# kkrt-labs/stwo-brainfuck

Hardware: AMD Instinct MI355X
Metric: trace cells committed+proved/sec (higher is better)
Workload: dtype u32 (M31 / QM31 modular arithmetic)

## Files before the change

bindings/rust/bfhip_sys.rs:

```rust
#![allow(non_camel_case_types, dead_code)]
use std::ffi::{c_char, c_void};

#[repr(C)] pub struct BfhipCtx { _private: [u8; 0] }
#[repr(C)] pub struct BfhipTrace { _private: [u8; 0] }
#[repr(C)] #[derive(Clone, Copy, Default, Debug, PartialEq, Eq)] pub struct BfhipConventions { pub merkle_node_hash: u32, pub mix_u64: u32, pub logup_mask_order: u32, pub merkle_channel: u32, pub reserved: [u32; 4] }
#[repr(C)] #[derive(Clone, Copy, Debug, PartialEq, Eq)] pub struct BfhipPcsConfig { pub pow_bits: u32, pub log_blowup_factor: u32, pub log_last_layer_degree_bound: u32, pub n_queries: u32, pub reserved: [u32; 4] }
#[repr(C)] #[derive(Clone, Copy, Default, Debug, PartialEq, Eq)] pub struct BfhipCheckReport { pub component: u32, pub log_size: u32, pub n_bad_cells: u64, pub first_bad_cell: u64, pub first_bad_constraint: i32, pub first_bad_value: [u32; 4], pub bad_per_constraint: [u64; 16], pub claimed_sum: [u32; 4], pub reserved: [u32; 3] }
#[repr(C)] #[derive(Clone, Copy, Default, Debug, PartialEq, Eq)] pub struct BfhipRelationEntry { pub relation: u32, pub n_words: u32, pub tuple: [u32; 7], pub net: u32, pub n_yield: u64, pub n_use: u64, pub n_other: u64, pub first_yield_table: i32, pub first_use_table: i32, pub first_yield_row: u64, pub first_use_row: u64, pub reserved: [u32; 2] }
#[repr(C)] #[derive(Clone, Copy, Default, Debug, PartialEq, Eq)] pub struct BfhipRelationReport { pub relation: u32, pub n_words: u32, pub n_entries: u64, pub n_tuples: u64, pub n_unbalanced: u64, pub n_reported: u64, pub reserved: [u32; 2] }
#[repr(C)] #[derive(Clone, Copy, Debug)] pub struct BfhipRelationTable { pub component: i32, pub log_size: u32, pub main_rows_h: *const *const u32 }
#[repr(C)] pub struct BfhipLocalGroup { _private: [u8; 0] }
#[repr(C)] pub struct BfhipPool { _private: [u8; 0] }
#[repr(C)] pub struct BfhipChannel { _private: [u8; 0] }
#[repr(C)] pub struct BfhipPcs { _private: [u8; 0] }
#[repr(C)] pub struct BfhipPcsVerifier { _private: [u8; 0] }
#[repr(C)] pub struct BfhipAir { _private: [u8; 0] }
#[repr(C)] pub struct BfhipAirKernel { _private: [u8; 0] }
#[repr(C)] #[derive(Clone, Copy, Debug, PartialEq, Eq)] pub struct BfhipAirCheckReport { pub log_size: u32, pub n_constraints: u32, pub n_bad_cells: u64, pub first_bad_cell: u64, pub first_bad_constraint: i32, pub reserved0: u32, pub first_bad_value: [u32; 4], pub bad_per_constraint: [u64; 64], pub first_cell_per_constraint: [u64; 64], pub reserved: [u64; 2] }
#[repr(C)] pub struct BfhipLogup { _private: [u8; 0] }
#[repr(C)] pub struct BfhipRelationProgram { _private: [u8; 0] }
#[repr(C)] #[derive(Clone, Copy, Debug)] pub struct BfhipRelationProgramTable { pub program: *const BfhipRelationProgram, pub log_size: u32, pub row_shift: u32, pub cols_h: *const *const u32, pub col_shifts_h: *const u32 }
#[repr(C)] #[derive(Clone, Copy, Default, Debug, PartialEq, Eq)] pub struct BfhipMultiplicityReport { pub relation: u32, pub n_words: u32, pub target_table: u32, pub target_entry: u32, pub n_rows: u64, pub n_row_tuples: u64, pub n_entries: u64, pub n_tuples: u64, pub n_filled: u64, pub n_missing: u64, pub n_reported: u64, pub reserved: [u32; 2] }
#[repr(C)] #[derive(Clone, Copy, Debug)] pub struct BfhipPoolResult { pub ticket: u64, pub user_tag: u64, pub status: i32, pub worker: u32, pub flags: u32, pub log_max_rows: u32, pub proof_json: *mut c_char, pub proof_len: usize, pub error: *mut c_char, pub seconds_queued: f64, pub seconds_proving: f64, pub reserved: [u64; 2] }
#[repr(C)] #[derive(Clone, Copy, Debug)] pub struct BfhipPreflightReport { pub ran: u32, pub rejected: u32, pub n_bad_components: i32, pub n_entries: u32, pub logup_total: [u32; 4], pub components: [BfhipCheckReport; 13], pub relations: [BfhipRelationReport; 3], pub entries: [BfhipRelationEntry; 12], pub seconds: f64, pub reserved: [u64; 3] }
pub const BFHIP_TRACE_REJECTED: i32 = -3;
pub const BFHIP_JOB_CANCELLED: i32 = -2;
pub const BFHIP_POOL_MAX_OUTSTANDING: u32 = 4096;
pub const BFHIP_PCS_MAX_SAMPLES_PER_COLUMN: u32 = 2;
pub const BFHIP_PCS_MAX_POINTS: u32 = 64;
pub const BFHIP_PCS_MAX_COLUMNS: u32 = 4096;
pub const BFHIP_PCS_MAX_TREES: u32 = 64;
pub const BFHIP_AIR_M_COL: u32 = 0; pub const BFHIP_AIR_M_CONST: u32 = 1; pub const BFHIP_AIR_M_ADD: u32 = 2; pub const BFHIP_AIR_M_SUB: u32 = 3;
pub const BFHIP_AIR_M_MUL: u32 = 4; pub const BFHIP_AIR_M_NEG: u32 = 5; pub const BFHIP_AIR_Q_COL: u32 = 6; pub const BFHIP_AIR_Q_PARAM: u32 = 7;
pub const BFHIP_AIR_Q_FROM_M: u32 = 8; pub const BFHIP_AIR_Q_ADD: u32 = 9; pub const BFHIP_AIR_Q_SUB: u32 = 10; pub const BFHIP_AIR_Q_MUL: u32 = 11;
pub const BFHIP_AIR_Q_MULM: u32 = 12; pub const BFHIP_AIR_C_BASE: u32 = 13; pub const BFHIP_AIR_C_EXT: u32 = 14;
pub const BFHIP_AIR_MAX_M_REGS: u32 = 96; pub const BFHIP_AIR_MAX_Q_REGS: u32 = 24; pub const BFHIP_AIR_MAX_INSTRUCTIONS: u32 = 4096;
pub const BFHIP_AIR_MAX_COLUMNS: u32 = 256; pub const BFHIP_AIR_MAX_PARAMS: u32 = 64; pub const BFHIP_AIR_MAX_CONSTRAINTS: u32 = 64;
pub const BFHIP_AIR_MAX_OFFSET: i32 = 16;
pub const BFHIP_LOGUP_FRAC: u32 = 15; pub const BFHIP_LOGUP_END_COL: u32 = 16; pub const BFHIP_LOGUP_MAX_COLUMNS: u32 = 8; pub const BFHIP_LOGUP_MAX_FRACTIONS: u32 = 32;
pub const BFHIP_REL_WORD: u32 = 17; pub const BFHIP_REL_ENTRY: u32 = 18; pub const BFHIP_RELATION_PROGRAM_MAX_RELATIONS: u32 = 16;
pub const BFHIP_RELATION_PROGRAM_MAX_WORDS: u32 = 7; pub const BFHIP_RELATION_PROGRAM_MAX_ENTRIES: u32 = 32;

#[link(name = "bfhip")]
extern "C" {
    pub fn bfhip_last_error() -> *const c_char;
    pub fn bfhip_device_count() -> i32;
    pub fn bfhip_device_memory(device_id: i32, free_bytes: *mut u64, total_bytes: *mut u64) -> i32;
    pub fn bfhip_ctx_create(device_id: i32, max_log_domain: u32, out: *mut *mut BfhipCtx) -> i32;
    pub fn bfhip_ctx_destroy(ctx: *mut BfhipCtx) -> i32;
    pub fn bfhip_ctx_sync(ctx: *mut BfhipCtx) -> i32;
    pub fn bfhip_ctx_set_overlap(ctx: *mut BfhipCtx, mask: u32) -> i32;
    pub fn bfhip_ctx_memory(ctx: *mut BfhipCtx, out: *mut u64) -> i32;
    pub fn bfhip_ctx_set_sync_policy(ctx: *mut BfhipCtx, blocking: i32) -> i32;
    pub fn bfhip_ctx_set_mailbox(ctx: *mut BfhipCtx, mode: i32, timeout_ms: u32, test_delay_ms: i32) -> i32;
    pub fn bfhip_ctx_set_conventions(ctx: *mut BfhipCtx, conv: *const BfhipConventions) -> i32;
    pub fn bfhip_ctx_get_conventions(ctx: *mut BfhipCtx, out: *mut BfhipConventions) -> i32;
    pub fn bfhip_ctx_set_pcs_config(ctx: *mut BfhipCtx, pcs: *const BfhipPcsConfig) -> i32;
    pub fn bfhip_ctx_get_pcs_config(ctx: *mut BfhipCtx, out: *mut BfhipPcsConfig) -> i32;
    pub fn bfhip_malloc(ctx: *mut BfhipCtx, bytes: usize, out_d: *mut *mut c_void) -> i32;
    pub fn bfhip_free(ctx: *mut BfhipCtx, ptr_d: *mut c_void) -> i32;
    pub fn bfhip_upload(ctx: *mut BfhipCtx, dst_d: *mut c_void, src_h: *const c_void, bytes: usize) -> i32;
    pub fn bfhip_download(ctx: *mut BfhipCtx, dst_h: *mut c_void, src_d: *const c_void, bytes: usize) -> i32;
    pub fn bfhip_memset_zero(ctx: *mut BfhipCtx, dst_d: *mut c_void, bytes: usize) -> i32;
    pub fn bfhip_twiddles(ctx: *mut BfhipCtx, tw_d: *mut *const u32, itw_d: *mut *const u32, root_log: *mut u32) -> i32;
    pub fn bfhip_interpolate(ctx: *mut BfhipCtx, src_cols_h: *const *mut u32, dst_cols_h: *const *mut u32, n_cols: u32, log_size: u32, replicated: i32) -> i32;
    pub fn bfhip_evaluate(ctx: *mut BfhipCtx, coeff_cols_h: *const *mut u32, dst_cols_h: *const *mut u32, n_cols: u32, log_size: u32, log_eval: u32, replicated: i32) -> i32;
    pub fn bfhip_is_first_coeffs(ctx: *mut BfhipCtx, log_min: u32, log_max: u32, dst_cols_h: *const *mut u32) -> i32;
    pub fn bfhip_is_first_lde(ctx: *mut BfhipCtx, log_min: u32, log_max: u32, log_blowup: u32, dst_cols_h: *const *mut u32) -> i32;
    pub fn bfhip_is_first_eval_at_point(ctx: *mut BfhipCtx, log_size: u32, point_h: *const u32, out_h: *mut u32) -> i32;
    pub fn bfhip_broadcast16(ctx: *mut BfhipCtx, rows_d: *const u32, dst_d: *mut u32, n_rows: usize) -> i32;
    pub fn bfhip_bit_reverse(ctx: *mut BfhipCtx, src_d: *const u32, dst_d: *mut u32, log_size: u32) -> i32;
    pub fn bfhip_batch_inverse_m31(ctx: *mut BfhipCtx, src_d: *const u32, dst_d: *mut u32, n: usize) -> i32;
    pub fn bfhip_batch_inverse_qm31(ctx: *mut BfhipCtx, src_d: *const *const u32, dst_d: *const *mut u32, n: usize) -> i32;
    pub fn bfhip_accumulate(ctx: *mut BfhipCtx, dst_d: *mut u32, src_d: *const u32, n: usize) -> i32;
    pub fn bfhip_eval_at_point(ctx: *mut BfhipCtx, coeffs_d: *const u32, log_size: u32, replicated: i32, point_h: *const u32, out_h: *mut u32) -> i32;
    pub fn bfhip_merkle_commit_layer(ctx: *mut BfhipCtx, log_size: u32, prev_layer_d: *const c_void, cols_h: *const *const u32, col_shifts_h: *const u32, n_cols: u32, out_hashes_d: *mut c_void) -> i32;
    pub fn bfhip_merkle_commit_layer_poseidon252(ctx: *mut BfhipCtx, log_size: u32, prev_layer_d: *const c_void, cols_h: *const *const u32, col_shifts_h: *const u32, n_cols: u32, out_hashes_d: *mut c_void) -> i32;
    pub fn bfhip_hades_permutation(ctx: *mut BfhipCtx, in_h: *const u32, out_h: *mut u32) -> i32;
    pub fn bfhip_fold_line(ctx: *mut BfhipCtx, src_d: *const *const u32, dst_d: *const *mut u32, log_size: u32, alpha_h: *const u32) -> i32;
    pub fn bfhip_fold_circle_into_line(ctx: *mut BfhipCtx, dst_d: *const *mut u32, src_d: *const *const u32, log_size: u32, alpha_h: *const u32) -> i32;
    pub fn bfhip_fri_fold_leaf(ctx: *mut BfhipCtx, src_d: *const *const u32, quot_d: *const *const u32, dst_d: *const *mut u32, log_size: u32, alpha_h: *const u32, out_hashes_d: *mut c_void) -> i32;
    pub fn bfhip_grind(ctx: *mut BfhipCtx, digest_h: *const u8, pow_bits: u32, nonce: *mut u64) -> i32;
    pub fn bfhip_grind_poseidon252(ctx: *mut BfhipCtx, digest_h: *const u8, pow_bits: u32, start_nonce: u64, nonce: *mut u64, tried: *mut u64) -> i32;
    pub fn bfhip_gather(ctx: *mut BfhipCtx, col_d: *const u32, idx_h: *const u64, n: usize, out_h: *mut u32) -> i32;
    pub fn bfhip_component_shape(component: i32, n_main_cols: *mut u32, n_logup_cols: *mut u32, n_constraints: *mut u32) -> i32;
    pub fn bfhip_logup_generate(ctx: *mut BfhipCtx, component: i32, log_size: u32, main_rows_h: *const *const u32, lookup_h: *const u32, out_cols_h: *const *mut u32, claimed_sum_h: *mut u32) -> i32;
    pub fn bfhip_eval_constraints(ctx: *mut BfhipCtx, component: i32, log_size: u32, is_first_d: *const u32, main_lde_h: *const *const u32, main_shifts_h: *const u32, inter_lde_h: *const *const u32, inter_shifts_h: *const u32, lookup_h: *const u32, claimed_sum_h: *const u32, coeffs_h: *const u32, acc_d: *const *mut u32) -> i32;
    pub fn bfhip_check_constraints(ctx: *mut BfhipCtx, component: i32, log_size: u32, main_rows_h: *const *const u32, logup_cols_h: *const *const u32, lookup_h: *const u32, claimed_sum_h: *const u32, out: *mut BfhipCheckReport) -> i32;
    pub fn bfhip_accumulate_quotients(ctx: *mut BfhipCtx, log_size: u32, cols_h: *const *const u32, col_shifts_h: *const u32, n_cols: u32, n_samples_h: *const u32, sample_points_h: *const u32, sample_values_h: *const u32, random_coeff_h: *const u32, out_d: *const *mut u32) -> i32;
    pub fn bfhip_prove_brainfuck(ctx: *mut BfhipCtx, code: *const c_char, input_h: *const u8, n_input: usize, log_max_rows: u32, proof_json: *mut *mut c_char, proof_len: *mut usize, transcript: *mut *mut c_char, phase_seconds: *mut f64) -> i32;
    pub fn bfhip_free_host(p: *mut c_void);
    pub fn bfhip_ctx_last_proof_flags(ctx: *mut BfhipCtx, flags: *mut u32) -> i32;
    pub fn bfhip_local_group_create(count: u32, out: *mut *mut BfhipLocalGroup) -> i32;
    pub fn bfhip_local_group_destroy(group: *mut BfhipLocalGroup) -> i32;
    pub fn bfhip_ctx_join_local_group(ctx: *mut BfhipCtx, group: *mut BfhipLocalGroup, rank: u32) -> i32;
    pub fn bfhip_rccl_unique_id(id: *mut u8) -> i32;
    pub fn bfhip_ctx_join_rccl_group(ctx: *mut BfhipCtx, id: *const u8, rank: u32, count: u32) -> i32;
    pub fn bfhip_ctx_leave_group(ctx: *mut BfhipCtx) -> i32;
    pub fn bfhip_ctx_set_shard_policy(ctx: *mut BfhipCtx, policy: i32) -> i32;
    pub fn bfhip_ctx_group_stats(ctx: *mut BfhipCtx, out: *mut u64) -> i32;
    pub fn bfhip_ctx_group_times(ctx: *mut BfhipCtx, out_ms: *mut f64) -> i32;
    pub fn bfhip_ctx_group_latency(ctx: *mut BfhipCtx, reset: i32, out_us: *mut f64) -> i32;
    pub fn bfhip_rccl_exchange_raw(id: *const u8, rank: u32, count: u32, n_sends: u32, send_peer: *const u32, send_ptr: *const *mut c_void, send_bytes: *const usize, n_recvs: u32, recv_peer: *const u32, recv_ptr: *const *mut c_void, recv_bytes: *const usize, stats_out: *mut u64) -> i32;
    pub fn bfhip_rccl_selftest(ctx: *mut BfhipCtx) -> i32;
    pub fn bfhip_ctx_group_info(ctx: *mut BfhipCtx, rank: *mut u32, count: *mut u32, transport: *mut *const c_char) -> i32;
    pub fn bfhip_ctx_reuse_preprocessed(ctx: *mut BfhipCtx, on: i32) -> i32;
    pub fn bfhip_trace_create(ctx: *mut BfhipCtx, code: *const c_char, input_h: *const u8, n_input: usize, out: *mut *mut BfhipTrace, log_sizes: *mut u32, n_steps: *mut u64, main_cells: *mut u64, interaction_cells: *mut u64) -> i32;
    pub fn bfhip_trace_create_ram(ctx: *mut BfhipCtx, code: *const c_char, input_h: *const u8, n_input: usize, ram_size: usize, out: *mut *mut BfhipTrace, log_sizes: *mut u32, n_steps: *mut u64, main_cells: *mut u64, interaction_cells: *mut u64) -> i32;
    pub fn bfhip_trace_create_from_registers(ctx: *mut BfhipCtx, trace7_h: *const u32, n_rows: usize, code_words_h: *const u32, n_code: usize, out: *mut *mut BfhipTrace, log_sizes: *mut u32, main_cells: *mut u64, interaction_cells: *mut u64) -> i32;
    pub fn bfhip_trace_destroy(ctx: *mut BfhipCtx, trace: *mut BfhipTrace) -> i32;
    pub fn bfhip_ctx_set_table_builder(ctx: *mut BfhipCtx, on_gpu: i32) -> i32;
    pub fn bfhip_trace_column(ctx: *mut BfhipCtx, trace: *const BfhipTrace, component: u32, column: u32, out_h: *mut u32, cap: usize, n_rows: *mut usize) -> i32;
    pub fn bfhip_prove_trace(ctx: *mut BfhipCtx, trace: *const BfhipTrace, log_max_rows: u32, proof_json: *mut *mut c_char, proof_len: *mut usize, transcript: *mut *mut c_char, phase_seconds: *mut f64) -> i32;
    pub fn bfhip_prove_registers(ctx: *mut BfhipCtx, trace7_h: *const u32, n_rows: usize, code_words_h: *const u32, n_code: usize, log_max_rows: u32, proof_json: *mut *mut c_char, proof_len: *mut usize, transcript: *mut *mut c_char, phase_seconds: *mut f64) -> i32;
    pub fn bfhip_trace_check(ctx: *mut BfhipCtx, trace: *const BfhipTrace, lookup_h: *const u32, out: *mut BfhipCheckReport, logup_total_h: *mut u32, n_bad_components: *mut i32) -> i32;
    pub fn bfhip_relation_summary(ctx: *mut BfhipCtx, tables: *const BfhipRelationTable, n_tables: u32, out: *mut BfhipRelationReport, entries_h: *mut BfhipRelationEntry, cap_per_relation: u32) -> i32;
    pub fn bfhip_trace_relations(ctx: *mut BfhipCtx, trace: *const BfhipTrace, out: *mut BfhipRelationReport, entries_h: *mut BfhipRelationEntry, cap_per_relation: u32) -> i32;
    pub fn bfhip_ctx_set_preflight(ctx: *mut BfhipCtx, on: i32) -> i32;
    pub fn bfhip_ctx_get_preflight(ctx: *mut BfhipCtx, on: *mut i32) -> i32;
    pub fn bfhip_ctx_last_preflight(ctx: *mut BfhipCtx, out: *mut BfhipPreflightReport) -> i32;
    pub fn bfhip_format_preflight(rep: *const BfhipPreflightReport, buf: *mut c_char, cap: usize, need: *mut usize) -> i32;
    pub fn bfhip_pool_create(device_id: i32, n_in_flight: u32, max_log_domain: u32, out: *mut *mut BfhipPool) -> i32;
    pub fn bfhip_pool_destroy(pool: *mut BfhipPool) -> i32;
    pub fn bfhip_pool_size(pool: *mut BfhipPool, n_in_flight: *mut u32) -> i32;
    pub fn bfhip_pool_ctx(pool: *mut BfhipPool, i: u32, out: *mut *mut BfhipCtx) -> i32;
    pub fn bfhip_pool_set_conventions(pool: *mut BfhipPool, conv: *const BfhipConventions) -> i32;
    pub fn bfhip_pool_set_preprocessed(pool: *mut BfhipPool, mode: i32) -> i32;
    pub fn bfhip_pool_set_pcs_config(pool: *mut BfhipPool, pcs: *const BfhipPcsConfig) -> i32;
    pub fn bfhip_pool_set_preflight(pool: *mut BfhipPool, on: i32) -> i32;
    pub fn bfhip_prove_batch(pool: *mut BfhipPool, traces: *const *const BfhipTrace, n: u32, log_max_rows: u32, proofs_json: *mut *mut c_char, proof_lens: *mut usize, statuses: *mut i32, seconds: *mut f64) -> i32;
    pub fn bfhip_prove_batch_brainfuck(pool: *mut BfhipPool, codes: *const *const c_char, inputs_h: *const *const u8, n_inputs: *const usize, n: u32, log_max_rows: u32, proofs_json: *mut *mut c_char, proof_lens: *mut usize, statuses: *mut i32, seconds: *mut f64) -> i32;
    pub fn bfhip_pool_submit_trace(pool: *mut BfhipPool, trace: *const BfhipTrace, log_max_rows: u32, user_tag: u64, ticket: *mut u64) -> i32;
    pub fn bfhip_pool_submit_brainfuck(pool: *mut BfhipPool, code: *const c_char, input_h: *const u8, n_input: usize, log_max_rows: u32, user_tag: u64, ticket: *mut u64) -> i32;
    pub fn bfhip_pool_submit_registers(pool: *mut BfhipPool, trace7_h: *const u32, n_rows: usize, code_words_h: *const u32, n_code: usize, log_max_rows: u32, user_tag: u64, ticket: *mut u64) -> i32;
    pub fn bfhip_pool_wait(pool: *mut BfhipPool, timeout_ms: u32, out: *mut BfhipPoolResult) -> i32;
    pub fn bfhip_pool_outstanding(pool: *mut BfhipPool, queued: *mut u32, running: *mut u32, finished_not_taken: *mut u32) -> i32;
    pub fn bfhip_pool_cancel(pool: *mut BfhipPool, ticket: u64) -> i32;
    pub fn bfhip_verify_brainfuck(proof_json: *const c_char, proof_len: usize, log_max_rows: u32, err: *mut c_char, err_cap: usize) -> i32;
    pub fn bfhip_verify_brainfuck_conv(proof_json: *const c_char, proof_len: usize, log_max_rows: u32, conv: *const BfhipConventions, err: *mut c_char, err_cap: usize) -> i32;
    pub fn bfhip_verify_brainfuck_pcs(proof_json: *const c_char, proof_len: usize, log_max_rows: u32, conv: *const BfhipConventions, pcs: *const BfhipPcsConfig, err: *mut c_char, err_cap: usize) -> i32;
    pub fn bfhip_channel_create(conv: *const BfhipConventions, out: *mut *mut BfhipChannel) -> i32;
    pub fn bfhip_channel_destroy(ch: *mut BfhipChannel) -> i32;
    pub fn bfhip_channel_mix_root(ch: *mut BfhipChannel, hash32: *const u8) -> i32;
    pub fn bfhip_channel_mix_u64(ch: *mut BfhipChannel, v: u64) -> i32;
    pub fn bfhip_channel_mix_felts(ch: *mut BfhipChannel, felts_h: *const u32, n: usize) -> i32;
    pub fn bfhip_channel_draw_felts(ch: *mut BfhipChannel, n: usize, out_h: *mut u32) -> i32;
    pub fn bfhip_channel_draw_point(ch: *mut BfhipChannel, point_out: *mut u32) -> i32;
    pub fn bfhip_channel_state(ch: *mut BfhipChannel, digest: *mut u8, n_sent: *mut u32) -> i32;
    pub fn bfhip_channel_trailing_zeros(ch: *mut BfhipChannel, out: *mut u32) -> i32;
// ... 45 lines not shown
```

include/bfhip.h:

```cpp
#ifndef BFHIP_H
#define BFHIP_H
#include <stdint.h>
#include <stddef.h>

#ifdef __cplusplus
extern "C" {
#endif

typedef struct bfhip_ctx bfhip_ctx;
typedef struct bfhip_trace bfhip_trace;

enum { BFHIP_MERKLE_STWO_COMPRESS = 0, BFHIP_MERKLE_RFC7693 = 1 };
enum { BFHIP_MIX_U64_COMPRESS = 0, BFHIP_MIX_U64_HASH = 1 };
enum { BFHIP_LOGUP_MASK_CUR_PREV = 0, BFHIP_LOGUP_MASK_PREV_CUR = 1 };
enum { BFHIP_CHANNEL_BLAKE2S = 0, BFHIP_CHANNEL_POSEIDON252 = 1 };
typedef struct bfhip_conventions {
    uint32_t merkle_node_hash;
    uint32_t mix_u64;
    uint32_t logup_mask_order;
    uint32_t merkle_channel;
    uint32_t reserved[4];
} bfhip_conventions;

const char* bfhip_last_error(void);
int32_t bfhip_device_count(void);
int32_t bfhip_device_memory(int32_t device_id, uint64_t* free_bytes, uint64_t* total_bytes);

int32_t bfhip_ctx_create(int32_t device_id, uint32_t max_log_domain, bfhip_ctx** out);
int32_t bfhip_ctx_destroy(bfhip_ctx* ctx);
int32_t bfhip_ctx_sync(bfhip_ctx* ctx);
int32_t bfhip_ctx_set_overlap(bfhip_ctx* ctx, uint32_t mask);
int32_t bfhip_ctx_memory(bfhip_ctx* ctx, uint64_t out[4]);
int32_t bfhip_ctx_set_sync_policy(bfhip_ctx* ctx, int32_t blocking);
int32_t bfhip_ctx_set_mailbox(bfhip_ctx* ctx, int32_t mode, uint32_t timeout_ms, int32_t test_delay_ms);

int32_t bfhip_ctx_set_conventions(bfhip_ctx* ctx, const bfhip_conventions* conv);
int32_t bfhip_ctx_get_conventions(bfhip_ctx* ctx, bfhip_conventions* out);

enum { BFHIP_MAX_QUERIES = 256, BFHIP_MAX_LOG_BLOWUP = 16, BFHIP_MAX_POW_BITS = 32 };
typedef struct bfhip_pcs_config {
    uint32_t pow_bits;
    uint32_t log_blowup_factor;
    uint32_t log_last_layer_degree_bound;
    uint32_t n_queries;
    uint32_t reserved[4];
} bfhip_pcs_config;
int32_t bfhip_ctx_set_pcs_config(bfhip_ctx* ctx, const bfhip_pcs_config* pcs);
int32_t bfhip_ctx_get_pcs_config(bfhip_ctx* ctx, bfhip_pcs_config* out);

int32_t bfhip_malloc(bfhip_ctx* ctx, size_t bytes, void** out_d);
int32_t bfhip_free(bfhip_ctx* ctx, void* ptr_d);
int32_t bfhip_upload(bfhip_ctx* ctx, void* dst_d, const void* src_h, size_t bytes);
int32_t bfhip_download(bfhip_ctx* ctx, void* dst_h, const void* src_d, size_t bytes);
int32_t bfhip_memset_zero(bfhip_ctx* ctx, void* dst_d, size_t bytes);

int32_t bfhip_twiddles(bfhip_ctx* ctx, const uint32_t** tw_d, const uint32_t** itw_d, uint32_t* root_log);

int32_t bfhip_interpolate(bfhip_ctx* ctx, uint32_t* const* src_cols_h, uint32_t* const* dst_cols_h, uint32_t n_cols, uint32_t log_size, int32_t replicated);
int32_t bfhip_evaluate(bfhip_ctx* ctx, uint32_t* const* coeff_cols_h, uint32_t* const* dst_cols_h, uint32_t n_cols, uint32_t log_size, uint32_t log_eval, int32_t replicated);

int32_t bfhip_is_first_coeffs(bfhip_ctx* ctx, uint32_t log_min, uint32_t log_max, uint32_t* const* dst_cols_h);
int32_t bfhip_is_first_lde(bfhip_ctx* ctx, uint32_t log_min, uint32_t log_max, uint32_t log_blowup, uint32_t* const* dst_cols_h);
int32_t bfhip_is_first_eval_at_point(bfhip_ctx* ctx, uint32_t log_size, const uint32_t point_h[8], uint32_t out_h[4]);


int32_t bfhip_broadcast16(bfhip_ctx* ctx, const uint32_t* rows_d, uint32_t* dst_d, size_t n_rows);
int32_t bfhip_bit_reverse(bfhip_ctx* ctx, const uint32_t* src_d, uint32_t* dst_d, uint32_t log_size);
int32_t bfhip_batch_inverse_m31(bfhip_ctx* ctx, const uint32_t* src_d, uint32_t* dst_d, size_t n);
int32_t bfhip_batch_inverse_qm31(bfhip_ctx* ctx, const uint32_t* const src_d[4], uint32_t* const dst_d[4], size_t n);
int32_t bfhip_accumulate(bfhip_ctx* ctx, uint32_t* dst_d, const uint32_t* src_d, size_t n);
int32_t bfhip_eval_at_point(bfhip_ctx* ctx, const uint32_t* coeffs_d, uint32_t log_size, int32_t replicated, const uint32_t point_h[8], uint32_t out_h[4]);
int32_t bfhip_merkle_commit_layer(bfhip_ctx* ctx, uint32_t log_size, const void* prev_layer_d, const uint32_t* const* cols_h, const uint32_t* col_shifts_h,
                                  uint32_t n_cols, void* out_hashes_d);
int32_t bfhip_merkle_commit_layer_poseidon252(bfhip_ctx* ctx, uint32_t log_size, const void* prev_layer_d, const uint32_t* const* cols_h,
                                             const uint32_t* col_shifts_h, uint32_t n_cols, void* out_hashes_d);
int32_t bfhip_hades_permutation(bfhip_ctx* ctx, const uint32_t in_h[24], uint32_t out_h[24]);
int32_t bfhip_fold_line(bfhip_ctx* ctx, const uint32_t* const src_d[4], uint32_t* const dst_d[4], uint32_t log_size, const uint32_t alpha_h[4]);
int32_t bfhip_fold_circle_into_line(bfhip_ctx* ctx, uint32_t* const dst_d[4], const uint32_t* const src_d[4], uint32_t log_size, const uint32_t alpha_h[4]);
int32_t bfhip_fri_fold_leaf(bfhip_ctx* ctx, const uint32_t* const src_d[4], const uint32_t* const quot_d[4], uint32_t* const dst_d[4], uint32_t log_size,
                            const uint32_t alpha_h[4], void* out_hashes_d);
int32_t bfhip_grind(bfhip_ctx* ctx, const uint8_t digest_h[32], uint32_t pow_bits, uint64_t* nonce);
int32_t bfhip_grind_poseidon252(bfhip_ctx* ctx, const uint8_t digest_h[32], uint32_t pow_bits, uint64_t start_nonce,
                                uint64_t* nonce, uint64_t* tried);
int32_t bfhip_gather(bfhip_ctx* ctx, const uint32_t* col_d, const uint64_t* idx_h, size_t n, uint32_t* out_h);


int32_t bfhip_component_shape(int32_t component, uint32_t* n_main_cols, uint32_t* n_logup_cols, uint32_t* n_constraints);
int32_t bfhip_logup_generate(bfhip_ctx* ctx, int32_t component, uint32_t log_size, const uint32_t* const* main_rows_h, const uint32_t lookup_h[24],
                             uint32_t* const* out_cols_h, uint32_t claimed_sum_h[4]);
int32_t bfhip_eval_constraints(bfhip_ctx* ctx, int32_t component, uint32_t log_size, const uint32_t* is_first_d, const uint32_t* const* main_lde_h,
                               const uint32_t* main_shifts_h, const uint32_t* const* inter_lde_h, const uint32_t* inter_shifts_h, const uint32_t lookup_h[24],
                               const uint32_t claimed_sum_h[4], const uint32_t* coeffs_h, uint32_t* const acc_d[4]);
typedef struct bfhip_check_report {
    uint32_t component, log_size;
    uint64_t n_bad_cells;
    uint64_t first_bad_cell;
    int32_t  first_bad_constraint;
    uint32_t first_bad_value[4];
    uint64_t bad_per_constraint[16];
    uint32_t claimed_sum[4];
    uint32_t reserved[3];
} bfhip_check_report;
int32_t bfhip_check_constraints(bfhip_ctx* ctx, int32_t component, uint32_t log_size, const uint32_t* const* main_rows_h, const uint32_t* const* logup_cols_h,
                                const uint32_t lookup_h[24], const uint32_t claimed_sum_h[4], bfhip_check_report* out);
int32_t bfhip_accumulate_quotients(bfhip_ctx* ctx, uint32_t log_size, const uint32_t* const* cols_h, const uint32_t* col_shifts_h, uint32_t n_cols,
                                   const uint32_t* n_samples_h, const uint32_t* sample_points_h, const uint32_t* sample_values_h,
                                   const uint32_t random_coeff_h[4], uint32_t* const out_d[4]);

int32_t bfhip_prove_brainfuck(bfhip_ctx* ctx, const char* code, const uint8_t* input_h, size_t n_input, uint32_t log_max_rows,
                              char** proof_json, size_t* proof_len, char** transcript, double* phase_seconds);
void bfhip_free_host(void* p);
int32_t bfhip_ctx_last_proof_flags(bfhip_ctx* ctx, uint32_t* flags);
typedef struct bfhip_local_group bfhip_local_group;
int32_t bfhip_local_group_create(uint32_t count, bfhip_local_group** out);
int32_t bfhip_local_group_destroy(bfhip_local_group* group);
int32_t bfhip_ctx_join_local_group(bfhip_ctx* ctx, bfhip_local_group* group, uint32_t rank);
int32_t bfhip_rccl_unique_id(uint8_t id[128]);
int32_t bfhip_ctx_join_rccl_group(bfhip_ctx* ctx, const uint8_t id[128], uint32_t rank, uint32_t count);
int32_t bfhip_ctx_leave_group(bfhip_ctx* ctx);
int32_t bfhip_ctx_set_shard_policy(bfhip_ctx* ctx, int32_t policy);
int32_t bfhip_ctx_group_stats(bfhip_ctx* ctx, uint64_t out[4]);
int32_t bfhip_ctx_group_times(bfhip_ctx* ctx, double out_ms[3]);
int32_t bfhip_ctx_group_latency(bfhip_ctx* ctx, int32_t reset, double out_us[21]);
int32_t bfhip_rccl_exchange_raw(const uint8_t id[128], uint32_t rank, uint32_t count, uint32_t n_sends, const uint32_t* send_peer, void* const* send_ptr,
                                const size_t* send_bytes, uint32_t n_recvs, const uint32_t* recv_peer, void* const* recv_ptr, const size_t* recv_bytes,
                                uint64_t stats_out[4]);
int32_t bfhip_rccl_selftest(bfhip_ctx* ctx);
int32_t bfhip_ctx_group_info(bfhip_ctx* ctx, uint32_t* rank, uint32_t* count, const char** transport);

int32_t bfhip_ctx_reuse_preprocessed(bfhip_ctx* ctx, int32_t on);

int32_t bfhip_trace_create(bfhip_ctx* ctx, const char* code, const uint8_t* input_h, size_t n_input, bfhip_trace** out,
                           uint32_t log_sizes[13], uint64_t* n_steps, uint64_t* main_cells, uint64_t* interaction_cells);
int32_t bfhip_trace_create_ram(bfhip_ctx* ctx, const char* code, const uint8_t* input_h, size_t n_input, size_t ram_size, bfhip_trace** out,
                               uint32_t log_sizes[13], uint64_t* n_steps, uint64_t* main_cells, uint64_t* interaction_cells);
int32_t bfhip_trace_create_from_registers(bfhip_ctx* ctx, const uint32_t* trace7_h, size_t n_rows, const uint32_t* code_words_h, size_t n_code,
                                          bfhip_trace** out, uint32_t log_sizes[13], uint64_t* main_cells, uint64_t* interaction_cells);
int32_t bfhip_trace_destroy(bfhip_ctx* ctx, bfhip_trace* trace);
int32_t bfhip_ctx_set_table_builder(bfhip_ctx* ctx, int32_t on_gpu);
int32_t bfhip_trace_column(bfhip_ctx* ctx, const bfhip_trace* trace, uint32_t component, uint32_t column, uint32_t* out_h, size_t cap, size_t* n_rows);
int32_t bfhip_prove_trace(bfhip_ctx* ctx, const bfhip_trace* trace, uint32_t log_max_rows, char** proof_json, size_t* proof_len,
                          char** transcript, double* phase_seconds);
// ... 221 lines not shown
```

stwo-brainfuck_amd/__init__.py:

```python
import ctypes
import os
import weakref

import numpy as np

_HERE = os.path.dirname(os.path.abspath(__file__))
_LIB_PATH = os.environ.get("BFHIP_LIBRARY") or os.path.join(_HERE, "libbfhip.so")
TESTHOOKS_LIBRARY = os.path.join(_HERE, "libbfhip_testhooks.so")
_lib = None

P = (1 << 31) - 1


class BfhipError(RuntimeError):
    pass


def lib():
    global _lib
    if _lib is None:
        if not os.path.exists(_LIB_PATH):
            raise BfhipError(f"{_LIB_PATH} is missing: build it with __graft_entry__.build(); there is no CPU fallback")
        _lib = ctypes.CDLL(_LIB_PATH)
        _lib.bfhip_last_error.restype = ctypes.c_char_p
# ... 368 lines not shown
        out = (ctypes.c_double * 6)()
        _check(lib().bfhip_clock_probe_mix(self._h, ctypes.c_double(seconds), int(log_nodes), out))
        d = dict(zip(("ghz", "G_compressions_per_s", "launches", "us_per_launch", "sampler_spanned_the_window", "sampler_seconds"), [float(v) for v in out]))
        d["sampler_spanned_the_window"] = bool(d["sampler_spanned_the_window"])
        return d

    def memory(self):
        out = (ctypes.c_uint64 * 4)()
        _check(lib().bfhip_ctx_memory(self._h, out))
        return dict(zip(("arena_reserved", "arena_peak", "twiddles", "arena_in_use"), [int(v) for v in out]))

    def set_table_builder(self, on_gpu=True):
        _check(lib().bfhip_ctx_set_table_builder(self._h, int(on_gpu)))

    def join_local_group(self, group, rank):
        _check(lib().bfhip_ctx_join_local_group(self._h, group._h, rank))
        self._group = group

    def join_rccl_group(self, unique_id: bytes, rank, count):
        if len(unique_id) != 128:
            raise BfhipError("an RCCL unique id has 128 bytes")
        _check(lib().bfhip_ctx_join_rccl_group(self._h, unique_id, rank, count))

    def set_shard_policy(self, policy=-1):
        _check(lib().bfhip_ctx_set_shard_policy(self._h, int(policy)))

    def leave_group(self):
        _check(lib().bfhip_ctx_leave_group(self._h))
        self._group = None

    def group_stats(self):
        out = (ctypes.c_uint64 * 4)()
        _check(lib().bfhip_ctx_group_stats(self._h, out))
        return dict(zip(("all_gathers", "max_reduces", "exchanges", "bytes_sent"), [int(v) for v in out]))

    def group_times(self):
        out = (ctypes.c_double * 3)()
        _check(lib().bfhip_ctx_group_times(self._h, out))
        return dict(zip(("all_gather_ms", "max_reduce_ms", "exchange_ms"), [float(v) for v in out]))

    def group_latency(self, reset=False):
        out = (ctypes.c_double * 21)()
        _check(lib().bfhip_ctx_group_latency(self._h, 1 if reset else 0, out))
        res = {}
        for k, name in enumerate(("all_gather", "max_reduce", "exchange")):
            v = [float(x) for x in out[7 * k:7 * k + 7]]
            res[name] = {"count": int(v[0]), "gpu_us": {"p50": round(v[1], 1), "p90": round(v[2], 1), "max": round(v[3], 1)},
                         "host_us": {"p50": round(v[4], 1), "p90": round(v[5], 1), "max": round(v[6], 1)}}
        return res

    def group_info(self):
        r, n, t = ctypes.c_uint32(), ctypes.c_uint32(), ctypes.c_char_p()
        _check(lib().bfhip_ctx_group_info(self._h, ctypes.byref(r), ctypes.byref(n), ctypes.byref(t)))
        return r.value, n.value, (t.value or b"").decode()

    def malloc(self, nbytes):
        p = ctypes.c_void_p()
        _check(lib().bfhip_malloc(self._h, ctypes.c_size_t(nbytes), ctypes.byref(p)))
        return p.value

    def free(self, ptr):
        _check(lib().bfhip_free(self._h, ctypes.c_void_p(ptr)))

    def upload(self, arr):
        arr = np.ascontiguousarray(arr)
        ptr = self.malloc(arr.nbytes)
        _check(lib().bfhip_upload(self._h, ctypes.c_void_p(ptr), arr.ctypes.data_as(ctypes.c_void_p), ctypes.c_size_t(arr.nbytes)))
        return ptr

    def download(self, ptr, n, dtype=np.uint32):
        out = np.empty(n, dtype=dtype)
        _check(lib().bfhip_download(self._h, out.ctypes.data_as(ctypes.c_void_p), ctypes.c_void_p(ptr), ctypes.c_size_t(out.nbytes)))
        return out

    @staticmethod
    def _ptr_array(ptrs):
        return (ctypes.c_void_p * len(ptrs))(*ptrs)

    def interpolate(self, src_ptrs, dst_ptrs, log_size, replicated=False):
        _check(lib().bfhip_interpolate(self._h, self._ptr_array(src_ptrs), self._ptr_array(dst_ptrs), len(src_ptrs), log_size, int(replicated)))

    def evaluate(self, coeff_ptrs, dst_ptrs, log_size, log_eval, replicated=False):
        _check(lib().bfhip_evaluate(self._h, self._ptr_array(coeff_ptrs), self._ptr_array(dst_ptrs), len(coeff_ptrs), log_size, log_eval, int(replicated)))

    def is_first_coeffs(self, log_min, log_max, dst_ptrs):
        arr = (ctypes.c_void_p * len(dst_ptrs))(*[p or None for p in dst_ptrs])
        _check(lib().bfhip_is_first_coeffs(self._h, log_min, log_max, arr))

    def is_first_lde(self, log_min, log_max, log_blowup, dst_ptrs):
        arr = (ctypes.c_void_p * len(dst_ptrs))(*[p or None for p in dst_ptrs])
        _check(lib().bfhip_is_first_lde(self._h, log_min, log_max, log_blowup, arr))

    def is_first_eval_at_point(self, log_size, point8):
        pt = (ctypes.c_uint32 * 8)(*[int(v) for v in point8])
        out = (ctypes.c_uint32 * 4)()
        _check(lib().bfhip_is_first_eval_at_point(self._h, log_size, pt, out))
        return list(out)

    def eval_at_point(self, coeff_ptr, log_size, point8, replicated=False):
        pt = (ctypes.c_uint32 * 8)(*[int(v) for v in point8])
        out = (ctypes.c_uint32 * 4)()
        _check(lib().bfhip_eval_at_point(self._h, ctypes.c_void_p(coeff_ptr), log_size, int(replicated), pt, out))
        return list(out)

    def broadcast16(self, rows_ptr, dst_ptr, n_rows):
        _check(lib().bfhip_broadcast16(self._h, ctypes.c_void_p(rows_ptr), ctypes.c_void_p(dst_ptr), ctypes.c_size_t(n_rows)))

    def bit_reverse(self, src_ptr, dst_ptr, log_size):
        _check(lib().bfhip_bit_reverse(self._h, ctypes.c_void_p(src_ptr), ctypes.c_void_p(dst_ptr), log_size))

    def batch_inverse_m31(self, src_ptr, dst_ptr, n):
        _check(lib().bfhip_batch_inverse_m31(self._h, ctypes.c_void_p(src_ptr), ctypes.c_void_p(dst_ptr), ctypes.c_size_t(n)))

    def batch_inverse_qm31(self, src_ptrs, dst_ptrs, n):
        _check(lib().bfhip_batch_inverse_qm31(self._h, self._ptr_array(src_ptrs), self._ptr_array(dst_ptrs), ctypes.c_size_t(n)))

    def accumulate(self, dst_ptr, src_ptr, n):
        _check(lib().bfhip_accumulate(self._h, ctypes.c_void_p(dst_ptr), ctypes.c_void_p(src_ptr), ctypes.c_size_t(n)))

    def merkle_commit_layer(self, log_size, prev_ptr, col_ptrs, out_ptr, col_shifts=None):
        sh = None if col_shifts is None else (ctypes.c_uint32 * len(col_shifts))(*col_shifts)
        _check(lib().bfhip_merkle_commit_layer(self._h, log_size, ctypes.c_void_p(prev_ptr) if prev_ptr else None, self._ptr_array(col_ptrs), sh, len(col_ptrs), ctypes.c_void_p(out_ptr)))

    def merkle_commit_layer_poseidon252(self, log_size, prev_ptr, col_ptrs, out_ptr, col_shifts=None):
        sh = None if col_shifts is None else (ctypes.c_uint32 * len(col_shifts))(*col_shifts)
        _check(lib().bfhip_merkle_commit_layer_poseidon252(self._h, log_size, ctypes.c_void_p(prev_ptr) if prev_ptr else None, self._ptr_array(col_ptrs), sh, len(col_ptrs), ctypes.c_void_p(out_ptr)))

    def hades_permutation(self, state3):
        words = []
        for x in state3:
            words += [(int(x) >> (32 * i)) & 0xFFFFFFFF for i in range(8)]
        out = (ctypes.c_uint32 * 24)()
        _check(lib().bfhip_hades_permutation(self._h, (ctypes.c_uint32 * 24)(*words), out))
        return [sum(int(out[8 * k + i]) << (32 * i) for i in range(8)) for k in range(3)]

    def fold_line(self, src_ptrs, dst_ptrs, log_size, alpha4):
        _check(lib().bfhip_fold_line(self._h, self._ptr_array(src_ptrs), self._ptr_array(dst_ptrs), log_size, (ctypes.c_uint32 * 4)(*[int(v) for v in alpha4])))

    def fri_fold_leaf(self, src_ptrs, quot_ptrs, dst_ptrs, log_size, alpha4, out_ptr):
        _check(lib().bfhip_fri_fold_leaf(self._h, self._ptr_array(src_ptrs) if src_ptrs is not None else None, self._ptr_array(quot_ptrs) if quot_ptrs is not None else None,
                                         self._ptr_array(dst_ptrs), log_size, (ctypes.c_uint32 * 4)(*[int(v) for v in alpha4]), ctypes.c_void_p(out_ptr)))

    def fold_circle_into_line(self, dst_ptrs, src_ptrs, log_size, alpha4):
        _check(lib().bfhip_fold_circle_into_line(self._h, self._ptr_array(dst_ptrs), self._ptr_array(src_ptrs), log_size, (ctypes.c_uint32 * 4)(*[int(v) for v in alpha4])))

    def grind(self, digest32, pow_bits):
        nonce = ctypes.c_uint64()
        _check(lib().bfhip_grind(self._h, bytes(digest32), pow_bits, ctypes.byref(nonce)))
        return nonce.value

    def grind_poseidon252(self, digest32, pow_bits, start_nonce=0, with_tried=False):
        digest32 = bytes(digest32)
        if len(digest32) != 32:
            raise ValueError("grind_poseidon252: the digest is 32 bytes")
        nonce, tried = ctypes.c_uint64(), ctypes.c_uint64()
        _check(lib().bfhip_grind_poseidon252(self._h, digest32, ctypes.c_uint32(pow_bits), ctypes.c_uint64(start_nonce), ctypes.byref(nonce), ctypes.byref(tried)))
        return (nonce.value, tried.value) if with_tried else nonce.value

    def gather(self, col_ptr, indices):
        idx = np.ascontiguousarray(indices, dtype=np.uint64)
        out = np.empty(idx.size, dtype=np.uint32)
        _check(lib().bfhip_gather(self._h, ctypes.c_void_p(col_ptr), idx.ctypes.data_as(ctypes.c_void_p), ctypes.c_size_t(idx.size), out.ctypes.data_as(ctypes.c_void_p)))
        return out

    @staticmethod
    def _u32s(values):
# ... 1162 lines not shown
```

stwo-brainfuck_amd/csrc/api.hip:

```cpp
#include "../../include/bfhip.h"
#include "api_guard.h"
#include "prover.h"
#include <cstdlib>
#include "host/circle.h"
#include "host/quotients.h"
#include "host/hash.h"
#include <cstdio>
#include <vector>
#include <algorithm>
#include <chrono>

using namespace bf;

static thread_local std::string g_err;
void bfhip_set_error(const std::string& s) { g_err = s; }

namespace bf {

void Ctx::ensure_aux() { for (auto& a : aux) if (!a) BF_HIP(hipStreamCreateWithFlags(&a, hipStreamNonBlocking)); }
void Ctx::ensure_side() { if (!stream2) BF_HIP(hipStreamCreateWithFlags(&stream2, hipStreamNonBlocking)); }

void Ctx::init(int dev, u32 max_log_domain, const Ctx* tables_from) {
    int n = 0;
    if (hipGetDeviceCount(&n) != hipSuccess || n == 0) throw HipError("no HIP device: the bfhip backend has no CPU fallback");
// ... 407 lines not shown
    return 0;
    API_CATCH
}
int32_t bfhip_ctx_memory(bfhip_ctx* ctx, uint64_t out[4]) {
    API_CTX(ctx)
    if (!out) throw HipError("null argument");
    uint64_t reserved = 0;
    for (auto& ch : ctx->c.arena.chunks) reserved += ch.size;
    out[0] = reserved; out[1] = ctx->c.arena.peak; out[2] = ctx->c.owns_tables ? (uint64_t)(2 * sizeof(u32)) << ctx->c.tw_root_log : 0;
    out[3] = ctx->c.arena.total_used;
    return 0;
    API_CATCH
}
int32_t bfhip_ctx_get_conventions(bfhip_ctx* ctx, bfhip_conventions* out) {
    API_CTX(ctx)
    if (!out) throw HipError("null argument");
    bfhip_conventions r{};
    r.merkle_node_hash = ctx->c.conv.merkle_node_hash; r.mix_u64 = ctx->c.conv.mix_u64; r.logup_mask_order = ctx->c.conv.logup_mask_order; r.merkle_channel = ctx->c.conv.merkle_channel;
    *out = r;
    return 0;
    API_CATCH
}
int32_t bfhip_ctx_sync(bfhip_ctx* ctx) { API_CTX(ctx) ctx->c.sync(); return 0; API_CATCH }

int32_t bfhip_malloc(bfhip_ctx* ctx, size_t bytes, void** out_d) { API_CTX(ctx) BF_HIP(hipSetDevice(ctx->c.device)); BF_HIP(hipMalloc(out_d, bytes ? bytes : 4)); return 0; API_CATCH }
int32_t bfhip_free(bfhip_ctx* ctx, void* p) { API_CTX(ctx) (void)ctx; BF_HIP(hipFree(p)); return 0; API_CATCH }
int32_t bfhip_upload(bfhip_ctx* ctx, void* dst_d, const void* src_h, size_t bytes) {
    API_CTX(ctx) BF_HIP(hipMemcpyAsync(dst_d, src_h, bytes, hipMemcpyHostToDevice, ctx->c.stream)); ctx->c.sync(); return 0; API_CATCH
}
int32_t bfhip_download(bfhip_ctx* ctx, void* dst_h, const void* src_d, size_t bytes) {
    API_CTX(ctx) BF_HIP(hipMemcpyAsync(dst_h, src_d, bytes, hipMemcpyDeviceToHost, ctx->c.stream)); ctx->c.sync(); return 0; API_CATCH
}
int32_t bfhip_memset_zero(bfhip_ctx* ctx, void* dst_d, size_t bytes) { API_CTX(ctx) BF_HIP(hipMemsetAsync(dst_d, 0, bytes, ctx->c.stream)); return 0; API_CATCH }

int32_t bfhip_twiddles(bfhip_ctx* ctx, const uint32_t** tw_d, const uint32_t** itw_d, uint32_t* root_log) {
    API_CTX(ctx) if (!tw_d || !itw_d || !root_log) throw HipError("null argument"); *tw_d = ctx->c.d_tw; *itw_d = ctx->c.d_itw; *root_log = ctx->c.tw_root_log; return 0; API_CATCH
}

int32_t bfhip_interpolate(bfhip_ctx* ctx, uint32_t* const* src_cols_h, uint32_t* const* dst_cols_h, uint32_t n_cols, uint32_t log_size, int32_t replicated) {
    API_CTX(ctx)
    Ctx& c = ctx->c;
    if (replicated && log_size < 4) throw HipError("replicated columns need log_size >= 4");
    if (!replicated && log_size < 3) throw HipError("circle transforms need log_size >= 3");
    if (log_size > c.tw_root_log + 1) throw HipError("log_size exceeds the context's twiddle tree");
    u32 log = replicated ? log_size - 4 : log_size;
    c.stage_checkpoint();
    StageBatch sb(c);
    auto* s = c.stage(src_cols_h, n_cols);
    auto* d = c.stage(dst_cols_h, n_cols);
    const FftJob job{(const u32* const*)s, (u32* const*)d, n_cols, log, log, !replicated};
    FftPlan plan;
    fft_plan(plan, true, &job, 1, c.d_tw, c.d_itw, c.tw_root_log);
    plan.d_groups = c.stage(plan.groups.data(), plan.groups.size());
    sb.end();
    fft_run(c.stream, plan);
    BF_HIP(hipGetLastError());
    return 0;
    API_CATCH
}

int32_t bfhip_evaluate(bfhip_ctx* ctx, uint32_t* const* coeff_cols_h, uint32_t* const* dst_cols_h, uint32_t n_cols, uint32_t log_size, uint32_t log_eval, int32_t replicated) {
    API_CTX(ctx)
    Ctx& c = ctx->c;
    if (log_eval < log_size) throw HipError("log_eval < log_size");
    if (replicated && log_size < 4) throw HipError("replicated columns need log_size >= 4");
    if (!replicated && log_eval < 3) throw HipError("circle transforms need log_eval >= 3");
    if (log_eval > c.tw_root_log + 1) throw HipError("log_eval exceeds the context's twiddle tree");
    u32 sh = replicated ? 4 : 0;
    c.stage_checkpoint();
    StageBatch sb(c);
    auto* s = c.stage(coeff_cols_h, n_cols);
    auto* d = c.stage(dst_cols_h, n_cols);
    const FftJob job{(const u32* const*)s, (u32* const*)d, n_cols, log_eval - sh, log_size - sh, !replicated};
    FftPlan plan;
    fft_plan(plan, false, &job, 1, c.d_tw, c.d_itw, c.tw_root_log);
    plan.d_groups = c.stage(plan.groups.data(), plan.groups.size());
    sb.end();
    fft_run(c.stream, plan);
    BF_HIP(hipGetLastError());
    return 0;
    API_CATCH
}


int32_t bfhip_is_first_coeffs(bfhip_ctx* ctx, uint32_t log_min, uint32_t log_max, uint32_t* const* dst_cols_h) {
    API_CTX(ctx)
    if (!dst_cols_h) throw HipError("null argument");
    if (log_min < 4 || log_max < log_min || log_max - log_min >= 28) throw HipError("is_first_coeffs: need 4 <= log_min <= log_max < log_min + 28");
    if (log_max > ctx->c.tw_root_log + 1) throw HipError("log_max exceeds the context's twiddle tree");
    IsFirstCols a{}; a.log_min = log_min; a.log_max = log_max;
    for (u32 n = log_min; n <= log_max; n++) a.ptr[n - log_min] = dst_cols_h[n - log_min];
    is_first_coeffs(ctx->c.stream, a, ctx->c.d_itw, ctx->c.tw_root_log);
    BF_HIP(hipGetLastError());
    return 0;
    API_CATCH
}
int32_t bfhip_is_first_lde(bfhip_ctx* ctx, uint32_t log_min, uint32_t log_max, uint32_t log_blowup, uint32_t* const* dst_cols_h) {
    API_CTX(ctx)
    if (!dst_cols_h) throw HipError("null argument");
    if (log_min < 4 || log_max < log_min || log_max - log_min >= 28) throw HipError("is_first_lde: need 4 <= log_min <= log_max < log_min + 28");
    if (log_blowup > 31 || log_max + log_blowup > ctx->c.tw_root_log + 1 || log_max + log_blowup > 31) throw HipError("log_max + log_blowup exceeds the context's twiddle tree");
    IsFirstCols a{}; a.log_min = log_min; a.log_max = log_max;
    for (u32 n = log_min; n <= log_max; n++) a.ptr[n - log_min] = dst_cols_h[n - log_min];
    is_first_lde(ctx->c.stream, a, log_blowup, ctx->c.d_tw, ctx->c.d_itw, ctx->c.tw_root_log);
    BF_HIP(hipGetLastError());
    return 0;
    API_CATCH
}
int32_t bfhip_is_first_eval_at_point(bfhip_ctx* ctx, uint32_t log_size, const uint32_t point_h[8], uint32_t out_h[4]) {
    API_CTX(ctx)
    Ctx& c = ctx->c;
    if (!point_h || !out_h) throw HipError("null argument");
    if (log_size < 4 || log_size > 31 || log_size > c.tw_root_log + 1) throw HipError("is_first_eval_at_point: need 4 <= log_size within the context's twiddle tree");
    c.stage_checkpoint();
    uint4 factors[32];
    Q31 x = q_make(point_h[0], point_h[1], point_h[2], point_h[3]);
    factors[0] = make_uint4(point_h[4], point_h[5], point_h[6], point_h[7]);
    for (u32 b = 1; b < 32; b++) { factors[b] = make_uint4(x.a.a, x.a.b, x.b.a, x.b.b); Q31 s = q_mul(x, x); x = q_subm(q_add(s, s), 1); }
    IsFirstSample job{log_size, 0, 0};
    const IsFirstSample* dj = c.stage(&job, 1);
    const uint4* df = c.stage(factors, 32);
    uint4* dout = nullptr;
    BF_HIP(hipMalloc((void**)&dout, sizeof(uint4)));
    is_first_samples(c.stream, dj, 1, df, dout, c.d_itw, c.tw_root_log);
    uint4 r;
    hipError_t e = hipMemcpyAsync(&r, dout, sizeof(uint4), hipMemcpyDeviceToHost, c.stream);
    if (e == hipSuccess) e = hipStreamSynchronize(c.stream);
    (void)hipFree(dout);
    BF_HIP(e);
    out_h[0] = r.x; out_h[1] = r.y; out_h[2] = r.z; out_h[3] = r.w;
    return 0;
    API_CATCH
}
int32_t bfhip_broadcast16(bfhip_ctx* ctx, const uint32_t* rows_d, uint32_t* dst_d, size_t n_rows) {
    API_CTX(ctx) broadcast16(ctx->c.stream, rows_d, dst_d, (u32)(n_rows * 16)); BF_HIP(hipGetLastError()); return 0; API_CATCH
}
int32_t bfhip_bit_reverse(bfhip_ctx* ctx, const uint32_t* src_d, uint32_t* dst_d, uint32_t log_size) {
    API_CTX(ctx) if (src_d == dst_d) throw HipError("bit_reverse is out of place"); bit_reverse(ctx->c.stream, src_d, dst_d, log_size); BF_HIP(hipGetLastError()); return 0; API_CATCH
}
int32_t bfhip_batch_inverse_m31(bfhip_ctx* ctx, const uint32_t* src_d, uint32_t* dst_d, size_t n) {
    API_CTX(ctx) batch_inverse_m31(ctx->c.stream, src_d, dst_d, (u32)n); BF_HIP(hipGetLastError()); return 0; API_CATCH
}
int32_t bfhip_batch_inverse_qm31(bfhip_ctx* ctx, const uint32_t* const src_d[4], uint32_t* const dst_d[4], size_t n) {
    API_CTX(ctx) batch_inverse_qm31(ctx->c.stream, src_d, dst_d, (u32)n); BF_HIP(hipGetLastError()); return 0; API_CATCH
}
int32_t bfhip_accumulate(bfhip_ctx* ctx, uint32_t* dst_d, const uint32_t* src_d, size_t n) {
    API_CTX(ctx) accumulate(ctx->c.stream, dst_d, src_d, (u32)n); BF_HIP(hipGetLastError()); return 0; API_CATCH
}
int32_t bfhip_eval_at_point(bfhip_ctx* ctx, const uint32_t* coeffs_d, uint32_t log_size, int32_t replicated, const uint32_t point_h[8], uint32_t out_h[4]) {
    API_CTX(ctx)
    Ctx& c = ctx->c;
    if (replicated && log_size < 4) throw HipError("replicated columns need log_size >= 4");
    c.stage_checkpoint();
    uint4 factors[32];
    Q31 x = q_make(point_h[0], point_h[1], point_h[2], point_h[3]);
    factors[0] = make_uint4(point_h[4], point_h[5], point_h[6], point_h[7]);
    for (u32 b = 1; b < 32; b++) { factors[b] = make_uint4(x.a.a, x.a.b, x.b.a, x.b.b); Q31 s = q_mul(x, x); x = q_subm(q_add(s, s), 1); }
    EvalJob job{coeffs_d, replicated ? log_size - 4 : log_size, 0, replicated ? 4u : 0u, 0};
    const EvalJob* dj = c.stage(&job, 1);
    const uint4* df = c.stage(factors, 32);
    u32 nchunks = job.log_n > 12 ? 1u << (job.log_n - 12) : 1u;
    uint4* partials = nullptr; uint4* dout = nullptr;
    BF_HIP(hipMalloc((void**)&partials, sizeof(uint4) * (nchunks + 1)));
    dout = partials + nchunks;
    eval_at_points(c.stream, dj, 1, nchunks, df, partials, dout);
    uint4 r;
// ... 417 lines not shown
```

stwo-brainfuck_amd/csrc/fft.hip:

```cpp
#include "kernels.h"
#include <cstdio>
#include <cstdlib>
#include <stdexcept>
#include <algorithm>
#include <vector>
#include <mutex>
#include <set>
#include <string>

namespace bf {

static constexpr int TILE_LOG = 12;
static constexpr int TILE = 1 << TILE_LOG;
static constexpr int CHUNK_LOG = 5;
static constexpr int STRIDED_K = TILE_LOG - CHUNK_LOG;
static constexpr int FFT_THREADS = 256;
__device__ __forceinline__ u32 scale_shift(u32 scale) { return (u32)__builtin_ctz(scale); }

__device__ __forceinline__ void point_of_index(u32 idx, const uint2* __restrict__ tlo, const uint2* __restrict__ thi, u32& x, u32& y) {
    uint2 a = tlo[idx & 0xffffu], b = thi[(idx >> 16) & 0x7fffu];
    x = m_sub(m_mul(a.x, b.x), m_mul(a.y, b.y));
    y = m_add(m_mul(a.x, b.y), m_mul(a.y, b.x));
}

__global__ void k_gen_twiddles(u32* __restrict__ tw, u32* __restrict__ itw, u32 R, const uint2* __restrict__ tlo, const uint2* __restrict__ thi) {
    u32 g = blockIdx.x * blockDim.x + threadIdx.x;
    u32 total = 1u << R;
    if (g >= total) return;
    if (g == total - 1) { tw[g] = 1; itw[g] = 1; return; }
    u32 j = __clz(~(g << (32 - R)));
    u32 off = total - (1u << (R - j));
    u32 k = g - off;
    u32 bits = R - 1 - j;
    u32 init = (1u << (31 - R - 2)) << j, step = (1u << (31 - R)) << j;
    u32 idx = (init + step * bit_rev(k, bits)) & 0x7fffffffu;
    u32 x, y;
    point_of_index(idx, tlo, thi, x, y);
    tw[g] = x;
    itw[g] = m_inv(x);
}

__global__ void __launch_bounds__(256) k_is_first_coeffs(IsFirstCols a, const u32* __restrict__ itw, u32 tw_total) {
    const u32 u = blockIdx.x * blockDim.x + threadIdx.x + (1u << (a.log_min - 4));
    if (u >= (1u << (a.log_max - 3))) return;
    const u32 n = 35u - __clz(u);
    u32* __restrict__ dst = a.ptr[n - a.log_min];
    if (!dst) return;
    const u32 jhi = u - (1u << (n - 4));
    auto t = [&](u32 i) -> u32 { return i == 0 ? itw[tw_total - (1u << (n - 1)) + 1] : itw[tw_total - (1u << (n - i))]; };
    u32 v[16];
    v[0] = m_inv_pow2(n);
    for (u32 i = 4; i < n; i++) if ((jhi >> (i - 4)) & 1) v[0] = m_mul(v[0], t(i));
#pragma unroll
    for (u32 b = 0; b < 4; b++) {
        const u32 tb = t(b);
#pragma unroll
        for (u32 e = 0; e < (1u << b); e++) v[e + (1u << b)] = m_mul(v[e], tb);
    }
    uint4* o = reinterpret_cast<uint4*>(dst + 16 * (size_t)jhi);
#pragma unroll
    for (int q = 0; q < 4; q++) o[q] = make_uint4(v[4 * q], v[4 * q + 1], v[4 * q + 2], v[4 * q + 3]);
}
void is_first_coeffs(hipStream_t stream, const IsFirstCols& a, const u32* itw, u32 tw_root_log) {
    if (a.log_min < 4 || a.log_max < a.log_min || a.log_max - a.log_min >= 28 || a.log_max > tw_root_log + 1) throw std::runtime_error("is_first_coeffs: unsupported sizes");
    const u32 lanes = (1u << (a.log_max - 3)) - (1u << (a.log_min - 4));
    hipLaunchKernelGGL(k_is_first_coeffs, dim3((lanes + 255) / 256), dim3(256), 0, stream, a, itw, 1u << tw_root_log);
}

__global__ void __launch_bounds__(256) k_is_first_lde(IsFirstCols a, u32 log_blowup, const u32* __restrict__ tw, const u32* __restrict__ itw, u32 tw_total) {
    const u32 u = blockIdx.x * blockDim.x + threadIdx.x;
    if (u < (1u << (a.log_min + log_blowup - 4)) || u >= (1u << (a.log_max + log_blowup - 3))) return;
    const u32 N = 35u - __clz(u), n = N - log_blowup;
    u32* __restrict__ dst = a.ptr[n - a.log_min];
    if (!dst) return;
    const u32 chi = u - (1u << (N - 4));
    auto t = [&](u32 i) -> u32 { return i == 0 ? itw[tw_total - (1u << (n - 1)) + 1] : itw[tw_total - (1u << (n - i))]; };
    u32 pre = m_inv_pow2(n), lane_layers = n;
    if (u >= 64u) {
        const u32 cw = __builtin_amdgcn_readfirstlane(chi >> 6), nw = __builtin_amdgcn_readfirstlane(n), Nw = nw + log_blowup;
        u32 pw = m_inv_pow2(nw);
        for (u32 i = 10; i < nw; i++) {
            const u32 f = m_mul(itw[tw_total - (1u << (nw - i))], tw[tw_total - (1u << (Nw - i)) + (cw >> (i - 9))]);
            pw = m_mul(pw, (cw >> (i - 10)) & 1 ? m_sub(1u, f) : m_add(1u, f));
        }
        pre = pw; lane_layers = min(n, 10u);
    }
    for (u32 i = 4; i < lane_layers; i++) {
        const u32 f = m_mul(t(i), tw[tw_total - (1u << (N - i)) + (chi >> (i - 3))]);
        pre = m_mul(pre, (chi >> (i - 4)) & 1 ? m_sub(1u, f) : m_add(1u, f));
    }
    const uint4 l0 = *reinterpret_cast<const uint4*>(tw + (tw_total - (1u << (N - 1))) + 4 * (size_t)chi);
    const u32 l0w[4] = {l0.x, l0.y, l0.z, l0.w};
    const u32 t0 = t(0), t1 = t(1), t2 = t(2), t3 = t(3);
    const u32 f3 = m_mul(t3, tw[tw_total - (1u << (N - 3)) + chi]);
    u32 w3[2] = {m_mul(pre, m_add(1u, f3)), m_mul(pre, m_sub(1u, f3))};
    u32 v[16];
#pragma unroll
    for (u32 b3 = 0; b3 < 2; b3++) {
        const u32 f2 = m_mul(t2, tw[tw_total - (1u << (N - 2)) + 2 * chi + b3]);
        const u32 w2[2] = {m_mul(w3[b3], m_add(1u, f2)), m_mul(w3[b3], m_sub(1u, f2))};
        const u32 gx = m_mul(t0, l0w[2 * b3]), gy = m_mul(t0, l0w[2 * b3 + 1]);
        const u32 py = m_add(1u, gy), ny = m_sub(1u, gy), px = m_add(1u, gx), nx = m_sub(1u, gx);
        const u32 f0[8] = {py, ny, ny, py, nx, px, px, nx};
#pragma unroll
        for (u32 b2 = 0; b2 < 2; b2++) {
            const u32 f1 = m_mul(t1, l0w[2 * b3 + b2]);
            const u32 w1[2] = {m_mul(w2[b2], m_add(1u, f1)), m_mul(w2[b2], m_sub(1u, f1))};
#pragma unroll
            for (u32 e = 0; e < 4; e++) v[8 * b3 + 4 * b2 + e] = m_mul(w1[e >> 1], f0[4 * b2 + e]);
        }
    }
    g_u32p o = as_global(dst) + 16 * (size_t)chi;
#pragma unroll
    for (int q = 0; q < 4; q++) st16(o + 4 * q, make_uint4(v[4 * q], v[4 * q + 1], v[4 * q + 2], v[4 * q + 3]));
}
__global__ void __launch_bounds__(64) k_is_first_samples(const IsFirstSample* __restrict__ jobs, const uint4* __restrict__ factors, uint4* __restrict__ out,
                                                         const u32* __restrict__ itw, u32 tw_total) {
    const IsFirstSample job = jobs[blockIdx.x];
    const u32 n = job.log_n, b = threadIdx.x;
    Q31 acc = q_one();
    if (b < n) {
        const u32 tb = b == 0 ? itw[tw_total - (1u << (n - 1)) + 1] : itw[tw_total - (1u << (n - b))];
        const uint4 f = factors[(size_t)job.point * 32 + b];
        acc = q_addm(q_mulm(q_make(f.x, f.y, f.z, f.w), tb), 1u);
    }
    for (int s = 1; s < 32; s <<= 1) {
        const Q31 o = q_make((u32)__shfl_xor((int)acc.a.a, s), (u32)__shfl_xor((int)acc.a.b, s), (u32)__shfl_xor((int)acc.b.a, s), (u32)__shfl_xor((int)acc.b.b, s));
        acc = q_mul(acc, o);
    }
    if (b == 0) { acc = q_mulm(acc, m_inv_pow2(n)); out[job.out_idx] = make_uint4(acc.a.a, acc.a.b, acc.b.a, acc.b.b); }
}
void is_first_samples(hipStream_t stream, const IsFirstSample* d_jobs, u32 n_jobs, const void* d_factors, void* d_out, const u32* itw, u32 tw_root_log) {
    if (!n_jobs) return;
    hipLaunchKernelGGL(k_is_first_samples, dim3(n_jobs), dim3(64), 0, stream, d_jobs, (const uint4*)d_factors, (uint4*)d_out, itw, 1u << tw_root_log);
}
void is_first_lde(hipStream_t stream, const IsFirstCols& a, u32 log_blowup, const u32* tw, const u32* itw, u32 tw_root_log) {
    if (a.log_min < 4 || a.log_max < a.log_min || a.log_max - a.log_min >= 28 || a.log_max + log_blowup > tw_root_log + 1 || a.log_max + log_blowup > 31)
        throw std::runtime_error("is_first_lde: unsupported sizes");
    const u32 lanes = 1u << (a.log_max + log_blowup - 3);
    double bytes = 0;
    for (u32 n = a.log_min; n <= a.log_max; n++) if (a.ptr[n - a.log_min]) bytes += 4.0 * (double)(1ull << (n + log_blowup));
    ProfScope ps(stream, "k_is_first_lde", bytes, bytes);
    hipLaunchKernelGGL(k_is_first_lde, dim3((lanes + 255) / 256), dim3(256), 0, stream, a, log_blowup, tw, itw, 1u << tw_root_log);
}

enum { K_TILE12 = 0, K_STRIDED5 = 1, K_STRIDED6 = 2, K_PASS = 3, K_TINY = 4, K_STRIDED_K8 = 5, K_STRIDED_K9 = 6, K_STRIDED_K10 = 7, K_KINDS = 8 };
struct BlockOfGroup { u32 g, tile, by; };
template <bool INV> __device__ __forceinline__ void fft_tiny_body(const PassArgs& a, const BlockOfGroup& bg);
__device__ __forceinline__ BlockOfGroup find_group(const PassArgs* __restrict__ groups, u32 ngroups) {
    u32 g = 0;
    while (g + 1 < ngroups && groups[g + 1].block0 <= blockIdx.x) g++;
    const u32 local = blockIdx.x - groups[g].block0, gx = groups[g].grid_x;
    return {g, local % gx, local / gx};
}
__device__ __forceinline__ const u32* layer_table(const PassArgs& a, u32 layer) {
    u32 eff = a.circle ? layer : layer + 1;
    u32 lg = a.circle ? a.log : a.log + 1;
    u32 len = 1u << (lg - 1 - eff);
    return a.tw + (a.tw_total - 2 * len);
}

template <bool INV>
__device__ __forceinline__ void fft_pass_body(const PassArgs& a, const BlockOfGroup& bg, u32* __restrict__ s_val, u32* __restrict__ s_tw) {
    const u32 t = threadIdx.x;
    const u32 lo = a.lo, k = a.k;
    const u32 c = lo == 0 ? 0 : CHUNK_LOG;
    const u32 tile_log = lo == 0 ? a.tile_log : k + c;
    const u32 tile_n = 1u << tile_log;
    const u32 kt = tile_log - c;
    const u32 tile = bg.tile;
    const u32 n_lhi_log = lo - c;
    const u32 H = lo ? (tile >> n_lhi_log) : 0, Lhi = lo ? (tile & ((1u << n_lhi_log) - 1)) : 0;
    const u32 base = lo ? ((H << (lo + k)) | (Lhi << c)) : (tile << tile_log);

    for (u32 e = t; e < (1u << kt) - (1u << (kt - k)); e += FFT_THREADS) {
        u32 j = __clz(~((e) << (32 - kt)));
        u32 off = (1u << kt) - (1u << (kt - j));
        u32 q = e - off;
        u32 gl = lo + j;
        u32 hbase = lo ? (H << (kt - 1 - j)) : (tile << (kt - 1 - j));
        u32 v;
        if (a.circle && gl == 0) {
            const u32* l0 = layer_table(a, 1);
            u32 h = hbase + q;
            u32 x = l0[(h >> 2) * 2], y = l0[(h >> 2) * 2 + 1];
            u32 sel = h & 3;
            v = sel == 0 ? y : sel == 1 ? m_neg(y) : sel == 2 ? m_neg(x) : x;
        } else {
            v = layer_table(a, gl)[hbase + q];
        }
        s_tw[e] = v;
    }

    const u32 col0 = bg.by * a.cols_per_block;
    const u32 col1 = min(a.ncols, col0 + a.cols_per_block);
    for (u32 col = col0; col < col1; col++) {
        g_cu32p src = as_global(a.src[col]);
        g_u32p dst = as_global(a.dst[col]);
        __syncthreads();
        for (u32 e4 = t * 4; e4 < tile_n; e4 += 4 * FFT_THREADS) {
            u32 gidx = lo ? (base | ((e4 >> c) << lo) | (e4 & ((1u << c) - 1))) : (base + e4);
            uint4 v = a.src_mask < 3u ? make_uint4(src[0], a.src_mask ? src[1] : 0u, 0u, 0u) : ld16(src + (gidx & a.src_mask));
            *reinterpret_cast<uint4*>(&s_val[e4]) = v;
        }
        __syncthreads();
        const u32 nb = tile_n >> 1;
        if (INV) {
            for (u32 j = 0; j < k; j++) {
                u32 dist = 1u << (j + c);
                u32 toff = (1u << kt) - (1u << (kt - j));
                for (u32 b = t; b < nb; b += FFT_THREADS) {
                    u32 i0 = ((b >> (j + c)) << (j + c + 1)) | (b & (dist - 1));
                    u32 tw = s_tw[toff + (b >> (j + c))];
                    u32 v0 = s_val[i0], v1 = s_val[i0 + dist];
                    s_val[i0] = m_add(v0, v1);
                    s_val[i0 + dist] = m_mul(m_sub(v0, v1), tw);
                }
                __syncthreads();
            }
        } else {
            for (int j = (int)k - 1; j >= 0; j--) {
                u32 dist = 1u << (j + c);
                u32 toff = (1u << kt) - (1u << (kt - j));
                for (u32 b = t; b < nb; b += FFT_THREADS) {
                    u32 i0 = ((b >> (j + c)) << (j + c + 1)) | (b & (dist - 1));
                    u32 tw = s_tw[toff + (b >> (j + c))];
                    u32 v0 = s_val[i0], v1 = m_mul(s_val[i0 + dist], tw);
                    s_val[i0] = m_add(v0, v1);
                    s_val[i0 + dist] = m_sub(v0, v1);
                }
                __syncthreads();
            }
        }
        for (u32 e4 = t * 4; e4 < tile_n; e4 += 4 * FFT_THREADS) {
            u32 gidx = lo ? (base | ((e4 >> c) << lo) | (e4 & ((1u << c) - 1))) : (base + e4);
            uint4 v = *reinterpret_cast<uint4*>(&s_val[e4]);
            if (INV && a.scale != 1) { const u32 sk = scale_shift(a.scale); v.x = m_mul_pow2(v.x, sk); v.y = m_mul_pow2(v.y, sk); v.z = m_mul_pow2(v.z, sk); v.w = m_mul_pow2(v.w, sk); }
            st16(dst + gidx, v);
        }
    }
}

template <bool INV>
// ... 80 lines not shown
#pragma unroll
            for (int s = 0; s < 2; s++) {
                const int L = INV ? s : 1 - s;
                if ((u32)L < k) {
#pragma unroll
                    for (int q = 0; q < 4; q++) {
                        u32 i = 1024 * q + 4 * t;
                        if (L == 0) { bfly<INV>(r[q][0], r[q][1], TW(0, i >> 1)); bfly<INV>(r[q][2], r[q][3], TW(0, (i >> 1) + 1)); }
                        else { u32 w = TW(1, i >> 2); bfly<INV>(r[q][0], r[q][2], w); bfly<INV>(r[q][1], r[q][3], w); }
                    }
                }
            }
        };
        auto stage_high = [&]() {
#pragma unroll
            for (int s = 0; s < 2; s++) {
                const int L = INV ? 10 + s : 11 - s;
                if ((u32)L < k) {
                    if (L == 10) { u32 w0 = TW(10, 0), w1 = TW(10, 1);
#pragma unroll
                        for (int j = 0; j < 4; j++) { bfly<INV>(r[0][j], r[1][j], w0); bfly<INV>(r[2][j], r[3][j], w1); } }
                    else { u32 w = TW(11, 0);
#pragma unroll
                        for (int j = 0; j < 4; j++) { bfly<INV>(r[0][j], r[2][j], w); bfly<INV>(r[1][j], r[3][j], w); } }
                }
            }
        };
        auto round_lds = [&](u32 first_layer) {
            u32 lo_bits = first_layer;
            u32 lo = t & ((1u << lo_bits) - 1), hi = t >> lo_bits;
            u32 idx0 = (hi << (lo_bits + 4)) | lo;
            u32 v[16];
#pragma unroll
            for (int e = 0; e < 16; e++) v[e] = s_val[lds_pad(idx0 | ((u32)e << lo_bits))];
            u32 nl = k > first_layer ? k - first_layer : 0;
            radix16<INV>(v, nl, [&](int jl, int pe) -> u32 { return TW(first_layer + jl, ((hi << 4) >> (jl + 1)) + pe); });
#pragma unroll
            for (int e = 0; e < 16; e++) s_val[lds_pad(idx0 | ((u32)e << lo_bits))] = v[e];
        };
        auto put = [&]() {
#pragma unroll
            for (int q = 0; q < 4; q++) *reinterpret_cast<uint4*>(&s_val[lds_pad(1024 * q + 4 * t)]) = make_uint4(r[q][0], r[q][1], r[q][2], r[q][3]);
        };
        auto get = [&]() {
#pragma unroll
            for (int q = 0; q < 4; q++) { uint4 v = *reinterpret_cast<uint4*>(&s_val[lds_pad(1024 * q + 4 * t)]); r[q][0] = v.x; r[q][1] = v.y; r[q][2] = v.z; r[q][3] = v.w; }
        };
        if (INV) {
            stage_low(); put(); __syncthreads();
            round_lds(2); __syncthreads();
            round_lds(6); __syncthreads();
            get(); stage_high();
        } else {
            stage_high(); put(); __syncthreads();
            round_lds(6); __syncthreads();
            round_lds(2); __syncthreads();
            get(); stage_low();
        }
#pragma unroll
        for (int q = 0; q < 4; q++) {
            uint4 v = make_uint4(r[q][0], r[q][1], r[q][2], r[q][3]);
            if (INV && a.scale != 1) { const u32 sk = scale_shift(a.scale); v.x = m_mul_pow2(v.x, sk); v.y = m_mul_pow2(v.y, sk); v.z = m_mul_pow2(v.z, sk); v.w = m_mul_pow2(v.w, sk); }
            st16(dst + base + 1024 * q + 4 * t, v);
        }
    }
}

template <bool INV>
__global__ void __launch_bounds__(256) k_fft_tile12(const PassArgs* __restrict__ groups, u32 ngroups, u32 generic) {
    const BlockOfGroup bg = find_group(groups, ngroups);
    const PassArgs a = groups[bg.g];
    __shared__ __attribute__((aligned(16))) u32 s_val[4096 + 4 * 64];
    __shared__ u32 s_tw[4096];
    if (a.kind == K_PASS) { fft_pass_body<INV>(a, bg, s_val, s_tw); return; }
    if (a.kind == K_TINY) { fft_tiny_body<INV>(a, bg); return; }
    const u32 k = generic ? 0u : a.k;
    if (k == 12) fft_tile12_body<INV, 12>(a, bg, s_val, s_tw);
    else if (k == 11) fft_tile12_body<INV, 11>(a, bg, s_val, s_tw);
    else if (k == 10) fft_tile12_body<INV, 10>(a, bg, s_val, s_tw);
    else if (k == 9) fft_tile12_body<INV, 9>(a, bg, s_val, s_tw);
    else fft_tile12_body<INV, 0>(a, bg, s_val, s_tw);
}

template <bool INV, int CL>
__global__ void __launch_bounds__(4 << CL, 3) k_fft_strided7(const PassArgs* __restrict__ groups, u32 ngroups) {
    const BlockOfGroup bg = find_group(groups, ngroups);
    const PassArgs a = groups[bg.g];
    constexpr u32 C = 1u << CL, NT = 4u << CL;
    __shared__ __attribute__((aligned(16))) u32 s_val[128 * C];
    __shared__ u32 s_tw[128];
    const u32 t = threadIdx.x, lo = a.lo, tile = bg.tile;
    const u32 n_lhi_log = lo - CL;
    const u32 H = tile >> n_lhi_log, Lhi = tile & ((1u << n_lhi_log) - 1);
    const u32 base = (H << (lo + 7)) | (Lhi << CL);
    if (t < 127) {
        u32 j = __clz(~(t << 25));
        u32 q = t - (128u - (128u >> j));
        s_tw[t] = 2u * layer_table(a, lo + j)[(H << (6 - j)) + q];
    }
    auto TW = [&](u32 layer, u32 idx) -> u32 { return s_tw[128u - (128u >> layer) + idx]; };
    const u32 col0 = bg.by * a.cols_per_block, col1 = min(a.ncols, col0 + a.cols_per_block);
    const u32 l4 = 4 * (t & (C / 4 - 1)), r4 = t >> (CL - 2);
    for (u32 col = col0; col < col1; col++) {
        g_cu32p src = as_global(a.src[col]);
        g_u32p dst = as_global(a.dst[col]);
        __syncthreads();
        auto wide_stage = [&](u32 (&r)[8][4]) {
#pragma unroll
            for (int s = 0; s < 3; s++) {
                const int jl = INV ? s : 2 - s;
#pragma unroll
                for (int b = 0; b < 4; b++) {
                    const int q0 = ((b >> jl) << (jl + 1)) | (b & ((1 << jl) - 1));
                    u32 w = TW(jl, (8 * r4 + q0) >> (jl + 1));
#pragma unroll
                    for (int j = 0; j < 4; j++) bfly<INV>(r[q0][j], r[q0 | (1 << jl)][j], w);
                }
            }
        };
        auto narrow_task = [&](u32 id, bool from_global, bool to_global) {
            u32 l = id & (C - 1), mlow = id >> CL;
            u32 v[16];
#pragma unroll
            for (int e = 0; e < 16; e++) {
                u32 m = 8 * e + mlow;
                v[e] = from_global ? __builtin_nontemporal_load(src + ((base | (m << lo) | l) & a.src_mask)) : s_val[C * m + l];
            }
            radix16<INV>(v, 4, [&](int jl, int pe) -> u32 { return TW(3 + jl, pe); });
#pragma unroll
            for (int e = 0; e < 16; e++) {
                u32 m = 8 * e + mlow;
                if (to_global) __builtin_nontemporal_store((INV && a.scale != 1) ? m_mul_pow2(v[e], scale_shift(a.scale)) : v[e], dst + (base | (m << lo) | l));
                else s_val[C * m + l] = v[e];
            }
        };
        if (INV) {
            u32 r[8][4];
#pragma unroll
            for (int q = 0; q < 8; q++) { uint4 v = ld16_stream(src + ((base | ((8 * r4 + q) << lo) | l4) & a.src_mask)); r[q][0] = v.x; r[q][1] = v.y; r[q][2] = v.z; r[q][3] = v.w; }
            wide_stage(r);
#pragma unroll
            for (int q = 0; q < 8; q++) *reinterpret_cast<uint4*>(&s_val[C * (8 * r4 + q) + l4]) = make_uint4(r[q][0], r[q][1], r[q][2], r[q][3]);
            __syncthreads();
            narrow_task(t, false, true);
            narrow_task(t + NT, false, true);
        } else {
            narrow_task(t, true, false);
            __builtin_amdgcn_sched_barrier(0);
            narrow_task(t + NT, true, false);
            __syncthreads();
            u32 r[8][4];
#pragma unroll
            for (int q = 0; q < 8; q++) { uint4 v = *reinterpret_cast<uint4*>(&s_val[C * (8 * r4 + q) + l4]); r[q][0] = v.x; r[q][1] = v.y; r[q][2] = v.z; r[q][3] = v.w; }
            wide_stage(r);
#pragma unroll
            for (int q = 0; q < 8; q++) st16(dst + (base | ((8 * r4 + q) << lo) | l4), make_uint4(r[q][0], r[q][1], r[q][2], r[q][3]));
        }
    }
}

template <bool INV, class TW> __device__ __forceinline__ void radix16_range(u32 (&v)[16], int jl_lo, TW tw) {
#pragma unroll
    for (int s = 0; s < 4; s++) {
        const int jl = INV ? s : 3 - s;
        if (jl >= jl_lo) {
#pragma unroll
            for (int b = 0; b < 8; b++) {
                const int e0 = ((b >> jl) << (jl + 1)) | (b & ((1 << jl) - 1));
                bfly<INV>(v[e0], v[e0 | (1 << jl)], tw(jl, e0 >> (jl + 1)));
            }
        }
    }
}
template <bool INV, int K, int CL>
__global__ void __launch_bounds__((1 << (K + CL)) / 32) k_fft_stridedK(const PassArgs* __restrict__ groups, u32 ngroups) {
    constexpr u32 C = 1u << CL, ROWS = 1u << K, CELLS = ROWS * C, NT = CELLS / 32;
    constexpr int NR = (K + 3) / 4;
    const BlockOfGroup bg = find_group(groups, ngroups);
    const PassArgs a = groups[bg.g];
    __shared__ __attribute__((aligned(16))) u32 s_val[CELLS];
    __shared__ u32 s_tw[ROWS];
    const u32 t = threadIdx.x, lo = a.lo, tile = bg.tile;
    const u32 n_lhi_log = lo - CL;
    const u32 H = tile >> n_lhi_log, Lhi = tile & ((1u << n_lhi_log) - 1);
    const u32 base = (H << (lo + K)) | (Lhi << CL);
    for (u32 e = t; e < ROWS - 1; e += NT) {
        const u32 j = __clz(~(e << (32 - K)));
        const u32 q = e - (ROWS - (ROWS >> j));
        s_tw[e] = 2u * layer_table(a, lo + j)[(H << (K - 1 - j)) + q];
    }
    auto TW = [&](u32 layer, u32 idx) -> u32 { return s_tw[ROWS - (ROWS >> layer) + idx]; };
    const u32 col0 = bg.by * a.cols_per_block, col1 = min(a.ncols, col0 + a.cols_per_block);
    for (u32 col = col0; col < col1; col++) {
        g_cu32p src = as_global(a.src[col]);
        g_u32p dst = as_global(a.dst[col]);
        __syncthreads();
#pragma unroll
        for (u32 i = 0; i < 8; i++) {
            const u32 idx = 4 * (t + NT * i), m = idx >> CL, l = idx & (C - 1);
            const uint4 v = ld16_stream(src + ((base | (m << lo) | l) & a.src_mask));
            *reinterpret_cast<uint4*>(&s_val[idx]) = v;
        }
        __syncthreads();
#pragma unroll
        for (int rr = 0; rr < NR; rr++) {
            const int r = INV ? rr : NR - 1 - rr;
            const int b = (4 * r + 4 <= K) ? 4 * r : K - 4;
            const int jl_lo = 4 * r - b;
#pragma unroll
            for (u32 g2 = 0; g2 < 2; g2++) {
                const u32 id = t + NT * g2, l = id & (C - 1), rest = id >> CL;
                const u32 rest_lo = rest & ((1u << b) - 1), rest_hi = rest >> b;
                const u32 m0 = (rest_hi << (b + 4)) | rest_lo;
                u32 v[16];
#pragma unroll
                for (int e = 0; e < 16; e++) v[e] = s_val[((m0 | ((u32)e << b)) << CL) | l];
                radix16_range<INV>(v, jl_lo, [&](int jl, int pe) -> u32 { return TW(b + jl, (rest_hi << (3 - jl)) + pe); });
#pragma unroll
                for (int e = 0; e < 16; e++) s_val[((m0 | ((u32)e << b)) << CL) | l] = v[e];
            }
            __syncthreads();
        }
#pragma unroll
        for (u32 i = 0; i < 8; i++) {
            const u32 idx = 4 * (t + NT * i), m = idx >> CL, l = idx & (C - 1);
            uint4 v = *reinterpret_cast<uint4*>(&s_val[idx]);
            if (INV && a.scale != 1) { const u32 sk = scale_shift(a.scale); v.x = m_mul_pow2(v.x, sk); v.y = m_mul_pow2(v.y, sk); v.z = m_mul_pow2(v.z, sk); v.w = m_mul_pow2(v.w, sk); }
            st16(dst + (base | (m << lo) | l), v);
        }
    }
}

template <bool INV>
__device__ __forceinline__ void fft_tiny_body(const PassArgs& a, const BlockOfGroup& bg) {
    const u32 n = 1u << a.log, wave = threadIdx.x >> 6, lane = threadIdx.x & 63u, i = lane & (n - 1);
    const u32 col = (bg.tile * (blockDim.x >> 6) + wave) * (64u >> a.log) + (lane >> a.log);
    const bool act = col < a.ncols;
    u32 v = act ? a.src[col][i & a.src_mask] : 0u;
    u32 tw[5];
#pragma unroll
    for (u32 j = 0; j < 5; j++) {
        tw[j] = 1u;
        if (j < a.k) {
            const u32 h = i >> (j + 1);
            if (a.circle && j == 0) {
                const u32* l0 = layer_table(a, 1);
                const u32 x = l0[(h >> 2) * 2], y = l0[(h >> 2) * 2 + 1], sel = h & 3;
                tw[j] = sel == 0 ? y : sel == 1 ? m_neg(y) : sel == 2 ? m_neg(x) : x;
            } else tw[j] = layer_table(a, j)[h];
        }
    }
#pragma unroll
    for (u32 jj = 0; jj < 5; jj++) {
        if (jj >= a.k) break;
        const u32 j = INV ? jj : a.k - 1 - jj;
        const u32 other = (u32)__shfl_xor((int)v, 1 << j);
        const bool hi = (i >> j) & 1u;
        const u32 x = hi ? other : v, y = hi ? v : other;
        u32 t = 0;
#pragma unroll
        for (u32 q = 0; q < 5; q++) if (q == j) t = tw[q];
        if (INV) v = hi ? m_mul(m_sub(x, y), t) : m_add(x, y);
        else { const u32 w = m_mul(y, t); v = hi ? m_sub(x, w) : m_add(x, w); }
    }
    if (act) a.dst[col][i] = INV ? m_mul(v, a.scale) : v;
}
template <bool INV>
__global__ void __launch_bounds__(256) k_fft_tiny(const PassArgs* __restrict__ groups, u32 ngroups) {
    const BlockOfGroup bg = find_group(groups, ngroups);
    const PassArgs a = groups[bg.g];
    fft_tiny_body<INV>(a, bg);
}


void fft_plan(FftPlan& plan, bool inverse, const FftJob* jobs, size_t njobs, const u32* tw, const u32* itw, u32 tw_root_log) {
    plan.inverse = inverse; plan.groups.clear(); plan.launches.clear(); plan.d_groups = nullptr;
    struct Item { int pi, kind; PassArgs a; double bytes, alg; bool single = false; double bfly() const { return 0.5 * a.ncols * (double)(1u << a.log) * a.k; } };
    std::vector<Item> items;
    int max_np = 0;
    for (size_t ji = 0; ji < njobs; ji++) {
        const FftJob& job = jobs[ji];
        const u32 ncols = job.ncols, log = job.log, src_log = job.src_log;
        if (ncols == 0) continue;
        PassArgs a{};
        a.ncols = ncols; a.log = log; a.circle = job.circle ? 1 : 0; a.tw = inverse ? itw : tw; a.tw_total = 1u << tw_root_log; a.scale = 1;
        const u32 nl = inverse ? log : (log > 5 && src_log < 2) ? 2u : src_log;
        if (log <= 5) {
            a.dst = job.d_dst; a.src = job.d_src; a.src_mask = (1u << src_log) - 1; a.lo = 0; a.k = nl;
            a.scale = inverse ? m_inv(1u << log) : 1;
            a.grid_x = (ncols + (256u >> log) - 1) / (256u >> log); a.cols_per_block = 1;
            items.push_back({0, K_TINY, a, 0.0, 0.0, true});
            max_np = std::max(max_np, 1);
            continue;
        }
        if (log >= 12 && nl >= 6) {
            u32 ns = nl > 12 ? (nl - 12 + 6) / 7 : 0;
            u32 k0 = nl - 7 * ns;
            static const bool two_pass = [] { const char* v = getenv("BFHIP_FFT_TWO_PASS"); return !v || v[0] != '0'; }();
            const u32 big_k = (two_pass && nl >= 20 && nl <= 22) ? nl - 12 : 0;
            if (big_k) { ns = 1; k0 = 12; }
            int np = 1 + (int)ns;
            max_np = std::max(max_np, np);
            const double alg = 4.0 * ncols * ((double)(1u << src_log) + (double)(1u << log)) / np;
            for (int pi = 0; pi < np; pi++) {
                int p = inverse ? pi : np - 1 - pi;
                bool first = pi == 0, last = pi == np - 1;
                a.src = first ? job.d_src : (const u32* const*)job.d_dst;
                a.dst = job.d_dst;
                a.src_mask = first ? ((1u << src_log) - 1) : 0xffffffffu;
                a.scale = (inverse && last) ? m_inv(1u << log) : 1;
                u32 ntiles = 1u << (log - 12);
                u32 cpb = ncols;
                while (cpb > 1 && (u64)ntiles * ((ncols + cpb - 1) / cpb) < 2048) cpb = (cpb + 1) / 2;
                a.cols_per_block = cpb;
                const u32 gy = (ncols + cpb - 1) / cpb;
                const double bytes = 8.0 * ncols * (double)(1u << log);
                if (p == 0) {
                    a.lo = 0; a.k = k0; a.tile_log = 12; a.grid_x = ntiles;
                    PassArgs b = a; b.block0 = gy;
                    items.push_back({pi, K_TILE12, b, bytes, alg});
                } else if (big_k) {
                    a.lo = 12; a.k = big_k;
                    const u32 cl = big_k == 10 ? 4 : 5;
                    PassArgs b = a; b.grid_x = 1u << (log - big_k - cl); b.block0 = gy;
                    items.push_back({pi, big_k == 8 ? K_STRIDED_K8 : big_k == 9 ? K_STRIDED_K9 : K_STRIDED_K10, b, bytes, alg});
                } else {
                    a.lo = k0 + 7 * (p - 1); a.k = 7;
#ifndef BF_STRIDED_WIDE_MIN_LOG
#define BF_STRIDED_WIDE_MIN_LOG 20
#endif
                    const bool wide = a.lo >= 6 && log >= BF_STRIDED_WIDE_MIN_LOG;
                    PassArgs b = a; b.grid_x = wide ? ntiles / 2 : ntiles; b.block0 = gy;
                    items.push_back({pi, wide ? K_STRIDED6 : K_STRIDED5, b, bytes, alg});
                }
            }
            continue;
        }
        u32 bounds[8]; int np = 0;
        bounds[0] = 0;
        a.tile_log = log < (u32)TILE_LOG ? log : (u32)TILE_LOG;
        u32 k0 = nl < a.tile_log ? nl : a.tile_log;
        bounds[++np] = k0;
        while (bounds[np] < nl) {
            u32 rem = nl - bounds[np];
            u32 passes_left = (rem + STRIDED_K - 1) / STRIDED_K;
            u32 kk = (rem + passes_left - 1) / passes_left;
            bounds[np + 1] = bounds[np] + kk; np++;
        }
        max_np = std::max(max_np, np);
        const double alg = 4.0 * ncols * ((double)(1u << src_log) + (double)(1u << log)) / np;
        for (int pi = 0; pi < np; pi++) {
            int p = inverse ? pi : np - 1 - pi;
            bool first = pi == 0, last = pi == np - 1;
            a.lo = bounds[p]; a.k = bounds[p + 1] - bounds[p];
            u32 tl = a.lo == 0 ? a.tile_log : a.k + CHUNK_LOG;
            u32 ntiles = 1u << (log - tl);
            a.src = first ? job.d_src : (const u32* const*)job.d_dst;
            a.dst = job.d_dst;
            a.src_mask = first ? ((1u << src_log) - 1) : 0xffffffffu;
            a.scale = (inverse && last) ? m_inv(1u << log) : 1;
            u32 cpb = 1;
            while ((u64)ntiles * ((ncols + cpb - 1) / cpb) > 8192 && cpb < ncols) cpb *= 2;
            a.cols_per_block = cpb;
            PassArgs b = a; b.grid_x = ntiles; b.block0 = (ncols + cpb - 1) / cpb;
            items.push_back({pi, K_PASS, b, 8.0 * ncols * (double)(1u << log), alg, np == 1 && log < (u32)TILE_LOG});
        }
    }
    {
        static const bool fuse = [] { const char* v = getenv("BFHIP_FFT_FUSE_SMALL"); return !v || v[0] != '0'; }();
        int host_pi = -1;
        for (auto& it : items) if (it.kind == K_TILE12 && (host_pi < 0 || it.pi < host_pi)) host_pi = it.pi;
        if (fuse && host_pi >= 0)
            for (auto& it : items)
                if (it.single && (it.kind == K_PASS || it.kind == K_TINY)) { it.a.kind = (u32)it.kind; it.kind = K_TILE12; it.pi = host_pi; }
    }
    for (int pi = 0; pi < max_np; pi++)
        for (int kind = 0; kind < K_KINDS; kind++) {
            FftLaunch L{}; L.kind = kind; L.first_group = (u32)plan.groups.size();
            u32 blocks = 0;
            for (auto& it : items) {
                if (it.pi != pi || it.kind != kind) continue;
                PassArgs a = it.a;
                const u32 gy = (kind == K_TINY || a.kind == K_TINY) ? 1u : a.block0;
                a.block0 = blocks; blocks += a.grid_x * gy;
                plan.groups.push_back(a);
                L.bytes += it.bytes; L.alg += it.alg; L.bfly += it.bfly();
            }
            L.ngroups = (u32)plan.groups.size() - L.first_group; L.total_blocks = blocks;
            if (L.ngroups) plan.launches.push_back(L);
        }
}

static const char* fft_prof_name(const char* base, const FftLaunch& L) {
    static const bool detail = [] { const char* v = getenv("BFHIP_FFT_PROF_DETAIL"); return v && v[0] == '1'; }();
    if (!detail) return base;
    static std::mutex mu; static std::set<std::string> names;
    std::lock_guard<std::mutex> g(mu);
    return names.insert(std::string(base) + "/b" + std::to_string(L.total_blocks) + "/g" + std::to_string(L.ngroups)).first->c_str();
}

void fft_run(hipStream_t stream, const FftPlan& plan) {
    if (plan.launches.empty()) return;
    if (!plan.d_groups) throw std::runtime_error("fft_run: the plan's group table has not been staged");
    const bool inverse = plan.inverse;
    for (const FftLaunch& L : plan.launches) {
        const PassArgs* g = plan.d_groups + L.first_group;
        const dim3 grid(L.total_blocks);
        switch (L.kind) {
            case K_TILE12: {
                ProfScope ps(stream, fft_prof_name(inverse ? "k_fft_tile12<true>" : "k_fft_tile12<false>", L), L.bytes, L.alg, false, L.bfly);
                static const u32 generic = [] { const char* v = getenv("BFHIP_FFT_TILE12_GENERIC"); return (v && v[0] == '1') ? 1u : 0u; }();
                if (inverse) hipLaunchKernelGGL(k_fft_tile12<true>, grid, dim3(256), 0, stream, g, L.ngroups, generic);
                else hipLaunchKernelGGL(k_fft_tile12<false>, grid, dim3(256), 0, stream, g, L.ngroups, generic);
                break; }
            case K_STRIDED5: {
                ProfScope ps(stream, fft_prof_name(inverse ? "k_fft_strided7<true>" : "k_fft_strided7<false>", L), L.bytes, L.alg, false, L.bfly);
                if (inverse) hipLaunchKernelGGL((k_fft_strided7<true, 5>), grid, dim3(128), 0, stream, g, L.ngroups);
                else hipLaunchKernelGGL((k_fft_strided7<false, 5>), grid, dim3(128), 0, stream, g, L.ngroups);
                break; }
            case K_STRIDED6: {
                ProfScope ps(stream, fft_prof_name(inverse ? "k_fft_strided7<true>" : "k_fft_strided7<false>", L), L.bytes, L.alg, false, L.bfly);
                if (inverse) hipLaunchKernelGGL((k_fft_strided7<true, 6>), grid, dim3(256), 0, stream, g, L.ngroups);
                else hipLaunchKernelGGL((k_fft_strided7<false, 6>), grid, dim3(256), 0, stream, g, L.ngroups);
                break; }
            case K_STRIDED_K8: {
                ProfScope ps(stream, fft_prof_name(inverse ? "k_fft_stridedK<true>" : "k_fft_stridedK<false>", L), L.bytes, L.alg, false, L.bfly);
                if (inverse) hipLaunchKernelGGL((k_fft_stridedK<true, 8, 5>), grid, dim3(256), 0, stream, g, L.ngroups);
                else hipLaunchKernelGGL((k_fft_stridedK<false, 8, 5>), grid, dim3(256), 0, stream, g, L.ngroups);
                break; }
            case K_STRIDED_K9: {
                ProfScope ps(stream, fft_prof_name(inverse ? "k_fft_stridedK<true>" : "k_fft_stridedK<false>", L), L.bytes, L.alg, false, L.bfly);
                if (inverse) hipLaunchKernelGGL((k_fft_stridedK<true, 9, 5>), grid, dim3(512), 0, stream, g, L.ngroups);
                else hipLaunchKernelGGL((k_fft_stridedK<false, 9, 5>), grid, dim3(512), 0, stream, g, L.ngroups);
                break; }
            case K_STRIDED_K10: {
                ProfScope ps(stream, fft_prof_name(inverse ? "k_fft_stridedK<true>" : "k_fft_stridedK<false>", L), L.bytes, L.alg, false, L.bfly);
                if (inverse) hipLaunchKernelGGL((k_fft_stridedK<true, 10, 4>), grid, dim3(512), 0, stream, g, L.ngroups);
                else hipLaunchKernelGGL((k_fft_stridedK<false, 10, 4>), grid, dim3(512), 0, stream, g, L.ngroups);
                break; }
            case K_PASS: {
                ProfScope ps(stream, fft_prof_name(inverse ? "k_fft_pass<true>" : "k_fft_pass<false>", L), L.bytes, L.alg, false, L.bfly);
                if (inverse) hipLaunchKernelGGL(k_fft_pass<true>, grid, dim3(FFT_THREADS), 0, stream, g, L.ngroups);
                else hipLaunchKernelGGL(k_fft_pass<false>, grid, dim3(FFT_THREADS), 0, stream, g, L.ngroups);
                break; }
            default:
                if (inverse) hipLaunchKernelGGL(k_fft_tiny<true>, grid, dim3(256), 0, stream, g, L.ngroups);
                else hipLaunchKernelGGL(k_fft_tiny<false>, grid, dim3(256), 0, stream, g, L.ngroups);
        }
    }
}

void gen_twiddles(hipStream_t stream, u32* d_tw, u32* d_itw, u32 R, const uint2* d_tlo, const uint2* d_thi) {
    u32 total = 1u << R;
    hipLaunchKernelGGL(k_gen_twiddles, dim3((total + 255) / 256), dim3(256), 0, stream, d_tw, d_itw, R, d_tlo, d_thi);
}

}
```

stwo-brainfuck_amd/csrc/kernels.h:

```cpp
#pragma once
#include <hip/hip_runtime.h>
#include "m31.h"
#include "air.h"
#include <string>
#include <vector>

struct bfhip_trace;

namespace bf {

struct ColDesc { const u32* ptr; u32 shift; u32 pad_; };

int prof_mode(hipStream_t s);
void prof_enable(hipStream_t s, int mode);
void prof_run_begin(hipStream_t s, const char* name);
void prof_run_end(hipStream_t s);
void prof_begin(hipStream_t s, const char* name, double bytes, double units, double aux = 0.0);
void prof_end(hipStream_t s);
void prof_reset(hipStream_t s);
std::string prof_report_json(const hipStream_t* streams, int n);
void prof_forget(hipStream_t s);
struct ProfScope {
    hipStream_t s; bool on;
    ProfScope(hipStream_t s_, const char* name, double bytes, double units = 0.0, bool dominant = false, double aux = 0.0) : s(s_) {
        int m = prof_mode(s);
        on = m == 1 || (m == 2 && dominant);
        if (on) prof_begin(s, name, bytes, units, aux);
    }
    ~ProfScope() { if (on) prof_end(s); }
};

#if defined(__HIPCC__)
#define BF_GLOBAL __attribute__((address_space(1)))
typedef u32 bf_u32x4 __attribute__((ext_vector_type(4)));
typedef BF_GLOBAL u32* g_u32p;
typedef const BF_GLOBAL u32* g_cu32p;
__device__ __forceinline__ g_cu32p as_global(const u32* p) { return (g_cu32p)(unsigned long long)p; }
__device__ __forceinline__ g_u32p as_global(u32* p) { return (g_u32p)(unsigned long long)p; }
__device__ __forceinline__ uint4 ld16(g_cu32p p) { bf_u32x4 v = *(const BF_GLOBAL bf_u32x4*)p; return make_uint4(v.x, v.y, v.z, v.w); }
__device__ __forceinline__ uint4 ld16_stream(g_cu32p p) { bf_u32x4 v = __builtin_nontemporal_load((const BF_GLOBAL bf_u32x4*)p); return make_uint4(v.x, v.y, v.z, v.w); }
__device__ __forceinline__ void st16(g_u32p p, uint4 v) { bf_u32x4 w = {v.x, v.y, v.z, v.w}; __builtin_nontemporal_store(w, (BF_GLOBAL bf_u32x4*)p); }
#define BF_CONSTANT __attribute__((address_space(4)))
template <class T> __device__ __forceinline__ T ld_constant(const T* p) {
    static_assert(sizeof(T) % 4 == 0 && alignof(T) >= 4, "word-sized parameter blocks only");
    T out;
    const BF_CONSTANT u32* s = (const BF_CONSTANT u32*)(unsigned long long)p;
#pragma unroll
    for (u32 i = 0; i < sizeof(T) / 4; i++) reinterpret_cast<u32*>(&out)[i] = s[i];
    return out;
}
__device__ __forceinline__ u32 ld_col(const ColDesc& d, u32 i) {
    const u32 byte_off = (i >> d.shift) << 2;
    return *(g_cu32p)((const BF_GLOBAL char*)(unsigned long long)d.ptr + byte_off);
}
#endif

void gen_twiddles(hipStream_t stream, u32* d_tw, u32* d_itw, u32 R, const uint2* d_tlo, const uint2* d_thi);
struct FftJob { const u32* const* d_src; u32* const* d_dst; u32 ncols, log, src_log; bool circle; };
struct PassArgs {
    u32* const* dst;
    const u32* const* src;
    u32 ncols, cols_per_block;
    u32 log;
    u32 lo, k;
    u32 tile_log;
    u32 src_mask;
    u32 circle;
    u32 scale;
    u32 tw_total;
    const u32* tw;
    u32 block0, grid_x;
    u32 kind;
};
struct FftLaunch { int kind; u32 first_group, ngroups, total_blocks; double bytes, alg, bfly; };
struct FftPlan { bool inverse = false; std::vector<PassArgs> groups; std::vector<FftLaunch> launches; const PassArgs* d_groups = nullptr; };
void fft_plan(FftPlan& plan, bool inverse, const FftJob* jobs, size_t njobs, const u32* tw, const u32* itw, u32 tw_root_log);
void fft_run(hipStream_t stream, const FftPlan& plan);

struct IsFirstCols { u32* ptr[28]; u32 log_min, log_max; };
void is_first_coeffs(hipStream_t stream, const IsFirstCols& a, const u32* itw, u32 tw_root_log);
void is_first_lde(hipStream_t stream, const IsFirstCols& a, u32 log_blowup, const u32* tw, const u32* itw, u32 tw_root_log);
struct IsFirstSample { u32 log_n, point, out_idx; };
void is_first_samples(hipStream_t stream, const IsFirstSample* d_jobs, u32 n_jobs, const void* d_factors, void* d_out, const u32* itw, u32 tw_root_log);

void merkle_layer(hipStream_t stream, void* out, const void* prev, const ColDesc* d_cols, u32 ncols, u32 log, double col_bytes, u32 out_shift, u32 prev_shift,
                  u32 node_conv, u32 first = 0, u32 count = 0);
struct MerkleTreeDesc { uint4* layers[32]; u32 shifts[32]; u32 col_off[32]; const ColDesc* cols; u32 n_cols, max_log; };
static constexpr u32 MERKLE_SUBTREE_ROOT_LEVEL = 9;
void merkle_subtree(hipStream_t stream, const MerkleTreeDesc& tree, u32 hi, u32 node_conv, double bytes, double compressions);
void merkle_subtree_share(hipStream_t stream, const MerkleTreeDesc& tree, u32 hi, u32 stop, u32 lo, u32 wg0, u32 n_wg, u32 node_conv, double bytes, double compressions);
void merkle_top(hipStream_t stream, const MerkleTreeDesc& tree, u32 top_hi, u32 node_conv, u32* d_chan, u32* d_alpha8, u32* d_root_copy, double bytes, double compressions,
                u32* d_stamp = nullptr, u32 stamp_value = 0);
struct FriTailLayer {
    u32* ev[4];
    const u32* quot[4];
    uint4* tree[11];
};
struct FriTailArgs {
    u32 n_layers, top_log;
    u32 alpha_idx, root_idx;
    u32* ev_last[4];
    u32* chan; u32* alpha; u32* roots;
    const u32* itw; u32 tw_total, rfc;
    FriTailLayer layer[10];
};
void fri_tail(hipStream_t stream, const FriTailArgs* d_args, double bytes, double compressions);
struct FriLayerArgs {
    const u32* src[4]; const u32* quot[4]; u32* dst[4]; uint4* tree[18];
    const u32* alpha8; const u32* itw; u32 tw_total, log, rfc, pad_;
    u32* counter; u32* chan; u32* alpha_out; u32* root_out;
};
void fri_layer(hipStream_t stream, const FriLayerArgs& a);
enum FriFoldMode : int { FF_LINE = 0, FF_LINE_CIRCLE = 1, FF_CIRCLE = 2 };
struct FriFoldLeafArgs { const u32* src[4]; const u32* quot[4]; u32* dst[4]; const u32* alpha8; const u32* itw; u32 tw_total, log; };
void fri_fold_leaf(hipStream_t stream, void* out, const FriFoldLeafArgs& a, int mode, u32 node_conv);
void grind_span(hipStream_t stream, const u32* d_digest, u64 base, u32 span, u32 pow_bits, unsigned long long* d_best, u32 mix_u64_conv);
void clock_probe_launch(hipStream_t stream, uint4* d_stamps, u32* d_sink, u32 blocks, u32 iters);
void clock_sampler_launch(hipStream_t stream, uint4* d_out, const u32* d_stop_alias, unsigned long long max_ticks);
void fill_mix(hipStream_t stream, u32* p, size_t n);
void channel_mix_root_draw(hipStream_t stream, u32* d_chan, const u32* d_root, u32* d_alpha8, u32* d_root_copy);

void merkle_layer_poseidon(hipStream_t stream, void* out, const void* prev, const ColDesc* d_cols, u32 ncols, u32 log, u32 out_shift = 0, u32 prev_shift = 0,
                           u32 first = 0, u32 count = 0);
void hades_once(hipStream_t stream, const u32* d_in24, u32* d_out24);
void grind_poseidon_span(hipStream_t stream, const u32* d_digest, u64 base, u32 span, u32 pow_bits, unsigned long long* d_best);

struct ConstraintLaunch {
    const u32* is_first; ColDesc trace[13]; ColDesc inter[12]; u32* acc[4]; Q31 coeff[12]; Lookups el; Q31 total_sum; u32 denom_inv[2]; u32 log_size;
    u32 overwrite;
    u32 row0, n_rows;
    const u32* inter_prev[4];
};
void eval_constraints(hipStream_t stream, int comp, const ConstraintLaunch* d_args, u32 log_size, u32 n_rows = 0, u32 group_rows = 0);
u32 constraint_group_rows(const ConstraintLaunch& L, int comp);
struct ConstraintClass { u32 n_comps, block0, group_rows, pad_; u32 comp[13]; u32 pad2_[3]; };
struct ConstraintBatch { u32 n_classes, total_blocks, pad_[2]; ConstraintClass cls[13]; };
void constraint_batch_init(ConstraintBatch& b, const ConstraintLaunch* launches, u32 n);
void eval_constraints_batch(hipStream_t stream, const ConstraintBatch* d_batch, const ConstraintBatch& h_batch, const ConstraintLaunch* d_args);
struct LogupLaunch {
    const u32* cols[13];
    u32* out_rep[8];
    u32* out_last[4];
    void* vrow; void* wloc; void* totals; void* claimed;
    Lookups el; u32 log_rows; int comp;
};
struct LogupItem { const u32* cols[13]; u32* out_rep[8]; u32* out_last[4]; uint4* vrow; uint4* wloc; uint4* totals; uint4* claimed; u32 log_rows; int comp; u32 nb; u32 pad_; };
struct LogupBatch { Lookups el; u32 n; u32 rows_blk0[14], scan_blk0[14], last_blk0[14]; u32 pad_; LogupItem item[13]; };
void logup_batch_init(LogupBatch& b, const Lookups& el, const LogupLaunch* L, u32 n);
void logup_batch_run(hipStream_t stream, const LogupBatch* d_batch, const LogupBatch& h_batch);
void broadcast16(hipStream_t stream, const u32* d_rows, u32* d_out, u32 n_cells);

struct CheckReportDev { u64 n_bad_cells, first_bad_cell; u64 bad_per_constraint[16]; u32 first_bad_constraint; u32 first_bad_value[4]; u32 pad_[3]; };
struct CheckLaunch { ColDesc trace[13]; ColDesc inter[12]; Lookups el; Q31 total_sum; u32 log_size; u32 pad_; CheckReportDev* report; };
void check_constraints_launch(hipStream_t stream, int comp, const CheckLaunch* d_args, u32 log_size);
struct CheckReadback { CheckReportDev report[N_COMPONENTS]; uint4 claimed[N_COMPONENTS]; uint4 total; };
struct CheckBatch { u32 blk0[N_COMPONENTS + 1]; u32 pad_[2]; CheckReadback* out; };
void check_batch_init(CheckBatch& b, const u32 log_sizes[N_COMPONENTS], CheckReadback* d_out);
void check_batch_run(hipStream_t stream, const CheckBatch* d_batch, const CheckBatch& h_batch, const CheckLaunch* d_launches);

// ... 34 lines not shown
```

stwo-brainfuck_amd/csrc/prover.h:

```cpp
#pragma once
#include "../../include/bfhip.h"
#include "ctx.h"
#include "host/circle.h"
#include "host/quotients.h"
#include "host/proof.h"
#include <chrono>
#include <functional>
#include <map>
#include <string>
#include <vector>

namespace bf {

void build_tables_device(Ctx& c, const std::vector<u32> trace7_soa[7], u32 n, const std::vector<u32>& code, const std::function<u32*(size_t)>& alloc,
                         std::vector<std::vector<u32*>>& cols_out, u32 log_sizes_out[13]);
void build_tables_device(Ctx& c, const TraceSoA& t, const std::vector<u32>& code, const std::function<u32*(size_t)>& alloc,
                         std::vector<std::vector<u32*>>& cols_out, u32 log_sizes_out[13]);

static constexpr u32 OWNER_ALL = 0xFFFFFFFFu;

struct DCol {
    u32* ptr = nullptr; u32 log_size = 0; u32 shift = 0;
    u32 lc = 0;
    bool sliced() const { return lc != 0; }
    size_t stored() const { return size_t(1) << (log_size - shift - lc); }
    ColDesc desc() const { return ColDesc{ptr, shift, 0}; }
    bool mine(u64 cell, u32 rank) const { return lc == 0 || (cell >> (log_size - lc)) == rank; }
};
struct DevMerkle { std::vector<u32*> layers; std::vector<u32> shifts; u32 max_log = 0; Hash32 root; int band_lo = 0, band_hi = -1; std::vector<DCol> cols; };
struct DTree { std::vector<DCol> polys, evals, prev; std::vector<u32> owner; DevMerkle mk; bool is_first_closed = false; };
struct DSecure {
    u32* c[4]; u32 log_size; u32 lc = 0;
    bool mine(u64 cell, u32 rank) const { return lc == 0 || (cell >> (log_size - lc)) == rank; }
};

struct Gather {
    std::vector<GatherReq> reqs;
    u32 n_words = 0;
    size_t add(const u32* base, u64 idx, bool mine = true) { reqs.push_back({mine ? base : nullptr, idx, n_words, 1u}); n_words += 1; return n_words - 1; }
    size_t add_hash(const u32* layer, u64 node_slot, bool mine) { reqs.push_back({mine ? layer : nullptr, node_slot * 8, n_words, 8u}); n_words += 8; return n_words - 8; }
    size_t add_col(const DCol& col, u64 cell, u32 rank) { return add(col.ptr, cell >> col.shift, col.mine(cell, rank)); }
    std::vector<u32> run(Ctx& c, int stamp_slot = -1);
};

struct TraceInput {
    std::vector<std::vector<DCol>> rows;
    u32 log_sizes[N_COMPONENTS];
    u64 n_steps = 0, main_cells = 0, interaction_cells = 0;
    std::vector<u32*> owned;
    void release() { for (u32* p : owned) (void)hipFree(p); owned.clear(); rows.clear(); }
};

struct PreprocessedCache {
    bool enabled = false, valid = false, replicate = false; u32 lmr = 0, node_conv = 0, channel = 0, log_blowup = 0, shard_rank = 0, shard_count = 1; DTree tree; Arena keep;
    bool matches(const Ctx& c, u32 log_max_rows) const {
        return enabled && valid && lmr == log_max_rows && node_conv == c.conv.merkle_node_hash && channel == c.conv.merkle_channel && log_blowup == c.pcs.log_blowup &&
               shard_rank == c.shard.rank && shard_count == c.shard.count && replicate == (c.shard.count > 1 && c.shard_replicate);
    }
};

struct SharedPreprocessed {
    bool valid = false; u32 lmr = 0, node_conv = 0, channel = 0, log_blowup = 0;
    DTree tree;
    hipEvent_t ready = nullptr;
    const Hash32* pinned_root = nullptr;
    u32 root_slot = 0;
    bool matches(const Ctx& c, u32 log_max_rows) const {
        return valid && lmr == log_max_rows && node_conv == c.conv.merkle_node_hash && channel == c.conv.merkle_channel && log_blowup == c.pcs.log_blowup &&
               c.shard.count == 1;
    }
};

inline CheckReportDev check_report_init() { CheckReportDev r{}; r.first_bad_cell = ~u64(0); r.first_bad_constraint = 0xffffffffu; return r; }
inline void check_report_fill(bfhip_check_report& out, const CheckReportDev& r, int component, u32 log_size, Q31 claimed) {
    out = bfhip_check_report{};
    out.component = (u32)component; out.log_size = log_size;
    out.n_bad_cells = r.n_bad_cells; out.first_bad_cell = r.first_bad_cell; out.first_bad_constraint = (int32_t)r.first_bad_constraint;
    for (int w = 0; w < 4; w++) out.first_bad_value[w] = r.first_bad_value[w];
    for (int j = 0; j < 16; j++) out.bad_per_constraint[j] = r.bad_per_constraint[j];
    out.claimed_sum[0] = claimed.a.a; out.claimed_sum[1] = claimed.a.b; out.claimed_sum[2] = claimed.b.a; out.claimed_sum[3] = claimed.b.b;
}
inline CheckLaunch check_launch_of(int component, u32 log_size, const u32* const* main_rows, const u32* const* logup_cols, const Lookups& el, Q31 total_sum,
                                   CheckReportDev* d_report) {
    CheckLaunch L{};
    const u32 n_inter = 4 * n_logup_cols(component);
    for (u32 j = 0; j < n_main_cols(component); j++) L.trace[j] = ColDesc{main_rows[j], LOG_N_LANES, 0};
    for (u32 j = 0; j < n_inter; j++) L.inter[j] = ColDesc{logup_cols[j], j + 4 < n_inter ? LOG_N_LANES : 0u, 0};
    L.el = el; L.total_sum = total_sum; L.log_size = log_size; L.report = d_report;
    return L;
}
inline Lookups default_check_lookups() {
    Lookups el;
    Channel ch;
    { Q31 z, a; ch.draw_two_felts(z, a); el.memory = make_lookup(z, a); }
    { Q31 z, a; ch.draw_two_felts(z, a); el.instruction = make_lookup(z, a); }
    { Q31 z, a; ch.draw_two_felts(z, a); el.processor = make_lookup(z, a); }
    return el;
}

inline void sync_both(Ctx& c) { c.sync(); if (c.stream2) BF_HIP(hipStreamSynchronize(c.stream2)); for (auto a : c.aux) if (a) BF_HIP(hipStreamSynchronize(a)); }

struct PhaseTimes { double preprocessed = 0, main_trace = 0, interaction = 0, composition = 0, oods = 0, quotients = 0, fri = 0, decommit = 0, tables = 0, total = 0; };

struct HipProver {
    Ctx& c;
    PcsConfig cfg;
    u32 log_max_rows;
    Channel ch;
    PhaseTimes tm;
    std::string transcript;
    bool want_transcript = false;

    HipProver(Ctx& ctx, u32 lmr) : c(ctx), cfg(ctx.pcs), log_max_rows(lmr) {}

    void tap(const char* name);
    static double now() { return std::chrono::duration<double>(std::chrono::steady_clock::now().time_since_epoch()).count(); }
    std::vector<std::pair<const char*, double>> host_marks;
    bool trace_host = [] { const char* v = getenv("BFHIP_TRACE_HOST"); return v && (v[0] == '1' || v[0] == '2'); }();
    bool trace_host_mean = [] { const char* v = getenv("BFHIP_TRACE_HOST"); return v && v[0] == '2'; }();
    double mark_t0 = 0;
    void mark(const char* label) { if (trace_host) host_marks.push_back({label, (now() - mark_t0) * 1e6}); }
    void print_marks();
    void check_config() const;
    BrainfuckProof prove(const TraceInput& in) { return prove([&]() -> const TraceInput& { return in; }); }
    BrainfuckProof prove(const std::function<const TraceInput&()>& get_input);
    void preflight(const TraceInput& in);

    FftPlan fft_prepare(bool inverse, const std::vector<DCol>& src, const std::vector<DCol>& dst);
    void fft_launch(const FftPlan& plan);
    void fft_cols(bool inverse, const std::vector<DCol>& src, const std::vector<DCol>& dst);
    template <class F> void stage_blocks(Mailbox* mbx, F&& f) {
        if (mbx) { mbx->begin(); f(); mbx->arm(); }
        else { StageBatch sb(c); f(); sb.end(); }
    }

    struct ChannelStep { u32* chan; u32* alpha8; u32* root_copy; };
    struct MerklePlan {
        DevMerkle mk; std::vector<DCol> cols; std::vector<size_t> off; std::vector<double> bytes; size_t n_all = 0;
        const ColDesc* d_all = nullptr; MerkleTreeDesc tree{}; bool poseidon = false;
        u32 fused_top = 0, sub_hi = 0;
        double top_bytes = 0, top_comp = 0, sub_bytes = 0, sub_comp = 0;
        int band_fuse_hi = -1; u32 band_fuse_r = 0; double band_bytes = 0, band_comp = 0;
        bool folded_leaves = false; FriFoldLeafArgs fold{}; int fold_mode = -1;
    };
    MerklePlan merkle_plan(const std::vector<DCol>& cols_in, bool folded_leaves = false);
    struct LevelWait { int level; hipEvent_t ev; };
    DevMerkle merkle_run(MerklePlan& p, Hash32* pinned_root = nullptr, bool no_readback = false, const ChannelStep* step = nullptr, const std::vector<LevelWait>* waits = nullptr,
                         int stamp_slot = -1, bool* stamped = nullptr);
    DevMerkle merkle_commit(const std::vector<DCol>& cols_in, Hash32* pinned_root = nullptr, bool no_readback = false, const ChannelStep* step = nullptr);

    static constexpr u32 SLICE_MIN_LOG_PER_RANK = 14;
    static constexpr u32 SHARE_MIN_LOG_PER_RANK = 14;
    bool sharded() const { return c.shard.count > 1; }
    u32 lc() const { return c.shard.log_count; }
    bool slice_log(u32 log) const { return sharded() && log >= lc() + SLICE_MIN_LOG_PER_RANK; }
    bool replicate() const { return sharded() && c.shard_replicate; }
    bool transforms_here(u32 owner) const { return owner == OWNER_ALL || owner == c.shard.rank || replicate(); }
    bool slice_col(u32 log, u32 shift) const { return sharded() && log >= shift + lc() + SLICE_MIN_LOG_PER_RANK; }
    size_t slice_cells(u32 log) const { return size_t(1) << (log - lc()); }
    size_t slice_first(u32 log) const { return (size_t)c.shard.rank << (log - lc()); }
    u32* alloc_slice(u32 log, u32 shift = 0);
    std::vector<u32> assign_owners(const std::vector<DCol>& polys, u32 log_blowup) const;
    void commit_tree(DTree& t, Hash32* pinned_root = nullptr, bool with_prev = false);
    void commit_tree_overlapped(DTree& t, Hash32* pinned_root, const std::vector<DCol>* interp_src = nullptr, int stamp_slot = -1, bool evals_ready = false);
    static void upload_trace(Ctx& c, const std::vector<Registers>& vm_trace, const std::vector<u32>& code, TraceInput& in, bool use_arena = false, bool on_gpu = true);
    static void upload_registers(Ctx& c, const u32* trace7_h, size_t n_rows, const u32* code_words_h, size_t n_code, TraceInput& in, bool use_arena, bool with_place);
    void build_preprocessed(DTree& tree, Hash32* pinned_root);
    void build_shared_preprocessed(SharedPreprocessed& sp);

    struct CompositionPlan {
        std::vector<ConstraintLaunch> launches; std::vector<DSecure> acc; std::vector<bool> have; u32 total = 0, max_log = 0;
        ConstraintLaunch* h_staged = nullptr;
    };
    CompositionPlan composition_prepare(std::vector<DTree>& trees, const BrainfuckProof& bp, const size_t* main_off, const size_t* inter_off, const Lookups& el);
    static void composition_challenge_fields(const BrainfuckProof& bp, u32 total, Q31 random_coeff, ConstraintLaunch* launches);
    void composition_fill(const BrainfuckProof& bp, CompositionPlan& cp, Q31 random_coeff);
    void compute_composition(std::vector<DTree>& trees, const BrainfuckProof& bp, CompositionPlan& cp, Q31 random_coeff, Mailbox* mbx = nullptr);
    struct SamplePlan { std::vector<EvalJob> jobs; std::vector<IsFirstSample> isf; u32 partial_off = 0, n_all = 0; };
    SamplePlan sample_prepare(const std::vector<DTree>& trees, const std::vector<std::vector<std::vector<u32>>>& mask);
    static void sample_factors(const std::vector<PtQ>& points, uint4* factors);
    struct SampleRun { uint4* h_factors = nullptr; uint4* d_out = nullptr; };
    SampleRun sample_launch(const SamplePlan& sp, const std::vector<PtQ>& points, Mailbox* mbx);
    const uint4* sample_results() const { return reinterpret_cast<const uint4*>(c.h_small + 4096); }
    void sample_unpack(const std::vector<DTree>& trees, const std::vector<std::vector<std::vector<u32>>>& mask, const uint4* out, u32 n_all, StarkProof& pf);
    void sample(const std::vector<DTree>& trees, const std::vector<std::vector<std::vector<u32>>>& mask, const std::vector<PtQ>& points, StarkProof& pf, const SamplePlan& sp);
    struct QuotientGroup {
        u32 log = 0; std::vector<ColDesc> descs; std::vector<ColSamples> cols; std::vector<std::pair<size_t, size_t>> src;
        QuotientBatch* h_batches = nullptr; QuotientEntry* h_entries = nullptr; size_t n_batches = 0, n_entries = 0;
    };
    struct QuotientRun { std::vector<QuotientGroup> groups; std::vector<DSecure> out; };
    std::vector<QuotientGroup> quotient_groups(const std::vector<DTree>& trees, const std::vector<std::vector<std::vector<u32>>>& mask);
    static void quotient_constants(QuotientGroup& g, const std::vector<PtQ>& points, const StarkProof* pf, Q31 random_coeff,
                                   std::vector<QuotientBatch>& batches, std::vector<QuotientEntry>& entries);
    QuotientRun compute_quotients(const std::vector<DTree>& trees, const std::vector<std::vector<std::vector<u32>>>& mask, const std::vector<PtQ>& points,
                                  const StarkProof* pf, Q31 random_coeff, std::vector<LevelWait>* q_waits, Mailbox* mb0 = nullptr, Mailbox* mb1 = nullptr);
    void quotients_fill(QuotientRun& qr, const std::vector<PtQ>& points, const StarkProof& pf, Q31 random_coeff, Mailbox* mb0, Mailbox* mb1);

    typedef std::function<void(const std::vector<u32>&)> Finisher;
    Finisher decommit(Gather& g, const DevMerkle& mk, const std::vector<DCol>& cols_in, const std::map<u32, std::vector<size_t>>& queries_per_log,
                      std::vector<u32>* queried_values, MerkleDecommitment* dec);
    static std::vector<size_t> fold_queries(const std::vector<size_t>& q, u32 n);
    static void positions_and_witness(const std::vector<size_t>& queries, std::vector<size_t>& positions, std::vector<size_t>& witness_pos);
    Finisher gather_secure_deferred(Gather& g, const DSecure& s, const std::vector<size_t>& pos, std::vector<Q31>* out);
    static std::vector<DCol> secure_cols(const DSecure& s);
    enum : u32 { FRI_BY_LAUNCHES = 0, FRI_BY_FOLD_LEAF = 1, FRI_BY_LAYER_KERNEL = 2, FRI_BY_TAIL = 3, FRI_QUOTIENT = 4, FRI_NO_TREE = 15 };
    static constexpr size_t FRI_MAX_LAYERS = 40;
    struct FriCommitted {
        struct Inner { DSecure ev; DevMerkle tree; }; DevMerkle first_tree; std::vector<DCol> first_cols; std::vector<Inner> inner;
        std::vector<DSecure> layers; std::vector<u32> path; u32* d_alpha = nullptr; u32* d_chan = nullptr;
    };
    FriCommitted fri_commit(std::vector<DSecure>& quotients, StarkProof& pf, const std::vector<LevelWait>& q_waits, const std::function<void()>& while_the_commit_phase_runs,
// ... 9 lines not shown
```

stwo-brainfuck_amd/csrc/prover.hip:

```cpp
#include <atomic>
#include "prover.h"
#include "host/verifier.h"
#include <algorithm>
#include <cstdio>
#include <mutex>
#include <thread>

namespace bf {

void HipProver::tap(const char* name) {
    if (!want_transcript) return;
    char buf[3]; transcript += name; transcript += ':';
    for (int i = 0; i < 32; i++) { snprintf(buf, sizeof buf, "%02x", ch.digest.b[i]); transcript += buf; }
    transcript += '\n';
}
void HipProver::print_marks() {
    if (!trace_host) return;
    if (trace_host_mean) {
        static std::mutex mu; static std::vector<std::pair<const char*, double>> sum; static int n = 0;
        std::lock_guard<std::mutex> g(mu);
        if (sum.size() != host_marks.size()) { sum.assign(host_marks.size(), {nullptr, 0.0}); n = 0; }
        double prev = 0;
        for (size_t i = 0; i < host_marks.size(); i++) { sum[i].first = host_marks[i].first; sum[i].second += host_marks[i].second - prev; prev = host_marks[i].second; }
        if (++n == 20) {
// ... 164 lines not shown
                    trees[1].polys[i].ptr = c.alloc_u32(trees[1].polys[i].stored());
                    s_mine.push_back(src[i]); p_mine.push_back(trees[1].polys[i]);
                }
                fft_cols(true, s_mine, p_mine);
                commit_tree(trees[1], pinned_root1);
            } else {
                for (auto& p : trees[1].polys) p.ptr = c.alloc_u32(p.stored());
                commit_tree_overlapped(trees[1], pinned_root1, &src, mb ? 1 : -1);
            }
        }
        BF_HIP(hipEventRecord(c.ev[2], c.stream));
        mark("main tree enqueued");
        prepare_logup();
        if (mb) {
            h_lb = enqueue_interaction(Lookups{}, &mb_logup);
            mark("interaction phase enqueued behind its mailbox");
            c.wait_stamp(1);
        } else c.sync();
        mark("main root arrived");
    } catch (...) { join_side(); throw; }
    join_side();
    mark("side stream joined");
    if (shared) {
        const auto w0 = std::chrono::steady_clock::now();
        for (u32 polls = 0;; polls++) {
            hipError_t e = hipEventQuery(shared->ready);
            if (e == hipSuccess) break;
            if (e != hipErrorNotReady) BF_HIP(e);
            if (polls > 64) std::this_thread::yield();
            if ((polls & 1023u) == 1023u && std::chrono::duration<double>(std::chrono::steady_clock::now() - w0).count() > 120.0)
                throw HipError("pool: the batch's shared preprocessed commitment did not complete");
        }
        trees[0].mk.root = *shared->pinned_root;
        mark("shared preprocessed tree ready");
    }
    if (!reuse) {
        trees[0].mk.root = *pinned_root0;
        if (cache.enabled) {
            cache.tree = trees[0]; cache.lmr = log_max_rows; cache.node_conv = c.conv.merkle_node_hash; cache.channel = c.conv.merkle_channel; cache.log_blowup = cfg.log_blowup;
            cache.shard_rank = c.shard.rank; cache.shard_count = c.shard.count; cache.replicate = replicate(); cache.valid = true;
        }
    }
    trees[1].mk.root = *pinned_root1;
    ch.mix_root(trees[0].mk.root);
    tap("root0");
    for (int k = 0; k < N_COMPONENTS; k++) ch.mix_u64(bp.log_sizes[k]);
    ch.mix_root(trees[1].mk.root);
    tap("root1");
    const double wall_phase01 = now() - t0;

    t0 = now();
    Lookups el;
    { Q31 z, a; ch.draw_two_felts(z, a); el.memory = make_lookup(z, a); }
    { Q31 z, a; ch.draw_two_felts(z, a); el.instruction = make_lookup(z, a); }
    { Q31 z, a; ch.draw_two_felts(z, a); el.processor = make_lookup(z, a); }
    mark("lookup elements drawn");
    auto take_claimed = [&](const uint4* h_claimed) {
        for (int k = 0; k < N_COMPONENTS; k++) bp.claimed_sums[k] = q_make(h_claimed[k].x, h_claimed[k].y, h_claimed[k].z, h_claimed[k].w);
        for (int k = 0; k < N_COMPONENTS; k++) ch.mix_felts(&bp.claimed_sums[k], 1);
    };
    std::vector<std::vector<std::vector<u32>>> mask(4);
    auto build_mask = [&]() {
        mask[0].assign(trees[0].polys.size(), {});
        for (int k = 0; k < N_COMPONENTS; k++) mask[0][log_max_rows - bp.log_sizes[k]] = {0};
        for (int k = 0; k < N_COMPONENTS; k++) {
            for (u32 j = 0; j < n_main_cols(k); j++) mask[1].push_back({0});
            u32 ni = 4 * n_logup_cols(k);
            for (u32 j = 0; j < ni; j++) {
                if (j + 4 >= ni) { if (c.conv.logup_mask_order == 1) mask[2].push_back({(u32)(1 + k), 0}); else mask[2].push_back({0, (u32)(1 + k)}); }
                else mask[2].push_back({0});
            }
        }
        mask[3].assign(4, {0});
    };
    Hash32* pinned_root3 = reinterpret_cast<Hash32*>(c.h_small + 2368);
    Q31 random_coeff;
    if (mb) {
        h_lb->el = el;
        mb_logup.post();
        mark("lookup elements posted");
        composition_plan = composition_prepare(trees, bp, main_off, inter_off, el);
        compute_composition(trees, bp, composition_plan, q_zero(), &mb_constraints);
        build_mask();
        commit_tree_overlapped(trees[3], pinned_root3, nullptr, 3);
        sample_plan = sample_prepare(trees, mask);
        mark("composition phase enqueued behind its mailbox");
        c.wait_stamp(2);
        mark("interaction root arrived");
        take_claimed(pinned_claimed);
        trees[2].mk.root = *pinned_root2;
        ch.mix_root(trees[2].mk.root);
        tap("root2");
        tm.interaction = now() - t0;
        t0 = now();
        random_coeff = ch.draw_felt();
        composition_fill(bp, composition_plan, random_coeff);
        mb_constraints.post();
        mark("random coefficient posted");
    } else {
        enqueue_interaction(el, nullptr);
        if (sharded()) {
            uint4 h_claimed[N_COMPONENTS];
            c.read_back(h_claimed, d_claimed, sizeof(h_claimed));
            take_claimed(h_claimed);
            std::vector<DCol> mine_cols;
            for (size_t i = 0; i < inter_vals.size(); i++) if (kept(i)) mine_cols.push_back(inter_vals[i]);
            fft_cols(true, mine_cols, mine_cols);
            commit_tree(trees[2], nullptr, true);
        } else {
            composition_plan = composition_prepare(trees, bp, main_off, inter_off, el);
            mark("interaction tree enqueued + composition prepared");
            c.sync();
            mark("interaction root arrived");
            take_claimed(pinned_claimed);
            trees[2].mk.root = *pinned_root2;
            ch.mix_root(trees[2].mk.root);
        }
        tap("root2");
        tm.interaction = now() - t0;

        t0 = now();
        random_coeff = ch.draw_felt();
        if (sharded()) composition_plan = composition_prepare(trees, bp, main_off, inter_off, el);
        compute_composition(trees, bp, composition_plan, random_coeff);
        mark("constraints + composition transforms launched");
        build_mask();
        if (sharded()) commit_tree(trees[3]);
        else {
            commit_tree_overlapped(trees[3], pinned_root3);
            sample_plan = sample_prepare(trees, mask);
            mark("composition tree enqueued + samples prepared");
        }
    }

    std::vector<PtQ> points(1 + N_COMPONENTS);
    PtQ oods;
    auto draw_oods = [&]() {
        Q31 t = ch.draw_felt();
        Q31 t2 = q_mul(t, t);
        Q31 d = q_inv(q_addm(t2, 1));
        oods.x = q_mul(q_sub(q_one(), t2), d);
        oods.y = q_mul(q_add(t, t), d);
        points[0] = oods;
        for (int k = 0; k < N_COMPONENTS; k++) points[1 + k] = pq_add(oods, pq_neg(to_q(index_to_point(subgroup_gen(bp.log_sizes[k])))));
    };
    auto mix_samples = [&]() {
        std::vector<Q31> flat;
        for (auto& t : bp.proof.sampled_values) for (auto& col : t) for (auto& v : col) flat.push_back(v);
        ch.mix_felts(flat.data(), flat.size());
    };
    std::vector<LevelWait> q_waits;
    std::vector<DSecure> quotients;
    if (mb) {
        const SampleRun sr = sample_launch(sample_plan, points, &mb_samples);
        c.post_stamp(4);
        mark("sampling enqueued behind its mailbox");
        c.wait_stamp(3);
        mark("composition root arrived");
        trees[3].mk.root = *pinned_root3;
        ch.mix_root(trees[3].mk.root);
        tap("root3");
        tm.composition = now() - t0;
        t0 = now();
        draw_oods();
        sample_factors(points, sr.h_factors);
        mb_samples.post();
        mark("out-of-domain point posted");
        QuotientRun qr = compute_quotients(trees, mask, points, nullptr, q_one(), nullptr, &mb_quot0, &mb_quot1);
        BF_HIP(hipEventRecord(c.ev[5], c.stream));
        quotients = qr.out;
        mark("quotients enqueued behind their mailboxes");
        c.wait_stamp(4);
        sample_unpack(trees, mask, sample_results(), sample_plan.n_all, bp.proof);
        mark("sampled values arrived");
        mix_samples();
        tap("sampled");
        tm.oods = now() - t0;
        t0 = now();
        Q31 q_coeff = ch.draw_felt();
        mark("sampled values mixed, quotient coefficient drawn");
        quotients_fill(qr, points, bp.proof, q_coeff, &mb_quot0, &mb_quot1);
        mark("quotient constants posted");
    } else {
        if (!sharded()) {
            c.sync();
            mark("composition root arrived");
            trees[3].mk.root = *pinned_root3;
            ch.mix_root(trees[3].mk.root);
        }
        tap("root3");
        tm.composition = now() - t0;
        t0 = now();
        draw_oods();
        if (sharded()) sample_plan = sample_prepare(trees, mask);
        sample(trees, mask, points, bp.proof, sample_plan);
        mark("sampled values arrived");
        mix_samples();
        tap("sampled");
        tm.oods = now() - t0;

        t0 = now();
        Q31 q_coeff = ch.draw_felt();
        mark("sampled values mixed, quotient coefficient drawn");
        BF_HIP(hipEventRecord(c.ev[4], c.stream));
        quotients = compute_quotients(trees, mask, points, &bp.proof, q_coeff, &q_waits).out;
        BF_HIP(hipEventRecord(c.ev[5], c.stream));
        mark("quotients launched");
    }


    auto mailbox_gave_up = [&]() { for (int k = 1; k <= 5; k++) if (c.mailbox_err_host()[2 * k]) return true; return false; };
    const char* mailbox_msg = "a mailbox kernel gave up waiting for the host (BFHIP_MAILBOX_TIMEOUT_MS): the proof was computed from stale challenge words";
// ... 47 lines not shown
```

stwo-brainfuck_amd/csrc/prover_commit.hip:

```cpp
#include "prover.h"
#include <algorithm>

namespace bf {

#ifdef BFHIP_TEST_HOOKS
struct PolyCapture {
    struct Poly { u32 log_size, shift; std::vector<u32> stored; };
    bool on = false; int saved_mailbox_mode = -1;
    std::vector<std::vector<Poly>> trees;
};
static void capture_tree(Ctx& c, const DTree& t) {
    if (!c.capture || !c.capture->on) return;
    c.capture->trees.emplace_back();
    auto& out = c.capture->trees.back();
    out.resize(t.polys.size());
    for (size_t i = 0; i < t.polys.size(); i++) {
        const DCol& p = t.polys[i];
        if (!p.ptr || p.sliced()) throw HipError("bfhip_test_capture_polys: a polynomial this rank does not hold whole");
        out[i].log_size = p.log_size; out[i].shift = p.shift; out[i].stored.resize(p.stored());
        BF_HIP(hipMemcpyAsync(out[i].stored.data(), p.ptr, p.stored() * sizeof(u32), hipMemcpyDeviceToHost, c.stream));
    }
}
#endif

FftPlan HipProver::fft_prepare(bool inverse, const std::vector<DCol>& src, const std::vector<DCol>& dst) {
    std::map<std::pair<u32, u32>, std::vector<size_t>> groups;
    for (size_t i = 0; i < dst.size(); i++) groups[{dst[i].log_size, dst[i].shift}].push_back(i);
    struct Job { size_t off, n; u32 log, src_log, sh; };
    std::vector<Job> jobs; std::vector<const u32*> ptrs;
    for (auto it = groups.rbegin(); it != groups.rend(); ++it) {
        const auto& idx = it->second;
        u32 log = it->first.first, sh = it->first.second;
        std::map<u32, std::vector<size_t>> by_src;
        for (size_t i : idx) by_src[src[i].log_size].push_back(i);
        for (auto& kv : by_src) {
            jobs.push_back({ptrs.size(), kv.second.size(), log, kv.first, sh});
            for (size_t i : kv.second) ptrs.push_back(src[i].ptr);
            for (size_t i : kv.second) ptrs.push_back(dst[i].ptr);
        }
    }
    FftPlan plan;
    if (jobs.empty()) return plan;
    StageBatch sb(c);
    const u32* const* d_ptrs = c.stage(ptrs.data(), ptrs.size());
    std::vector<FftJob> fj;
    for (auto& j : jobs) fj.push_back({d_ptrs + j.off, (u32* const*)(d_ptrs + j.off + j.n), (u32)j.n, j.log - j.sh, j.src_log - j.sh, j.sh == 0});
    fft_plan(plan, inverse, fj.data(), fj.size(), c.d_tw, c.d_itw, c.tw_root_log);
    plan.d_groups = c.stage(plan.groups.data(), plan.groups.size());
    sb.end();
    return plan;
}
void HipProver::fft_launch(const FftPlan& plan) { fft_run(c.stream, plan); BF_HIP(hipGetLastError()); }
void HipProver::fft_cols(bool inverse, const std::vector<DCol>& src, const std::vector<DCol>& dst) {
    c.stage_checkpoint();
    fft_launch(fft_prepare(inverse, src, dst));
}

HipProver::MerklePlan HipProver::merkle_plan(const std::vector<DCol>& cols_in, bool folded_leaves) {
    if (cols_in.empty()) throw HipError("merkle_commit: no columns");
    MerklePlan p;
    p.cols = cols_in;
    std::vector<DCol>& cols = p.cols;
    std::stable_sort(cols.begin(), cols.end(), [](const DCol& a, const DCol& b) { return a.log_size > b.log_size; });
    DevMerkle& mk = p.mk;
    mk.cols = cols;
    mk.max_log = cols[0].log_size;
    mk.layers.resize(mk.max_log + 1);
    mk.shifts.assign(mk.max_log + 1, 0);
    u32 min_col_log = cols.back().log_size;
    std::vector<ColDesc> all; p.off.assign(mk.max_log + 2, 0); p.bytes.assign(mk.max_log + 1, 0.0);
    {
        size_t ci = 0;
        for (int log = (int)mk.max_log; log >= 0; log--) {
            p.off[log] = all.size();
            u32 sh = log < (int)mk.max_log ? (mk.shifts[log + 1] ? mk.shifts[log + 1] - 1 : 0) : 32;
            while (ci < cols.size() && cols[ci].log_size == (u32)log) { sh = std::min(sh, cols[ci].shift); p.bytes[log] += 4.0 * cols[ci].stored(); all.push_back(cols[ci++].desc()); }
            mk.shifts[log] = std::min<u32>(sh == 32 ? 0 : sh, (u32)log);
        }
    }
    p.n_all = all.size();
    p.poseidon = c.conv.merkle_channel == 1;
    (void)min_col_log;
    u32 fused_top = std::min<u32>(mk.max_log + 1, 10);
    while (fused_top > 0 && mk.shifts[std::min(fused_top, mk.max_log)] != 0) fused_top--;
    if (p.poseidon) fused_top = 0;
    p.fused_top = fused_top;
    const ShardGroup& sg = c.shard;
    if (sg.count > 1) {
        const int share_min = p.poseidon ? 8 : (int)SHARE_MIN_LOG_PER_RANK;
        int lo = std::max<int>((int)sg.log_count + share_min, (int)fused_top);
        while (lo <= (int)mk.max_log && (int)lo - (int)mk.shifts[lo] < (int)sg.log_count + share_min) lo++;
        const bool worth = (int)mk.max_log - (int)mk.shifts[mk.max_log] >= (int)sg.log_count + (int)SLICE_MIN_LOG_PER_RANK;
        if (worth && lo <= (int)mk.max_log) { mk.band_hi = (int)mk.max_log; mk.band_lo = lo; }
        for (auto& col : cols) if (col.sliced() && ((int)col.log_size < mk.band_lo || (int)col.log_size > mk.band_hi)) throw HipError("shard group: a row-sharded column lies outside the share-wise Merkle band");
    }
    const bool banded = mk.band_hi >= mk.band_lo;
    for (int log = (int)mk.max_log; log >= 0; log--) {
        const size_t stored = (size_t(1) << log) >> mk.shifts[log];
        if (banded && log > mk.band_lo && log <= mk.band_hi) {
            const size_t per_rank = stored >> sg.log_count;
            mk.layers[log] = reinterpret_cast<u32*>(reinterpret_cast<uintptr_t>(c.arena.alloc(32 * per_rank)) - 32 * per_rank * sg.rank);
        } else mk.layers[log] = (u32*)c.arena.alloc(32 * stored);
    }
    if (fused_top == 10 && mk.max_log >= 11) {
        u32 hi = std::min<u32>(banded ? (u32)mk.band_lo - 1 : mk.max_log, 17);
        if (folded_leaves && hi == mk.max_log) hi--;
        while (hi > 10 && mk.shifts[hi] != 0) hi--;
        if (hi > 10) { p.sub_hi = hi; p.fused_top = fused_top = MERKLE_SUBTREE_ROOT_LEVEL; }
    }
    auto level_cols = [&](int log) { return (log > 0 ? p.off[log - 1] : all.size()) - p.off[log]; };
    auto level_cost = [&](int log, double& bytes, double& comp) {
        const double nodes = (double)(1u << log), nc = (double)level_cols(log);
        const bool has = log < (int)mk.max_log;
        bytes += nodes * ((has ? 64.0 : 0.0) + 32.0) + p.bytes[log];
        comp += nodes * ((has ? 1.0 : 0.0) + (double)(((u32)nc + 15) / 16) + ((!has && nc == 0) ? 1.0 : 0.0));
    };
    if (banded && !p.poseidon && fused_top > 0 && mk.band_hi > mk.band_lo && c.shard.band_fusion) {
        const int hi = std::min(mk.band_hi, mk.band_lo + 3);
        bool plain = true;
        for (int lg = mk.band_lo; lg <= std::min(hi + 1, (int)mk.max_log); lg++) plain = plain && mk.shifts[lg] == 0;
        const u32 r = 8 - (u32)(hi - mk.band_lo);
        if (plain && (u32)mk.band_lo >= sg.log_count + r) {
            p.band_fuse_hi = hi; p.band_fuse_r = r;
            for (int lg = hi; lg >= mk.band_lo; lg--) level_cost(lg, p.band_bytes, p.band_comp);
            p.band_bytes /= sg.count; p.band_comp /= sg.count;
        }
    }
    for (int log = (int)fused_top - 1; log >= 0; log--) level_cost(log, p.top_bytes, p.top_comp);
    if (p.sub_hi) for (int log = (int)p.sub_hi; log >= (int)MERKLE_SUBTREE_ROOT_LEVEL; log--) level_cost(log, p.sub_bytes, p.sub_comp);
    p.d_all = all.empty() ? nullptr : c.stage(all.data(), all.size());
// ... 135 lines not shown
        }
        if (recvs.empty()) return;
        if (comm_stream != c.stream) { BF_HIP(hipEventRecord(after_copies, c.stream)); BF_HIP(hipStreamWaitEvent(comm_stream, after_copies, 0)); }
        c.shard.comm->exchange(comm_stream, sends, recvs);
    };
    std::vector<size_t> owned;
    u32 big = 0;
    for (size_t i = 0; i < n; i++) if (t.owner[i] != OWNER_ALL && !replicate()) { owned.push_back(i); big = std::max(big, t.evals[i].log_size); }
    std::vector<size_t> first_wave, second_wave;
    for (size_t i : owned) (t.evals[i].log_size == big ? first_wave : second_wave).push_back(i);
    if (sharded() && c.exchange_overlapped() && !second_wave.empty() && c.aux[0]) {
        std::vector<DCol> sa, da, sb2, db2;
        {
            size_t k = 0;
            for (size_t i = 0; i < n; i++) {
                const bool mine = t.owner[i] == OWNER_ALL || t.owner[i] == c.shard.rank;
                if (!mine) continue;
                const bool wave_a = t.owner[i] != OWNER_ALL && t.evals[i].log_size == big;
                (wave_a ? sa : sb2).push_back(fsrc[k]); (wave_a ? da : db2).push_back(fdst[k]);
                k++;
            }
        }
        c.stage_checkpoint();
        FftPlan pa = fft_prepare(false, sa, da), pb = fft_prepare(false, sb2, db2);
        try {
            fft_launch(pa);
            exchange_columns(c.aux[0], first_wave, c.next_event());
            fft_launch(pb);
            exchange_columns(c.aux[0], second_wave, c.next_event());
            hipEvent_t done = c.next_event();
            BF_HIP(hipEventRecord(done, c.aux[0]));
            BF_HIP(hipStreamWaitEvent(c.stream, done, 0));
        } catch (...) {
            (void)hipStreamSynchronize(c.aux[0]);
            throw;
        }
    } else {
        fft_cols(false, fsrc, fdst);
        if (sharded() && !replicate()) exchange_columns(c.stream, owned, nullptr);
    }
    BF_HIP(hipGetLastError());
    t.mk = merkle_commit(t.evals, pinned_root);
    if (!pinned_root) ch.mix_root(t.mk.root);
#ifdef BFHIP_TEST_HOOKS
    capture_tree(c, t);
#endif
}

void HipProver::commit_tree_overlapped(DTree& t, Hash32* pinned_root, const std::vector<DCol>* interp_src, int stamp_slot, bool evals_ready) {
    const size_t n = t.polys.size();
    t.owner.assign(n, OWNER_ALL);
    if (evals_ready) {
        if (interp_src || t.evals.size() != n) throw HipError("commit_tree_overlapped: ready evaluations do not match the tree");
        t.prev.assign(n, DCol());
        c.stage_checkpoint();
        StageBatch sb(c);
        MerklePlan mp = merkle_plan(t.evals);
        sb.end();
        bool stamped = false;
        t.mk = merkle_run(mp, pinned_root, false, nullptr, nullptr, stamp_slot, &stamped);
        if (stamp_slot >= 0 && !stamped) c.post_stamp(stamp_slot);
        if (!pinned_root) ch.mix_root(t.mk.root);
#ifdef BFHIP_TEST_HOOKS
        capture_tree(c, t);
#endif
        return;
    }
    t.evals.resize(n); t.prev.assign(n, DCol());
    u32 max_log = 0;
    for (size_t i = 0; i < n; i++) {
        DCol e; e.log_size = t.polys[i].log_size + cfg.log_blowup; e.shift = t.polys[i].shift; e.ptr = c.alloc_u32(e.stored());
        t.evals[i] = e; max_log = std::max(max_log, e.log_size);
    }
    std::vector<DCol> src[2], pol[2], ev[2];
    u32 next_log = 0;
    for (size_t i = 0; i < n; i++) {
        const int w = t.evals[i].log_size == max_log ? 0 : 1;
        if (interp_src) src[w].push_back((*interp_src)[i]);
        pol[w].push_back(t.polys[i]); ev[w].push_back(t.evals[i]);
        if (w) next_log = std::max(next_log, t.evals[i].log_size);
    }
    const bool overlap = (c.overlap & 1u) && !ev[1].empty() && max_log >= 19;
    c.stage_checkpoint();
    FftPlan fi[2], fe[2];
    MerklePlan mp;
    {
        StageBatch sb(c);
        for (int w = 0; w < 2; w++) {
            if (interp_src) fi[w] = fft_prepare(true, src[w], pol[w]);
            fe[w] = fft_prepare(false, pol[w], ev[w]);
        }
        mp = merkle_plan(t.evals);
        sb.end();
    }
    hipStream_t main = c.stream, aux = c.aux_of(main);
    if (interp_src) fft_launch(fi[0]);
    fft_launch(fe[0]);
    if (!overlap) {
        if (interp_src) fft_launch(fi[1]);
        fft_launch(fe[1]);
        bool stamped = false;
        t.mk = merkle_run(mp, pinned_root, false, nullptr, nullptr, stamp_slot, &stamped);
        if (stamp_slot >= 0 && !stamped) c.post_stamp(stamp_slot);
    } else {
        hipEvent_t e1 = c.next_event(), e2 = c.next_event(), e3 = c.next_event();
        BF_HIP(hipEventRecord(e1, main));
        if (interp_src) fft_launch(fi[1]);
        fft_launch(fe[1]);
        BF_HIP(hipEventRecord(e2, main));
        BF_HIP(hipStreamWaitEvent(aux, e1, 0));
        std::vector<LevelWait> waits = {{(int)next_log, e2}};
        c.stream = aux;
        try { t.mk = merkle_run(mp, nullptr, true, nullptr, &waits); } catch (...) { c.stream = main; (void)hipStreamSynchronize(aux); throw; }
        c.stream = main;
        BF_HIP(hipEventRecord(e3, aux));
        BF_HIP(hipStreamWaitEvent(main, e3, 0));
        if (pinned_root) BF_HIP(hipMemcpyAsync(pinned_root->b, t.mk.layers[0], 32, hipMemcpyDeviceToHost, main));
        else c.read_back(t.mk.root.b, t.mk.layers[0], 32);
        if (stamp_slot >= 0) c.post_stamp(stamp_slot);
    }
    if (!pinned_root) ch.mix_root(t.mk.root);
#ifdef BFHIP_TEST_HOOKS
    capture_tree(c, t);
#endif
}

void HipProver::upload_trace(Ctx& c, const std::vector<Registers>& vm_trace, const std::vector<u32>& code, TraceInput& in, bool use_arena, bool on_gpu) {
    c.refuse_in_session("trace upload");
    in.rows.assign(N_COMPONENTS, {});
    in.n_steps = vm_trace.size();
    in.main_cells = in.interaction_cells = 0;
    auto alloc = [&](size_t words) -> u32* {
        if (use_arena) return c.alloc_u32(words);
        u32* p = nullptr; BF_HIP(hipMalloc((void**)&p, (words ? words : 1) * sizeof(u32))); in.owned.push_back(p); return p;
    };
    if (on_gpu) {
        std::vector<u32> soa[7];
        size_t n = vm_trace.size();
        for (auto& v : soa) v.resize(n);
        for (size_t i = 0; i < n; i++) { const Registers& r = vm_trace[i]; soa[0][i] = r.clk; soa[1][i] = r.ip; soa[2][i] = r.ci; soa[3][i] = r.ni; soa[4][i] = r.mp; soa[5][i] = r.mv; soa[6][i] = r.mvi; }
        std::vector<std::vector<u32*>> cols;
        build_tables_device(c, soa, (u32)n, code, alloc, cols, in.log_sizes);
        for (int k = 0; k < N_COMPONENTS; k++)
            for (u32 j = 0; j < n_main_cols(k); j++) { DCol r; r.log_size = in.log_sizes[k]; r.shift = LOG_N_LANES; r.ptr = cols[k][j]; in.rows[k].push_back(r); }
    } else {
        std::vector<Table> tables = build_tables(vm_trace, code);
        for (int k = 0; k < N_COMPONENTS; k++) {
            in.log_sizes[k] = tables[k].log_size();
            for (u32 j = 0; j < n_main_cols(k); j++) {
                DCol r; r.log_size = in.log_sizes[k]; r.shift = LOG_N_LANES;
                r.ptr = alloc(r.stored());
                BF_HIP(hipMemcpyAsync(r.ptr, tables[k].cols[j].data(), r.stored() * sizeof(u32), hipMemcpyHostToDevice, c.stream));
                in.rows[k].push_back(r);
            }
        }
    }
    for (int k = 0; k < N_COMPONENTS; k++) {
        in.main_cells += (u64)n_main_cols(k) << in.log_sizes[k];
        in.interaction_cells += (u64)(4 * n_logup_cols(k)) << in.log_sizes[k];
    }
    c.sync();
}

void HipProver::upload_registers(Ctx& c, const u32* trace7_h, size_t n_rows, const u32* code_words_h, size_t n_code, TraceInput& in, bool use_arena, bool with_place) {
    auto bad_register = [&](size_t row, int reg) {
        std::string m = "register value is not a canonical M31";
        if (with_place) m += " (row " + std::to_string(row) + ", register " + std::to_string(reg) + ")";
        return HipError(m);
    };
    c.refuse_in_session("trace upload");
    auto check_code = [&]() {
        std::vector<u32> ins(code_words_h, code_words_h + n_code);
        for (u32 w : ins) if (w >= P31) throw HipError("program word is not a canonical M31");
        return ins;
    };
    if (!c.tables_on_gpu) {
        std::vector<Registers> tr(n_rows);
        for (size_t i = 0; i < n_rows; i++) {
            const u32* v = trace7_h + 7 * i;
            for (int k = 0; k < 7; k++) if (v[k] >= P31) throw bad_register(i, k);
            tr[i] = Registers{v[0], v[1], v[2], v[3], v[4], v[5], v[6]};
        }
        upload_trace(c, tr, check_code(), in, use_arena, false);
        return;
    }
    c.stage_checkpoint();
    u64 first_bad = ~u64(0);
    TraceSoA t = ingest_registers(c, trace7_h, n_rows, &first_bad);
    if (first_bad != ~u64(0)) throw bad_register(size_t(first_bad >> 3), int(first_bad & 7));
    std::vector<u32> ins = check_code();
// ... 133 lines not shown
```

stwo-brainfuck_amd/csrc/prover_oods.hip:

```cpp
#include "prover.h"
#include <algorithm>

namespace bf {

HipProver::CompositionPlan HipProver::composition_prepare(std::vector<DTree>& trees, const BrainfuckProof& bp, const size_t* main_off, const size_t* inter_off, const Lookups& el) {
    CompositionPlan cp;
    for (int k = 0; k < N_COMPONENTS; k++) { cp.total += n_constraints(k); cp.max_log = std::max(cp.max_log, bp.log_sizes[k] + 1); }
    const bool own_domain = cfg.log_blowup != 1;
    std::vector<DCol> cd_src, cd_dst;
    IsFirstCols cd_is_first{}; cd_is_first.log_min = LOG_N_LANES; cd_is_first.log_max = log_max_rows;
    auto on_constraint_domain = [&](const DCol& poly) {
        if (poly.sliced()) throw HipError("composition: a row-sharded polynomial on the constraint domain");
        DCol e; e.log_size = poly.log_size + 1; e.shift = poly.shift; e.ptr = c.alloc_u32(e.stored());
        cd_src.push_back(poly); cd_dst.push_back(e);
        return e;
    };
    cp.acc.resize(cp.max_log + 1); cp.have.assign(cp.max_log + 1, false); cp.launches.resize(N_COMPONENTS);
    for (int k = 0; k < N_COMPONENTS; k++) {
        u32 log = bp.log_sizes[k], eval_log = log + 1;
        const bool sl = slice_log(eval_log) && !replicate();
        if (!cp.have[eval_log]) {
            cp.acc[eval_log].log_size = eval_log; cp.acc[eval_log].lc = sl ? lc() : 0;
            for (int w = 0; w < 4; w++) cp.acc[eval_log].c[w] = sl ? alloc_slice(eval_log) : c.alloc_u32(size_t(1) << eval_log);
        }
        ConstraintLaunch L{};
        L.overwrite = cp.have[eval_log] ? 0u : 1u;
        cp.have[eval_log] = true;
        const u32 ni = 4 * n_logup_cols(k);
        if (!own_domain) {
            L.is_first = trees[0].evals[log_max_rows - log].ptr;
            for (u32 j = 0; j < n_main_cols(k); j++) L.trace[j] = trees[1].evals[main_off[k] + j].desc();
            for (u32 j = 0; j < ni; j++) L.inter[j] = trees[2].evals[inter_off[k] + j].desc();
        } else {
            const DCol& isf = trees[0].polys[log_max_rows - log];
            if (isf.shift != 0 || isf.log_size != log) throw HipError("composition: unexpected IsFirst polynomial layout");
            if (trees[0].is_first_closed) {
                u32*& e = cd_is_first.ptr[log - LOG_N_LANES];
                if (!e) e = c.alloc_u32(size_t(1) << eval_log);
                L.is_first = e;
            } else L.is_first = on_constraint_domain(isf).ptr;
            for (u32 j = 0; j < n_main_cols(k); j++) L.trace[j] = on_constraint_domain(trees[1].polys[main_off[k] + j]).desc();
            for (u32 j = 0; j < ni; j++) L.inter[j] = on_constraint_domain(trees[2].polys[inter_off[k] + j]).desc();
        }
        for (int w = 0; w < 4; w++) { const DCol& pv = trees[2].prev[inter_off[k] + ni - 4 + w]; L.inter_prev[w] = pv.ptr; }
        if (sl) { L.row0 = (u32)slice_first(eval_log); L.n_rows = (u32)slice_cells(eval_log); }
        for (int w = 0; w < 4; w++) L.acc[w] = cp.acc[eval_log].c[w];
        L.el = el; L.log_size = log;
        for (u32 i = 0; i < 2; i++) L.denom_inv[i] = m_inv(coset_vanishing_m(log, canonic_domain_at(eval_log, i)));
        cp.launches[k] = L;
    }
    if (own_domain) fft_cols(false, cd_src, cd_dst);
    if (own_domain && trees[0].is_first_closed) is_first_lde(c.stream, cd_is_first, 1, c.d_tw, c.d_itw, c.tw_root_log);
    return cp;
}
void HipProver::composition_challenge_fields(const BrainfuckProof& bp, u32 total, Q31 random_coeff, ConstraintLaunch* launches) {
    std::vector<Q31> powers(total);
    { Q31 cur = q_one(); for (u32 i = 0; i < total; i++) { powers[i] = cur; cur = q_mul(cur, random_coeff); } }
    u32 remaining = total;
    for (int k = 0; k < N_COMPONENTS; k++) {
        const u32 nc = n_constraints(k);
        for (u32 j = 0; j < nc; j++) launches[k].coeff[j] = powers[remaining - 1 - j];
        remaining -= nc;
        launches[k].total_sum = bp.claimed_sums[k];
    }
}
void HipProver::composition_fill(const BrainfuckProof& bp, CompositionPlan& cp, Q31 random_coeff) {
    if (!cp.h_staged) throw HipError("composition_fill without a staged launch table");
    composition_challenge_fields(bp, cp.total, random_coeff, cp.h_staged);
}
void HipProver::compute_composition(std::vector<DTree>& trees, const BrainfuckProof& bp, CompositionPlan& cp, Q31 random_coeff, Mailbox* mbx) {
    const u32 max_log = cp.max_log;
    std::vector<DSecure>& acc = cp.acc;
    std::vector<bool>& have = cp.have;
    std::vector<ConstraintLaunch>& launches = cp.launches;
    if (!mbx) composition_challenge_fields(bp, cp.total, random_coeff, launches.data());
    c.stage_checkpoint();
    {
        ConstraintBatch cb;
        constraint_batch_init(cb, launches.data(), N_COMPONENTS);
        const ConstraintLaunch* d_launches = nullptr; const ConstraintBatch* d_cb = nullptr;
        stage_blocks(mbx, [&] {
            d_launches = c.stage(launches.data(), launches.size());
            d_cb = c.stage(&cb, 1);
        });
        if (mbx) cp.h_staged = mbx->host(d_launches);
        eval_constraints_batch(c.stream, d_cb, cb, d_launches);
    }
    BF_HIP(hipGetLastError());
    if (!sharded() || replicate()) {
        std::vector<DCol> all_vals;
        std::vector<u32> logs;
        for (u32 log = max_log; log >= 1; log--) {
            if (!have[log]) continue;
            logs.push_back(log);
            for (int w = 0; w < 4; w++) { DCol v; v.ptr = acc[log].c[w]; v.log_size = log; v.shift = 0; all_vals.push_back(v); }
        }
        if (logs.size() > 13) throw HipError("composition: too many distinct sizes");
        fft_cols(true, all_vals, all_vals);
        AccumulateSizes as{};
        for (int w = 0; w < 4; w++) as.dst[w] = acc[logs[0]].c[w];
        for (size_t k = 1; k < logs.size(); k++) { for (int w = 0; w < 4; w++) as.src[k - 1][w] = acc[logs[k]].c[w]; as.log[k - 1] = logs[k]; }
        as.n = (u32)logs.size() - 1;
        accumulate_sizes(c.stream, as);
        BF_HIP(hipGetLastError());
        trees[3].polys.assign(all_vals.begin(), all_vals.begin() + 4);
        trees[3].owner.assign(4, OWNER_ALL);
        if (replicate() && slice_log(all_vals[0].log_size + cfg.log_blowup)) for (int w = 0; w < 4; w++) trees[3].owner[w] = (u32)w % c.shard.count;
        return;
    }
    bool cur_have = false; std::vector<DCol> cur(4);
    bool cur_owned = false;
    auto owner_of = [&](int w) { return (u32)w % c.shard.count; };
    for (u32 log = 1; log <= max_log; log++) {
        if (!have[log]) continue;
        std::vector<DCol> vals(4), mine_vals;
        const bool sl = acc[log].lc != 0;
        if (sl) {
            const size_t cells = slice_cells(log), bytes = cells * sizeof(u32), first = slice_first(log);
            std::vector<Xfer> sends, recvs;
            for (int w = 0; w < 4; w++) {
                vals[w].log_size = log; vals[w].shift = 0;
                sends.push_back({owner_of(w), acc[log].c[w] + first, bytes});
                if (owner_of(w) == c.shard.rank) {
                    vals[w].ptr = c.alloc_u32(size_t(1) << log);
                    for (u32 r = 0; r < c.shard.count; r++) recvs.push_back({r, vals[w].ptr + r * cells, bytes});
                    mine_vals.push_back(vals[w]);
                }
            }
            std::stable_sort(recvs.begin(), recvs.end(), [](const Xfer& a, const Xfer& b) { return a.peer < b.peer; });
            c.shard.comm->exchange(c.stream, sends, recvs);
        } else {
            if (cur_owned) throw HipError("composition: a replicated accumulator above a row-sharded one");
            for (int w = 0; w < 4; w++) { vals[w].ptr = acc[log].c[w]; vals[w].log_size = log; vals[w].shift = 0; mine_vals.push_back(vals[w]); }
        }
        fft_cols(true, mine_vals, mine_vals);
        if (cur_have)
            for (int w = 0; w < 4; w++) if (!sl || owner_of(w) == c.shard.rank) accumulate(c.stream, vals[w].ptr, cur[w].ptr, 1u << cur[w].log_size);
        cur = vals; cur_have = true; cur_owned = sl;
    }
    trees[3].polys = cur;
    trees[3].owner.assign(4, OWNER_ALL);
    if (cur_owned || (sharded() && slice_log(cur[0].log_size + cfg.log_blowup))) for (int w = 0; w < 4; w++) trees[3].owner[w] = owner_of(w);
}

HipProver::SamplePlan HipProver::sample_prepare(const std::vector<DTree>& trees, const std::vector<std::vector<std::vector<u32>>>& mask) {
    SamplePlan sp;
    for (size_t t = 0; t < trees.size(); t++)
        for (size_t col = 0; col < trees[t].polys.size(); col++)
            for (u32 pt : mask[t][col]) {
                const u32 ji = sp.n_all++;
                const u32 owner = trees[t].owner.empty() ? OWNER_ALL : trees[t].owner[col];
                if (sharded() && ((owner == OWNER_ALL || replicate()) ? ji % c.shard.count : owner) != c.shard.rank) continue;
                const DCol& p = trees[t].polys[col];
                if (trees[t].is_first_closed) { sp.isf.push_back({p.log_size, pt, ji}); continue; }
                EvalJob j{}; j.coeffs = p.ptr; j.log_n = p.log_size - p.shift; j.point = pt; j.factor_shift = p.shift; j.partial_off = sp.partial_off; j.out_idx = ji;
                sp.partial_off += j.log_n > 12 ? 1u << (j.log_n - 12) : 1u;
                sp.jobs.push_back(j);
            }
    return sp;
}
void HipProver::sample_factors(const std::vector<PtQ>& points, uint4* factors) {
    for (size_t p = 0; p < points.size(); p++) {
        Q31 x = points[p].x;
        auto pk = [](Q31 q) { return make_uint4(q.a.a, q.a.b, q.b.a, q.b.b); };
        factors[p * 32 + 0] = pk(points[p].y);
        for (u32 b = 1; b < 32; b++) { factors[p * 32 + b] = pk(x); x = q_double_x(x); }
    }
}
HipProver::SampleRun HipProver::sample_launch(const SamplePlan& sp, const std::vector<PtQ>& points, Mailbox* mbx) {
    SampleRun sr;
    const bool pinned = !sharded() && sp.n_all * sizeof(uint4) <= c.h_small_bytes - 4096;
    if (mbx && !pinned) throw HipError("sampling: too many samples for the pinned result buffer");
    std::vector<uint4> factors(points.size() * 32, make_uint4(0, 0, 0, 0));
    if (!mbx) sample_factors(points, factors.data());
    c.stage_checkpoint();
    const uint4* d_factors = nullptr; const EvalJob* d_jobs = nullptr; const IsFirstSample* d_isf = nullptr;
    stage_blocks(mbx, [&] {
        d_factors = c.stage(factors.data(), factors.size());
        d_jobs = sp.jobs.empty() ? nullptr : c.stage(sp.jobs.data(), sp.jobs.size());
        d_isf = sp.isf.empty() ? nullptr : c.stage(sp.isf.data(), sp.isf.size());
    });
    if (mbx) sr.h_factors = mbx->host(d_factors);
    void* d_partials = c.arena.alloc(size_t(sp.partial_off ? sp.partial_off : 1) * sizeof(uint4));
    if (!pinned) {
        sr.d_out = (uint4*)c.arena.alloc(sp.n_all * sizeof(uint4));
        if (sharded()) BF_HIP(hipMemsetAsync(sr.d_out, 0, sp.n_all * sizeof(uint4), c.stream));
// ... 132 lines not shown
```

Measured before the change: 14.07 billion.

## Fuse interpolation and low-degree extension into a single seam FFT pass

```diff
diff --git a/bindings/rust/bfhip_sys.rs b/bindings/rust/bfhip_sys.rs
--- a/bindings/rust/bfhip_sys.rs
+++ b/bindings/rust/bfhip_sys.rs
@@ -65,6 +65,7 @@
     pub fn bfhip_twiddles(ctx: *mut BfhipCtx, tw_d: *mut *const u32, itw_d: *mut *const u32, root_log: *mut u32) -> i32;
     pub fn bfhip_interpolate(ctx: *mut BfhipCtx, src_cols_h: *const *mut u32, dst_cols_h: *const *mut u32, n_cols: u32, log_size: u32, replicated: i32) -> i32;
     pub fn bfhip_evaluate(ctx: *mut BfhipCtx, coeff_cols_h: *const *mut u32, dst_cols_h: *const *mut u32, n_cols: u32, log_size: u32, log_eval: u32, replicated: i32) -> i32;
+    pub fn bfhip_interpolate_extend(ctx: *mut BfhipCtx, src_cols_h: *const *mut u32, coeff_cols_h: *const *mut u32, ext_cols_h: *const *mut u32, n_cols: u32, log_size: u32, log_blowup: u32, replicated: i32, col_log_sizes_h: *const u32, addend_cols_h: *const *const u32, addend_log_sizes_h: *const u32, n_addends: u32) -> i32;
     pub fn bfhip_is_first_coeffs(ctx: *mut BfhipCtx, log_min: u32, log_max: u32, dst_cols_h: *const *mut u32) -> i32;
     pub fn bfhip_is_first_lde(ctx: *mut BfhipCtx, log_min: u32, log_max: u32, log_blowup: u32, dst_cols_h: *const *mut u32) -> i32;
     pub fn bfhip_is_first_eval_at_point(ctx: *mut BfhipCtx, log_size: u32, point_h: *const u32, out_h: *mut u32) -> i32;
diff --git a/include/bfhip.h b/include/bfhip.h
--- a/include/bfhip.h
+++ b/include/bfhip.h
@@ -58,6 +58,9 @@
 
 int32_t bfhip_interpolate(bfhip_ctx* ctx, uint32_t* const* src_cols_h, uint32_t* const* dst_cols_h, uint32_t n_cols, uint32_t log_size, int32_t replicated);
 int32_t bfhip_evaluate(bfhip_ctx* ctx, uint32_t* const* coeff_cols_h, uint32_t* const* dst_cols_h, uint32_t n_cols, uint32_t log_size, uint32_t log_eval, int32_t replicated);
+int32_t bfhip_interpolate_extend(bfhip_ctx* ctx, uint32_t* const* src_cols_h, uint32_t* const* coeff_cols_h, uint32_t* const* ext_cols_h, uint32_t n_cols, uint32_t log_size,
+                                 uint32_t log_blowup, int32_t replicated, const uint32_t* col_log_sizes_h, const uint32_t* const* addend_cols_h, const uint32_t* addend_log_sizes_h,
+                                 uint32_t n_addends);
 
 int32_t bfhip_is_first_coeffs(bfhip_ctx* ctx, uint32_t log_min, uint32_t log_max, uint32_t* const* dst_cols_h);
 int32_t bfhip_is_first_lde(bfhip_ctx* ctx, uint32_t log_min, uint32_t log_max, uint32_t log_blowup, uint32_t* const* dst_cols_h);
diff --git a/stwo-brainfuck_amd/__init__.py b/stwo-brainfuck_amd/__init__.py
--- a/stwo-brainfuck_amd/__init__.py
+++ b/stwo-brainfuck_amd/__init__.py
@@ -474,6 +474,15 @@
 
     def evaluate(self, coeff_ptrs, dst_ptrs, log_size, log_eval, replicated=False):
         _check(lib().bfhip_evaluate(self._h, self._ptr_array(coeff_ptrs), self._ptr_array(dst_ptrs), len(coeff_ptrs), log_size, log_eval, int(replicated)))
+
+    def interpolate_extend(self, src_ptrs, coeff_ptrs, ext_ptrs, log_size, log_blowup, replicated=False, col_log_sizes=None, addends=None, addend_log_sizes=()):
+        n = len(src_ptrs)
+        logs = (ctypes.c_uint32 * n)(*col_log_sizes) if col_log_sizes is not None else None
+        na = len(addend_log_sizes)
+        add = (ctypes.c_void_p * (n * na))(*[p or None for col in addends for p in col]) if na else None
+        add_logs = (ctypes.c_uint32 * na)(*addend_log_sizes) if na else None
+        _check(lib().bfhip_interpolate_extend(self._h, self._ptr_array(src_ptrs), self._ptr_array(coeff_ptrs), self._ptr_array(ext_ptrs), n, log_size, log_blowup,
+                                              int(replicated), logs, add, add_logs, na))
 
     def is_first_coeffs(self, log_min, log_max, dst_ptrs):
         arr = (ctypes.c_void_p * len(dst_ptrs))(*[p or None for p in dst_ptrs])
diff --git a/stwo-brainfuck_amd/csrc/api.hip b/stwo-brainfuck_amd/csrc/api.hip
--- a/stwo-brainfuck_amd/csrc/api.hip
+++ b/stwo-brainfuck_amd/csrc/api.hip
@@ -513,6 +513,47 @@
     API_CATCH
 }
 
+int32_t bfhip_interpolate_extend(bfhip_ctx* ctx, uint32_t* const* src_cols_h, uint32_t* const* coeff_cols_h, uint32_t* const* ext_cols_h, uint32_t n_cols, uint32_t log_size,
+                                 uint32_t log_blowup, int32_t replicated, const uint32_t* col_log_sizes_h, const uint32_t* const* addend_cols_h, const uint32_t* addend_log_sizes_h,
+                                 uint32_t n_addends) {
+    API_CTX(ctx)
+    Ctx& c = ctx->c;
+    if (!src_cols_h || !coeff_cols_h || !ext_cols_h || (n_addends && (!addend_cols_h || !addend_log_sizes_h))) throw HipError("null argument");
+    const u32 sh = replicated ? 4 : 0;
+    std::vector<DCol> src(n_cols), pol(n_cols), ev(n_cols);
+    std::vector<std::vector<HipProver::SeamAdd>> adds(n_cols);
+    bool seam_for_addends = true;
+    for (u32 i = 0; i < n_cols; i++) {
+        const u32 log = col_log_sizes_h ? col_log_sizes_h[i] : log_size;
+        if (replicated && log < 4) throw HipError("replicated columns need log_size >= 4");
+        if (!replicated && log < 3) throw HipError("circle transforms need log_size >= 3");
+        if (log + log_blowup > c.tw_root_log + 1) throw HipError("log_size + log_blowup exceeds the context's twiddle tree");
+        src[i].ptr = src_cols_h[i]; pol[i].ptr = coeff_cols_h[i]; ev[i].ptr = ext_cols_h[i];
+        if (!src[i].ptr || !pol[i].ptr || !ev[i].ptr) throw HipError("null column");
+        src[i].log_size = pol[i].log_size = log; ev[i].log_size = log + log_blowup;
+        src[i].shift = pol[i].shift = ev[i].shift = sh;
+        for (u32 k = 0; k < n_addends; k++) {
+            const u32* p = addend_cols_h[(size_t)i * n_addends + k];
+            if (!p) continue;
+            if (addend_log_sizes_h[k] > log || addend_log_sizes_h[k] < sh) throw HipError("an addend larger than its column");
+            adds[i].push_back({p, addend_log_sizes_h[k]});
+        }
+        if (adds[i].size() > 1 || (!adds[i].empty() && !fft_seam_eligible(log - sh, log + log_blowup - sh))) seam_for_addends = false;
+    }
+    HipProver pv(c, 0);
+    c.stage_checkpoint();
+    if (seam_for_addends) pv.fft_launch(pv.fft_prepare_seam(src, pol, ev, n_addends ? &adds : nullptr));
+    else {
+        pv.fft_launch(pv.fft_prepare(true, src, pol));
+        for (u32 i = 0; i < n_cols; i++) for (auto& ad : adds[i]) accumulate(c.stream, pol[i].ptr, ad.ptr, 1u << (ad.log - sh));
+        c.stage_checkpoint();
+        pv.fft_launch(pv.fft_prepare(false, pol, ev));
+    }
+    BF_HIP(hipGetLastError());
+    return 0;
+    API_CATCH
+}
+
 
 int32_t bfhip_is_first_coeffs(bfhip_ctx* ctx, uint32_t log_min, uint32_t log_max, uint32_t* const* dst_cols_h) {
     API_CTX(ctx)
diff --git a/stwo-brainfuck_amd/csrc/fft.hip b/stwo-brainfuck_amd/csrc/fft.hip
--- a/stwo-brainfuck_amd/csrc/fft.hip
+++ b/stwo-brainfuck_amd/csrc/fft.hip
@@ -7,6 +7,7 @@
 #include <mutex>
 #include <set>
 #include <string>
+#include <type_traits>
 
 namespace bf {
 
@@ -15,6 +16,7 @@
 static constexpr int CHUNK_LOG = 5;
 static constexpr int STRIDED_K = TILE_LOG - CHUNK_LOG;
 static constexpr int FFT_THREADS = 256;
+static constexpr u32 FFT_MAX_COSETS = 4;
 __device__ __forceinline__ u32 scale_shift(u32 scale) { return (u32)__builtin_ctz(scale); }
 
 __device__ __forceinline__ void point_of_index(u32 idx, const uint2* __restrict__ tlo, const uint2* __restrict__ thi, u32& x, u32& y) {
@@ -144,7 +146,8 @@
     hipLaunchKernelGGL(k_is_first_lde, dim3((lanes + 255) / 256), dim3(256), 0, stream, a, log_blowup, tw, itw, 1u << tw_root_log);
 }
 
-enum { K_TILE12 = 0, K_STRIDED5 = 1, K_STRIDED6 = 2, K_PASS = 3, K_TINY = 4, K_STRIDED_K8 = 5, K_STRIDED_K9 = 6, K_STRIDED_K10 = 7, K_KINDS = 8 };
+enum { K_TILE12 = 0, K_STRIDED5 = 1, K_STRIDED6 = 2, K_PASS = 3, K_TINY = 4, K_STRIDED_K8 = 5, K_STRIDED_K9 = 6, K_STRIDED_K10 = 7, K_STRIDED5_COSETS = 8, K_STRIDED6_COSETS = 9, K_KINDS = 10,
+       K_SEAM5 = 10, K_SEAM6 = 11, K_SEAM5_ADD = 12, K_SEAM6_ADD = 13 };
 struct BlockOfGroup { u32 g, tile, by; };
 template <bool INV> __device__ __forceinline__ void fft_tiny_body(const PassArgs& a, const BlockOfGroup& bg);
 __device__ __forceinline__ BlockOfGroup find_group(const PassArgs* __restrict__ groups, u32 ngroups) {
@@ -153,12 +156,13 @@
     const u32 local = blockIdx.x - groups[g].block0, gx = groups[g].grid_x;
     return {g, local % gx, local / gx};
 }
-__device__ __forceinline__ const u32* layer_table(const PassArgs& a, u32 layer) {
-    u32 eff = a.circle ? layer : layer + 1;
-    u32 lg = a.circle ? a.log : a.log + 1;
+__device__ __forceinline__ const u32* layer_table_of(const u32* tw, u32 tw_total, u32 circle, u32 log, u32 layer) {
+    u32 eff = circle ? layer : layer + 1;
+    u32 lg = circle ? log : log + 1;
     u32 len = 1u << (lg - 1 - eff);
-    return a.tw + (a.tw_total - 2 * len);
-}
+    return tw + (tw_total - 2 * len);
+}
+__device__ __forceinline__ const u32* layer_table(const PassArgs& a, u32 layer) { return layer_table_of(a.tw, a.tw_total, a.circle, a.log, layer); }
 
 template <bool INV>
 __device__ __forceinline__ void fft_pass_body(const PassArgs& a, const BlockOfGroup& bg, u32* __restrict__ s_val, u32* __restrict__ s_tw) {
@@ -405,42 +409,86 @@
     else fft_tile12_body<INV, 0>(a, bg, s_val, s_tw);
 }
 
-template <bool INV, int CL>
+template <bool INV, int CL, bool COSETS = false>
 __global__ void __launch_bounds__(4 << CL, 3) k_fft_strided7(const PassArgs* __restrict__ groups, u32 ngroups) {
     const BlockOfGroup bg = find_group(groups, ngroups);
     const PassArgs a = groups[bg.g];
     constexpr u32 C = 1u << CL, NT = 4u << CL;
     __shared__ __attribute__((aligned(16))) u32 s_val[128 * C];
-    __shared__ u32 s_tw[128];
+    static_assert(!(INV && COSETS), "the zero-extending pass is a forward pass");
+    __shared__ u32 s_tw[COSETS ? 128 * FFT_MAX_COSETS : 128];
     const u32 t = threadIdx.x, lo = a.lo, tile = bg.tile;
     const u32 n_lhi_log = lo - CL;
     const u32 H = tile >> n_lhi_log, Lhi = tile & ((1u << n_lhi_log) - 1);
     const u32 base = (H << (lo + 7)) | (Lhi << CL);
-    if (t < 127) {
-        u32 j = __clz(~(t << 25));
-        u32 q = t - (128u - (128u >> j));
-        s_tw[t] = 2u * layer_table(a, lo + j)[(H << (6 - j)) + q];
-    }
-    auto TW = [&](u32 layer, u32 idx) -> u32 { return s_tw[128u - (128u >> layer) + idx]; };
+    const u32 ncosets = COSETS ? a.ncosets : 1u;
+    for (u32 e = t; e < 128u * ncosets; e += NT) {
+        const u32 tt = e & 127u, hh = COSETS ? e >> 7 : H;
+        if (tt == 127u) continue;
+        u32 j = __clz(~(tt << 25));
+        u32 q = tt - (128u - (128u >> j));
+        s_tw[e] = 2u * layer_table(a, lo + j)[(hh << (6 - j)) + q];
+    }
+    u32 tw0 = 0;
+    auto TW = [&](u32 layer, u32 idx) -> u32 { return s_tw[tw0 + 128u - (128u >> layer) + idx]; };
     const u32 col0 = bg.by * a.cols_per_block, col1 = min(a.ncols, col0 + a.cols_per_block);
     const u32 l4 = 4 * (t & (C / 4 - 1)), r4 = t >> (CL - 2);
+    auto wide_stage = [&](u32 (&r)[8][4]) {
+#pragma unroll
+        for (int s = 0; s < 3; s++) {
+            const int jl = INV ? s : 2 - s;
+#pragma unroll
+            for (int b = 0; b < 4; b++) {
+                const int q0 = ((b >> jl) << (jl + 1)) | (b & ((1 << jl) - 1));
+                u32 w = TW(jl, (8 * r4 + q0) >> (jl + 1));
+#pragma unroll
+                for (int j = 0; j < 4; j++) bfly<INV>(r[q0][j], r[q0 | (1 << jl)][j], w);
+            }
+        }
+    };
+    if constexpr (COSETS) {
+        const u32 src_base = Lhi << CL;
+        for (u32 col = col0 + H; col < col1; col += ncosets) {
+            const BF_GLOBAL char* src = (const BF_GLOBAL char*)as_global(a.src[col]);
+            g_u32p dst = as_global(a.dst[col]);
+            u32 v[2][16];
+#pragma unroll
+            for (u32 g2 = 0; g2 < 2; g2++) {
+                const u32 id = t + NT * g2, l = id & (C - 1), mlow = id >> CL;
+#pragma unroll
+                for (u32 e = 0; e < 16; e++) v[g2][e] = __builtin_nontemporal_load((g_cu32p)(src + ((src_base | ((8 * e + mlow) << lo) | l) << 2)));
+                __builtin_amdgcn_sched_barrier(0);
+            }
+#pragma unroll 1
+            for (u32 h = 0; h < ncosets; h++) {
+                __syncthreads();
+                tw0 = 128u * h;
+#pragma unroll
+                for (u32 g2 = 0; g2 < 2; g2++) {
+                    const u32 id = t + NT * g2, l = id & (C - 1), mlow = id >> CL;
+                    u32 w[16];
+#pragma unroll
+                    for (u32 e = 0; e < 16; e++) w[e] = v[g2][e];
+                    radix16<false>(w, 4, [&](int jl, int pe) -> u32 { return TW(3 + jl, pe); });
+#pragma unroll
+                    for (u32 e = 0; e < 16; e++) s_val[C * (8 * e + mlow) + l] = w[e];
+                }
+                __syncthreads();
+                u32 r[8][4];
+#pragma unroll
+                for (int q = 0; q < 8; q++) { uint4 x = *reinterpret_cast<uint4*>(&s_val[C * (8 * r4 + q) + l4]); r[q][0] = x.x; r[q][1] = x.y; r[q][2] = x.z; r[q][3] = x.w; }
+                wide_stage(r);
+                const u32 out_base = (h << (lo + 7)) | src_base;
+#pragma unroll
+                for (int q = 0; q < 8; q++) st16(dst + (out_base | ((8 * r4 + q) << lo) | l4), make_uint4(r[q][0], r[q][1], r[q][2], r[q][3]));
+            }
+        }
+        return;
+    }
     for (u32 col = col0; col < col1; col++) {
         g_cu32p src = as_global(a.src[col]);
         g_u32p dst = as_global(a.dst[col]);
         __syncthreads();
-        auto wide_stage = [&](u32 (&r)[8][4]) {
-#pragma unroll
-            for (int s = 0; s < 3; s++) {
-                const int jl = INV ? s : 2 - s;
-#pragma unroll
-                for (int b = 0; b < 4; b++) {
-                    const int q0 = ((b >> jl) << (jl + 1)) | (b & ((1 << jl) - 1));
-                    u32 w = TW(jl, (8 * r4 + q0) >> (jl + 1));
-#pragma unroll
-                    for (int j = 0; j < 4; j++) bfly<INV>(r[q0][j], r[q0 | (1 << jl)][j], w);
-                }
-            }
-        };
         auto narrow_task = [&](u32 id, bool from_global, bool to_global) {
             u32 l = id & (C - 1), mlow = id >> CL;
             u32 v[16];
@@ -478,6 +526,131 @@
             wide_stage(r);
 #pragma unroll
             for (int q = 0; q < 8; q++) st16(dst + (base | ((8 * r4 + q) << lo) | l4), make_uint4(r[q][0], r[q][1], r[q][2], r[q][3]));
+        }
+    }
+}
+
+template <int CL, bool ADD>
+__global__ void __launch_bounds__(4 << CL, ADD ? 3 : 4) k_fft_seam(const PassArgs* __restrict__ groups, u32 ngroups) {
+    const BlockOfGroup bg = find_group(groups, ngroups);
+    const PassArgs a = groups[bg.g];
+    constexpr u32 C = 1u << CL, NT = 4u << CL;
+    __shared__ __attribute__((aligned(16))) u32 s_val[128 * C];
+    __shared__ u32 s_tw[128 * (1 + FFT_MAX_COSETS)];
+    const u32 t = threadIdx.x, lo = a.lo, ncosets = a.ncosets;
+    const u32 src_base = bg.tile << CL;
+    for (u32 e = t; e < 128u * (1 + ncosets); e += NT) {
+        const u32 tt = e & 127u, seg = e >> 7;
+        if (tt == 127u) continue;
+        const u32 j = __clz(~(tt << 25)), q = tt - (128u - (128u >> j));
+        s_tw[e] = 2u * (seg == 0 ? layer_table(a, lo + j)[q] : layer_table_of(a.tw2, a.tw_total, a.circle, a.log2, lo + j)[((seg - 1) << (6 - j)) + q]);
+    }
+    u32 tw0 = 0;
+    auto TW = [&](u32 layer, u32 idx) -> u32 { return s_tw[tw0 + 128u - (128u >> layer) + idx]; };
+    const u32 col0 = bg.by * a.cols_per_block, col1 = min(a.ncols, col0 + a.cols_per_block);
+    const u32 sk = scale_shift(a.scale);
+    constexpr bool has_add = ADD;
+    for (u32 col = col0; col < col1; col++) {
+        g_cu32p src = as_global(a.src[col]);
+        BF_GLOBAL char* coef = (BF_GLOBAL char*)as_global(a.dst[col]);
+        g_u32p ext = as_global(a.dst2[col]);
+        __syncthreads();
+        u32 tl = t;
+        asm volatile("" : "+v"(tl));
+        const u32 l4 = 4 * (tl & (C / 4 - 1)), r4 = tl >> (CL - 2);
+        tw0 = 0;
+        u32 asum[2][16];
+        bool add_here = false;
+        u32 add_log = 0;
+        auto add_rows = [&](u32 l) -> u32 { return add_log > lo ? 1u << (add_log - lo) : ((src_base | l) < (1u << add_log) ? 1u : 0u); };
+        if (has_add) {
+            const SeamAddend ad = ld_constant(a.addends + col);
+            add_here = ad.ptr != nullptr; add_log = ad.log;
+            if (add_here) {
+                const BF_GLOBAL char* ap = (const BF_GLOBAL char*)as_global(ad.ptr);
+#pragma unroll
+                for (u32 g2 = 0; g2 < 2; g2++) {
+                    const u32 id = tl + NT * g2, l = id & (C - 1), mlow = id >> CL;
+                    const u32 mlim = add_rows(l);
+                    auto take = [&](u32 m) -> u32 { return *(g_cu32p)(ap + (m < mlim ? ((m << lo) | src_base | l) << 2 : 0u)); };
+                    const u32 ne = ad.log > lo + 3 ? 1u << (ad.log - lo - 3) : 1u;
+                    auto fetch = [&](auto NE) {
+#pragma unroll
+                        for (u32 e = 0; e < 16; e++) asum[g2][e] = e < decltype(NE)::value ? take(8 * e + mlow) : 0u;
+                    };
+                    if (ne == 1) fetch(std::integral_constant<u32, 1>{});
+                    else if (ne == 2) fetch(std::integral_constant<u32, 2>{});
+                    else if (ne == 4) fetch(std::integral_constant<u32, 4>{});
+                    else if (ne == 8) fetch(std::integral_constant<u32, 8>{});
+                    else fetch(std::integral_constant<u32, 16>{});
+                }
+            }
+        }
+        {
+            u32 r[8][4];
+#pragma unroll
+            for (int q = 0; q < 8; q++) { uint4 x = ld16_stream(src + (src_base | ((8 * r4 + q) << lo) | l4)); r[q][0] = x.x; r[q][1] = x.y; r[q][2] = x.z; r[q][3] = x.w; }
+#pragma unroll
+            for (int jl = 0; jl < 3; jl++)
+#pragma unroll
+                for (int b = 0; b < 4; b++) {
+                    const int q0 = ((b >> jl) << (jl + 1)) | (b & ((1 << jl) - 1));
+                    const u32 w = TW(jl, (8 * r4 + q0) >> (jl + 1));
+#pragma unroll
+                    for (int j = 0; j < 4; j++) bfly<true>(r[q0][j], r[q0 | (1 << jl)][j], w);
+                }
+#pragma unroll
+            for (int q = 0; q < 8; q++) *reinterpret_cast<uint4*>(&s_val[C * (8 * r4 + q) + l4]) = make_uint4(r[q][0], r[q][1], r[q][2], r[q][3]);
+        }
+        __syncthreads();
+        u32 v[2][16];
+#pragma unroll
+        for (u32 g2 = 0; g2 < 2; g2++) {
+            const u32 id = tl + NT * g2, l = id & (C - 1), mlow = id >> CL;
+#pragma unroll
+            for (u32 e = 0; e < 16; e++) v[g2][e] = s_val[C * (8 * e + mlow) + l];
+            radix16<true>(v[g2], 4, [&](int jl, int pe) -> u32 { return TW(3 + jl, pe); });
+#pragma unroll
+            for (u32 e = 0; e < 16; e++) v[g2][e] = m_mul_pow2(v[g2][e], sk);
+            if (add_here) {
+                const u32 mlim = add_rows(l);
+#pragma unroll
+                for (u32 e = 0; e < 16; e++) v[g2][e] = m_add(v[g2][e], 8 * e + mlow < mlim ? asum[g2][e] : 0u);
+            }
+#pragma unroll
+            for (u32 e = 0; e < 16; e++) __builtin_nontemporal_store(v[g2][e], (g_u32p)(coef + ((src_base | ((8 * e + mlow) << lo) | l) << 2)));
+            __builtin_amdgcn_sched_barrier(0);
+        }
+#pragma unroll 1
+        for (u32 h = 0; h < ncosets; h++) {
+            if (h) __syncthreads();
+            tw0 = 128u * (1 + h);
+#pragma unroll
+            for (u32 g2 = 0; g2 < 2; g2++) {
+                const u32 id = tl + NT * g2, l = id & (C - 1), mlow = id >> CL;
+                u32 w[16];
+#pragma unroll
+                for (u32 e = 0; e < 16; e++) w[e] = v[g2][e];
+                radix16<false>(w, 4, [&](int jl, int pe) -> u32 { return TW(3 + jl, pe); });
+#pragma unroll
+                for (u32 e = 0; e < 16; e++) s_val[C * (8 * e + mlow) + l] = w[e];
+            }
+            __syncthreads();
+            u32 r[8][4];
+#pragma unroll
+            for (int q = 0; q < 8; q++) { uint4 x = *reinterpret_cast<uint4*>(&s_val[C * (8 * r4 + q) + l4]); r[q][0] = x.x; r[q][1] = x.y; r[q][2] = x.z; r[q][3] = x.w; }
+#pragma unroll
+            for (int jl = 2; jl >= 0; jl--)
+#pragma unroll
+                for (int b = 0; b < 4; b++) {
+                    const int q0 = ((b >> jl) << (jl + 1)) | (b & ((1 << jl) - 1));
+                    const u32 w = TW(jl, (8 * r4 + q0) >> (jl + 1));
+#pragma unroll
+                    for (int j = 0; j < 4; j++) bfly<false>(r[q0][j], r[q0 | (1 << jl)][j], w);
+                }
+            const u32 out_base = (h << (lo + 7)) | src_base;
+#pragma unroll
+            for (int q = 0; q < 8; q++) st16(ext + (out_base | ((8 * r4 + q) << lo) | l4), make_uint4(r[q][0], r[q][1], r[q][2], r[q][3]));
         }
     }
 }
@@ -596,12 +769,18 @@
 }
 
 
-void fft_plan(FftPlan& plan, bool inverse, const FftJob* jobs, size_t njobs, const u32* tw, const u32* itw, u32 tw_root_log) {
-    plan.inverse = inverse; plan.groups.clear(); plan.launches.clear(); plan.d_groups = nullptr;
-    struct Item { int pi, kind; PassArgs a; double bytes, alg; bool single = false; double bfly() const { return 0.5 * a.ncols * (double)(1u << a.log) * a.k; } };
-    std::vector<Item> items;
-    int max_np = 0;
+static int fft_seam_mode() {
+    static const int mode = [] { const char* v = getenv("BFHIP_FFT_SEAM"); return (v && v[0] == '0') ? 0 : (v && v[0] == '1') ? 1 : 2; }();
+    return mode;
+}
+
+namespace {
+struct Item { int pi, kind; PassArgs a; double bytes, alg; bool single = false; int job = -1; double bfly() const { return 0.5 * a.ncols * (double)(1u << a.log) * a.k; } };
+}
+static void plan_collect(std::vector<Item>& items, int& max_np, bool inverse, const FftJob* jobs, size_t njobs, const u32* tw, const u32* itw, u32 tw_root_log) {
+    auto tag = [&](int ji) { for (auto& it : items) if (it.job < 0) it.job = ji; };
     for (size_t ji = 0; ji < njobs; ji++) {
+        tag((int)ji - 1);
         const FftJob& job = jobs[ji];
         const u32 ncols = job.ncols, log = job.log, src_log = job.src_log;
         if (ncols == 0) continue;
@@ -654,7 +833,10 @@
 #endif
                     const bool wide = a.lo >= 6 && log >= BF_STRIDED_WIDE_MIN_LOG;
                     PassArgs b = a; b.grid_x = wide ? ntiles / 2 : ntiles; b.block0 = gy;
-                    items.push_back({pi, wide ? K_STRIDED6 : K_STRIDED5, b, bytes, alg});
+                    const bool cosets = !inverse && first && fft_seam_mode() >= 1 && a.lo + 7 == src_log && log > src_log && (1u << (log - src_log)) <= FFT_MAX_COSETS;
+                    if (cosets) b.ncosets = 1u << (log - src_log);
+                    if (cosets) items.push_back({pi, wide ? K_STRIDED6_COSETS : K_STRIDED5_COSETS, b, 4.0 * ncols * ((double)(1u << src_log) + (double)(1u << log)), alg});
+                    else items.push_back({pi, wide ? K_STRIDED6 : K_STRIDED5, b, bytes, alg});
                 }
             }
             continue;
@@ -689,6 +871,9 @@
             items.push_back({pi, K_PASS, b, 8.0 * ncols * (double)(1u << log), alg, np == 1 && log < (u32)TILE_LOG});
         }
     }
+    tag((int)njobs - 1);
+}
+static void plan_emit(FftPlan& plan, std::vector<Item>& items, int max_np, bool inverse) {
     {
         static const bool fuse = [] { const char* v = getenv("BFHIP_FFT_FUSE_SMALL"); return !v || v[0] != '0'; }();
         int host_pi = -1;
@@ -699,7 +884,7 @@
     }
     for (int pi = 0; pi < max_np; pi++)
         for (int kind = 0; kind < K_KINDS; kind++) {
-            FftLaunch L{}; L.kind = kind; L.first_group = (u32)plan.groups.size();
+            FftLaunch L{}; L.kind = kind; L.inverse = inverse; L.first_group = (u32)plan.groups.size();
             u32 blocks = 0;
             for (auto& it : items) {
                 if (it.pi != pi || it.kind != kind) continue;
@@ -714,6 +899,75 @@
         }
 }
 
+void fft_plan(FftPlan& plan, bool inverse, const FftJob* jobs, size_t njobs, const u32* tw, const u32* itw, u32 tw_root_log) {
+    plan.inverse = inverse; plan.groups.clear(); plan.launches.clear(); plan.d_groups = nullptr;
+    std::vector<Item> items;
+    int max_np = 0;
+    plan_collect(items, max_np, inverse, jobs, njobs, tw, itw, tw_root_log);
+    plan_emit(plan, items, max_np, inverse);
+}
+
+bool fft_seam_eligible(u32 log, u32 log_ext) {
+    const bool two_pass = [] { const char* v = getenv("BFHIP_FFT_TWO_PASS"); return !v || v[0] != '0'; }();
+    return fft_seam_mode() >= 2 && log >= 13 && !(two_pass && log >= 20 && log <= 22) && log_ext > log && (1u << (log_ext - log)) <= FFT_MAX_COSETS;
+}
+
+void fft_plan_seam(FftPlan& plan, const FftSeamJob* jobs, size_t njobs, const u32* tw, const u32* itw, u32 tw_root_log) {
+    plan.inverse = true; plan.groups.clear(); plan.launches.clear(); plan.d_groups = nullptr;
+    std::vector<FftJob> ji, jf;
+    std::vector<size_t> jf_of;
+    for (size_t j = 0; j < njobs; j++) {
+        const FftSeamJob& s = jobs[j];
+        ji.push_back({s.d_src, s.d_dst, s.ncols, s.log, s.log, s.circle});
+        if (s.d_ext) { jf.push_back({(const u32* const*)s.d_dst, s.d_ext, s.ncols, s.log_ext, s.log, s.circle}); jf_of.push_back(j); }
+    }
+    std::vector<Item> inv, fwd, seam;
+    int np_inv = 0, np_fwd = 0;
+    plan_collect(inv, np_inv, true, ji.data(), ji.size(), tw, itw, tw_root_log);
+    plan_collect(fwd, np_fwd, false, jf.data(), jf.size(), tw, itw, tw_root_log);
+    std::vector<bool> taken(njobs, false);
+    if (fft_seam_mode() >= 2)
+        for (size_t f = 0; f < fwd.size(); f++) {
+            if (fwd[f].pi != 0 || (fwd[f].kind != K_STRIDED5_COSETS && fwd[f].kind != K_STRIDED6_COSETS)) continue;
+            const size_t j = jf_of[(size_t)fwd[f].job];
+            for (size_t i = 0; i < inv.size(); i++) {
+                if (inv[i].job != (int)j || (inv[i].kind != K_STRIDED5 && inv[i].kind != K_STRIDED6) || inv[i].a.scale == 1 || inv[i].a.lo != fwd[f].a.lo) continue;
+                const u32 cl = fwd[f].kind == K_STRIDED6_COSETS ? 6 : 5;
+                Item s = inv[i];
+                s.a.dst2 = fwd[f].a.dst; s.a.tw2 = fwd[f].a.tw; s.a.log2 = fwd[f].a.log; s.a.ncosets = fwd[f].a.ncosets;
+                s.a.addends = jobs[j].d_addends; s.a.n_addends = jobs[j].d_addends ? 1 : 0;
+                s.pi = 0; s.kind = jobs[j].d_addends ? (cl == 6 ? K_SEAM6_ADD : K_SEAM5_ADD) : (cl == 6 ? K_SEAM6 : K_SEAM5);
+                s.a.grid_x = 1u << (s.a.lo - cl);
+                const double n = (double)(1u << s.a.log), n_ext = (double)(1u << s.a.log2);
+                s.bytes = 4.0 * s.a.ncols * (n + n + n_ext); s.alg = inv[i].alg + fwd[f].alg;
+                seam.push_back(s);
+                seam.back().a.k = 7;
+                inv.erase(inv.begin() + (long)i); fwd[f].pi = -1;
+                taken[j] = true;
+                break;
+            }
+        }
+    for (size_t j = 0; j < njobs; j++) if (jobs[j].d_addends && !taken[j]) throw std::runtime_error("fft_plan_seam: addends on a job that does not take the seam launch");
+    fwd.erase(std::remove_if(fwd.begin(), fwd.end(), [](const Item& it) { return it.pi < 0; }), fwd.end());
+    plan_emit(plan, inv, np_inv, true);
+    for (int kind : {K_SEAM5, K_SEAM6, K_SEAM5_ADD, K_SEAM6_ADD}) {
+        FftLaunch L{}; L.kind = kind; L.inverse = true; L.first_group = (u32)plan.groups.size();
+        u32 blocks = 0;
+        for (auto& it : seam) {
+            if (it.kind != kind) continue;
+            PassArgs a = it.a;
+            const u32 gy = a.block0;
+            a.block0 = blocks; blocks += a.grid_x * gy;
+            plan.groups.push_back(a);
+            L.bytes += it.bytes; L.alg += it.alg;
+            L.bfly += 0.5 * a.ncols * 7.0 * ((double)(1u << a.log) + (double)(1u << a.log2));
+        }
+        L.ngroups = (u32)plan.groups.size() - L.first_group; L.total_blocks = blocks;
+        if (L.ngroups) plan.launches.push_back(L);
+    }
+    plan_emit(plan, fwd, np_fwd, false);
+}
+
 static const char* fft_prof_name(const char* base, const FftLaunch& L) {
     static const bool detail = [] { const char* v = getenv("BFHIP_FFT_PROF_DETAIL"); return v && v[0] == '1'; }();
     if (!detail) return base;
@@ -725,8 +979,8 @@
 void fft_run(hipStream_t stream, const FftPlan& plan) {
     if (plan.launches.empty()) return;
     if (!plan.d_groups) throw std::runtime_error("fft_run: the plan's group table has not been staged");
-    const bool inverse = plan.inverse;
     for (const FftLaunch& L : plan.launches) {
+        const bool inverse = L.inverse;
         const PassArgs* g = plan.d_groups + L.first_group;
         const dim3 grid(L.total_blocks);
         switch (L.kind) {
@@ -745,6 +999,18 @@
                 ProfScope ps(stream, fft_prof_name(inverse ? "k_fft_strided7<true>" : "k_fft_strided7<false>", L), L.bytes, L.alg, false, L.bfly);
                 if (inverse) hipLaunchKernelGGL((k_fft_strided7<true, 6>), grid, dim3(256), 0, stream, g, L.ngroups);
                 else hipLaunchKernelGGL((k_fft_strided7<false, 6>), grid, dim3(256), 0, stream, g, L.ngroups);
+                break; }
+            case K_STRIDED5_COSETS: case K_STRIDED6_COSETS: {
+                ProfScope ps(stream, fft_prof_name("k_fft_strided7<false>", L), L.bytes, L.alg, false, L.bfly);
+                if (L.kind == K_STRIDED5_COSETS) hipLaunchKernelGGL((k_fft_strided7<false, 5, true>), grid, dim3(128), 0, stream, g, L.ngroups);
+                else hipLaunchKernelGGL((k_fft_strided7<false, 6, true>), grid, dim3(256), 0, stream, g, L.ngroups);
+                break; }
+            case K_SEAM5: case K_SEAM6: case K_SEAM5_ADD: case K_SEAM6_ADD: {
+                ProfScope ps(stream, fft_prof_name("k_fft_seam", L), L.bytes, L.alg, false, L.bfly);
+                if (L.kind == K_SEAM5) hipLaunchKernelGGL((k_fft_seam<5, false>), grid, dim3(128), 0, stream, g, L.ngroups);
+                else if (L.kind == K_SEAM6) hipLaunchKernelGGL((k_fft_seam<6, false>), grid, dim3(256), 0, stream, g, L.ngroups);
+                else if (L.kind == K_SEAM5_ADD) hipLaunchKernelGGL((k_fft_seam<5, true>), grid, dim3(128), 0, stream, g, L.ngroups);
+                else hipLaunchKernelGGL((k_fft_seam<6, true>), grid, dim3(256), 0, stream, g, L.ngroups);
                 break; }
             case K_STRIDED_K8: {
                 ProfScope ps(stream, fft_prof_name(inverse ? "k_fft_stridedK<true>" : "k_fft_stridedK<false>", L), L.bytes, L.alg, false, L.bfly);
diff --git a/stwo-brainfuck_amd/csrc/kernels.h b/stwo-brainfuck_amd/csrc/kernels.h
--- a/stwo-brainfuck_amd/csrc/kernels.h
+++ b/stwo-brainfuck_amd/csrc/kernels.h
@@ -57,6 +57,8 @@
 
 void gen_twiddles(hipStream_t stream, u32* d_tw, u32* d_itw, u32 R, const uint2* d_tlo, const uint2* d_thi);
 struct FftJob { const u32* const* d_src; u32* const* d_dst; u32 ncols, log, src_log; bool circle; };
+struct SeamAddend { const u32* ptr; u32 log, pad; };
+struct FftSeamJob { const u32* const* d_src; u32* const* d_dst; u32* const* d_ext; u32 ncols, log, log_ext; bool circle; const SeamAddend* d_addends; };
 struct PassArgs {
     u32* const* dst;
     const u32* const* src;
@@ -71,10 +73,17 @@
     const u32* tw;
     u32 block0, grid_x;
     u32 kind;
-};
-struct FftLaunch { int kind; u32 first_group, ngroups, total_blocks; double bytes, alg, bfly; };
+    u32* const* dst2;
+    const u32* tw2;
+    const SeamAddend* addends;
+    u32 log2, n_addends;
+    u32 ncosets;
+};
+struct FftLaunch { int kind; bool inverse; u32 first_group, ngroups, total_blocks; double bytes, alg, bfly; };
 struct FftPlan { bool inverse = false; std::vector<PassArgs> groups; std::vector<FftLaunch> launches; const PassArgs* d_groups = nullptr; };
 void fft_plan(FftPlan& plan, bool inverse, const FftJob* jobs, size_t njobs, const u32* tw, const u32* itw, u32 tw_root_log);
+void fft_plan_seam(FftPlan& plan, const FftSeamJob* jobs, size_t njobs, const u32* tw, const u32* itw, u32 tw_root_log);
+bool fft_seam_eligible(u32 log, u32 log_ext);
 void fft_run(hipStream_t stream, const FftPlan& plan);
 
 struct IsFirstCols { u32* ptr[28]; u32 log_min, log_max; };
diff --git a/stwo-brainfuck_amd/csrc/prover.h b/stwo-brainfuck_amd/csrc/prover.h
--- a/stwo-brainfuck_amd/csrc/prover.h
+++ b/stwo-brainfuck_amd/csrc/prover.h
@@ -28,7 +28,7 @@
     bool mine(u64 cell, u32 rank) const { return lc == 0 || (cell >> (log_size - lc)) == rank; }
 };
 struct DevMerkle { std::vector<u32*> layers; std::vector<u32> shifts; u32 max_log = 0; Hash32 root; int band_lo = 0, band_hi = -1; std::vector<DCol> cols; };
-struct DTree { std::vector<DCol> polys, evals, prev; std::vector<u32> owner; DevMerkle mk; bool is_first_closed = false; };
+struct DTree { std::vector<DCol> polys, evals, prev; std::vector<u32> owner; DevMerkle mk; bool is_first_closed = false; bool evals_on_stream = false; };
 struct DSecure {
     u32* c[4]; u32 log_size; u32 lc = 0;
     bool mine(u64 cell, u32 rank) const { return lc == 0 || (cell >> (log_size - lc)) == rank; }
@@ -127,6 +127,8 @@
     void preflight(const TraceInput& in);
 
     FftPlan fft_prepare(bool inverse, const std::vector<DCol>& src, const std::vector<DCol>& dst);
+    struct SeamAdd { const u32* ptr; u32 log; };
+    FftPlan fft_prepare_seam(const std::vector<DCol>& src, const std::vector<DCol>& pol, const std::vector<DCol>& ev, const std::vector<std::vector<SeamAdd>>* addends = nullptr);
     void fft_launch(const FftPlan& plan);
     void fft_cols(bool inverse, const std::vector<DCol>& src, const std::vector<DCol>& dst);
     template <class F> void stage_blocks(Mailbox* mbx, F&& f) {
diff --git a/stwo-brainfuck_amd/csrc/prover.hip b/stwo-brainfuck_amd/csrc/prover.hip
--- a/stwo-brainfuck_amd/csrc/prover.hip
+++ b/stwo-brainfuck_amd/csrc/prover.hip
@@ -270,7 +270,7 @@
         composition_plan = composition_prepare(trees, bp, main_off, inter_off, el);
         compute_composition(trees, bp, composition_plan, q_zero(), &mb_constraints);
         build_mask();
-        commit_tree_overlapped(trees[3], pinned_root3, nullptr, 3);
+        commit_tree_overlapped(trees[3], pinned_root3, nullptr, 3, trees[3].evals_on_stream);
         sample_plan = sample_prepare(trees, mask);
         mark("composition phase enqueued behind its mailbox");
         c.wait_stamp(2);
@@ -315,7 +315,7 @@
         build_mask();
         if (sharded()) commit_tree(trees[3]);
         else {
-            commit_tree_overlapped(trees[3], pinned_root3);
+            commit_tree_overlapped(trees[3], pinned_root3, nullptr, -1, trees[3].evals_on_stream);
             sample_plan = sample_prepare(trees, mask);
             mark("composition tree enqueued + samples prepared");
         }
diff --git a/stwo-brainfuck_amd/csrc/prover_commit.hip b/stwo-brainfuck_amd/csrc/prover_commit.hip
--- a/stwo-brainfuck_amd/csrc/prover_commit.hip
+++ b/stwo-brainfuck_amd/csrc/prover_commit.hip
@@ -1,5 +1,6 @@
 #include "prover.h"
 #include <algorithm>
+#include <tuple>
 
 namespace bf {
 
@@ -46,6 +47,43 @@
     std::vector<FftJob> fj;
     for (auto& j : jobs) fj.push_back({d_ptrs + j.off, (u32* const*)(d_ptrs + j.off + j.n), (u32)j.n, j.log - j.sh, j.src_log - j.sh, j.sh == 0});
     fft_plan(plan, inverse, fj.data(), fj.size(), c.d_tw, c.d_itw, c.tw_root_log);
+    plan.d_groups = c.stage(plan.groups.data(), plan.groups.size());
+    sb.end();
+    return plan;
+}
+FftPlan HipProver::fft_prepare_seam(const std::vector<DCol>& src, const std::vector<DCol>& pol, const std::vector<DCol>& ev, const std::vector<std::vector<SeamAdd>>* addends) {
+    std::map<std::tuple<u32, u32, u32, u32>, std::vector<size_t>> groups;
+    for (size_t i = 0; i < pol.size(); i++) {
+        if (src[i].log_size != pol[i].log_size || src[i].shift != pol[i].shift || (ev[i].ptr && ev[i].shift != pol[i].shift)) throw HipError("fft_prepare_seam: columns of one entry differ in size or storage");
+        groups[{pol[i].log_size, pol[i].shift, ev[i].ptr ? ev[i].log_size : 0u, (addends && !(*addends)[i].empty()) ? 1u : 0u}].push_back(i);
+    }
+    struct Job { size_t off, n, add_off; u32 log, log_ext, sh, n_add; };
+    std::vector<Job> jobs; std::vector<const u32*> ptrs; std::vector<SeamAddend> adds;
+    for (auto it = groups.rbegin(); it != groups.rend(); ++it) {
+        const auto& idx = it->second;
+        Job j{ptrs.size(), idx.size(), adds.size(), std::get<0>(it->first), std::get<2>(it->first), std::get<1>(it->first), 0};
+        for (size_t i : idx) ptrs.push_back(src[i].ptr);
+        for (size_t i : idx) ptrs.push_back(pol[i].ptr);
+        for (size_t i : idx) ptrs.push_back(ev[i].ptr);
+        if (std::get<3>(it->first))
+            for (size_t i : idx) {
+                const auto& l = (*addends)[i];
+                if (l.size() > 1) throw HipError("fft_prepare_seam: one addend per column (merge them first)");
+                adds.push_back(l.empty() ? SeamAddend{nullptr, 0, 0} : SeamAddend{l[0].ptr, l[0].log - j.sh, 0});
+                j.n_add = 1;
+            }
+        jobs.push_back(j);
+    }
+    FftPlan plan;
+    if (jobs.empty()) return plan;
+    StageBatch sb(c);
+    const u32* const* d_ptrs = c.stage(ptrs.data(), ptrs.size());
+    const SeamAddend* d_adds = adds.empty() ? nullptr : c.stage(adds.data(), adds.size());
+    std::vector<FftSeamJob> fj;
+    for (auto& j : jobs)
+        fj.push_back({d_ptrs + j.off, (u32* const*)(d_ptrs + j.off + j.n), j.log_ext ? (u32* const*)(d_ptrs + j.off + 2 * j.n) : nullptr, (u32)j.n, j.log - j.sh, j.log_ext ? j.log_ext - j.sh : 0u,
+                      j.sh == 0, j.n_add ? d_adds + j.add_off : nullptr});
+    fft_plan_seam(plan, fj.data(), fj.size(), c.d_tw, c.d_itw, c.tw_root_log);
     plan.d_groups = c.stage(plan.groups.data(), plan.groups.size());
     sb.end();
     return plan;
@@ -347,22 +385,17 @@
     }
     const bool overlap = (c.overlap & 1u) && !ev[1].empty() && max_log >= 19;
     c.stage_checkpoint();
-    FftPlan fi[2], fe[2];
+    FftPlan fe[2];
     MerklePlan mp;
     {
         StageBatch sb(c);
-        for (int w = 0; w < 2; w++) {
-            if (interp_src) fi[w] = fft_prepare(true, src[w], pol[w]);
-            fe[w] = fft_prepare(false, pol[w], ev[w]);
-        }
+        for (int w = 0; w < 2; w++) fe[w] = interp_src ? fft_prepare_seam(src[w], pol[w], ev[w]) : fft_prepare(false, pol[w], ev[w]);
         mp = merkle_plan(t.evals);
         sb.end();
     }
     hipStream_t main = c.stream, aux = c.aux_of(main);
-    if (interp_src) fft_launch(fi[0]);
     fft_launch(fe[0]);
     if (!overlap) {
-        if (interp_src) fft_launch(fi[1]);
         fft_launch(fe[1]);
         bool stamped = false;
         t.mk = merkle_run(mp, pinned_root, false, nullptr, nullptr, stamp_slot, &stamped);
@@ -370,7 +403,6 @@
     } else {
         hipEvent_t e1 = c.next_event(), e2 = c.next_event(), e3 = c.next_event();
         BF_HIP(hipEventRecord(e1, main));
-        if (interp_src) fft_launch(fi[1]);
         fft_launch(fe[1]);
         BF_HIP(hipEventRecord(e2, main));
         BF_HIP(hipStreamWaitEvent(aux, e1, 0));
diff --git a/stwo-brainfuck_amd/csrc/prover_oods.hip b/stwo-brainfuck_amd/csrc/prover_oods.hip
--- a/stwo-brainfuck_amd/csrc/prover_oods.hip
+++ b/stwo-brainfuck_amd/csrc/prover_oods.hip
@@ -96,12 +96,35 @@
             for (int w = 0; w < 4; w++) { DCol v; v.ptr = acc[log].c[w]; v.log_size = log; v.shift = 0; all_vals.push_back(v); }
         }
         if (logs.size() > 13) throw HipError("composition: too many distinct sizes");
-        fft_cols(true, all_vals, all_vals);
-        AccumulateSizes as{};
-        for (int w = 0; w < 4; w++) as.dst[w] = acc[logs[0]].c[w];
-        for (size_t k = 1; k < logs.size(); k++) { for (int w = 0; w < 4; w++) as.src[k - 1][w] = acc[logs[k]].c[w]; as.log[k - 1] = logs[k]; }
-        as.n = (u32)logs.size() - 1;
-        accumulate_sizes(c.stream, as);
+        const u32 top = logs[0];
+        if (!sharded() && fft_seam_eligible(top, top + cfg.log_blowup)) {
+            std::vector<DCol> top_vals(all_vals.begin(), all_vals.begin() + 4), small_vals(all_vals.begin() + 4, all_vals.end()), ev(4);
+            std::vector<std::vector<SeamAdd>> adds(4);
+            if (!small_vals.empty()) {
+                fft_cols(true, small_vals, small_vals);
+                AccumulateSizes as{};
+                for (int w = 0; w < 4; w++) as.dst[w] = acc[logs[1]].c[w];
+                for (size_t k = 2; k < logs.size(); k++) { for (int w = 0; w < 4; w++) as.src[k - 2][w] = acc[logs[k]].c[w]; as.log[k - 2] = logs[k]; }
+                as.n = (u32)logs.size() - 2;
+                accumulate_sizes(c.stream, as);
+                for (int w = 0; w < 4; w++) adds[w].push_back({acc[logs[1]].c[w], logs[1]});
+            }
+            trees[3].evals.resize(4);
+            for (int w = 0; w < 4; w++) {
+                DCol e; e.log_size = top + cfg.log_blowup; e.shift = 0; e.ptr = c.alloc_u32(e.stored());
+                ev[w] = e; trees[3].evals[w] = e;
+            }
+            c.stage_checkpoint();
+            fft_launch(fft_prepare_seam(top_vals, top_vals, ev, small_vals.empty() ? nullptr : &adds));
+            trees[3].evals_on_stream = true;
+        } else {
+            fft_cols(true, all_vals, all_vals);
+            AccumulateSizes as{};
+            for (int w = 0; w < 4; w++) as.dst[w] = acc[logs[0]].c[w];
+            for (size_t k = 1; k < logs.size(); k++) { for (int w = 0; w < 4; w++) as.src[k - 1][w] = acc[logs[k]].c[w]; as.log[k - 1] = logs[k]; }
+            as.n = (u32)logs.size() - 1;
+            accumulate_sizes(c.stream, as);
+        }
         BF_HIP(hipGetLastError());
         trees[3].polys.assign(all_vals.begin(), all_vals.begin() + 4);
         trees[3].owner.assign(4, OWNER_ALL);
```

Result: no change. 14.16 billion, median of 6 (+0.6%).
